# we1pingyu/CALD

Measured on AMD Instinct MI355X. Metric: unlabeled images scored/sec (CALD consistency sweep), higher is better.
Workload: dtype f32

## Files before the change

### cald_amd/_ffi.py

```python
import ctypes as C
import os

_HERE = os.path.dirname(os.path.abspath(__file__))
LIB_PATH = os.path.join(_HERE, "lib", "libcaldhip.so")
_lib = None

c_f = C.POINTER(C.c_float)
c_i = C.POINTER(C.c_int)
c_i64 = C.POINTER(C.c_int64)
c_d = C.POINTER(C.c_double)
c_u8 = C.POINTER(C.c_uint8)
c_i8 = C.POINTER(C.c_int8)


class ModelCfg(C.Structure):
    _fields_ = [("arch", C.c_int), ("depth", C.c_int), ("num_classes", C.c_int), ("min_size", C.c_int),
                ("max_size", C.c_int), ("box_score_thresh", C.c_float), ("box_nms_thresh", C.c_float),
                ("detections_per_img", C.c_int), ("rpn_pre_nms_top_n", C.c_int), ("rpn_post_nms_top_n", C.c_int),
                ("rpn_nms_thresh", C.c_float), ("precision", C.c_int)]


PRECISION = {"fp32": 0, "f16x3": 1}


# ... 144 lines not shown
    "cald_op_cls_corr": (C.c_int, [C.c_void_p, C.c_int, c_f, c_i64, C.c_int, c_f]),
    "cald_op_score_batch": (C.c_int, [C.c_void_p, C.POINTER(ScoreProbe)]),
    "cald_op_pair_params": (C.c_int, [C.c_int, C.c_int, C.c_int, C.c_double, c_f]),
    "cald_op_ls_tail": (C.c_int, [C.c_int, c_f, C.c_int, c_f, c_i, c_i, c_d]),
    "cald_op_coco_match": (C.c_int, [C.c_void_p, C.c_int, c_i64, c_i64, c_d, c_d, c_d, c_d, c_u8, c_u8, C.c_int, c_d, C.c_int, c_d,
                                     C.POINTER(C.c_int32), c_u8, c_u8]),
    "cald_op_voc_match": (C.c_int, [C.c_void_p, C.c_int, c_i64, c_i64, c_d, c_u8, c_d, c_i64, C.c_int, c_d, C.c_int64, c_d, c_i64, c_u8, c_u8]),
    "cald_op_pil_resize": (C.c_int, [C.c_void_p, C.c_void_p, C.c_int, C.c_int, C.c_void_p, C.c_int, C.c_int]),
    "cald_op_cutout_rects": (C.c_int, [C.c_uint64, C.c_int, C.c_int, C.c_int, c_f, C.c_int, c_i, c_i]),
    "cald_op_cutout_geometry": (C.c_int, [C.c_int, C.c_int, C.c_int, C.c_int, C.c_int, c_i, C.c_int, c_i, c_i]),
    "cald_op_augment": (C.c_int, [C.c_void_p, C.c_int, C.c_double, C.c_uint64, C.c_void_p, C.c_int, C.c_int, C.c_int, c_f,
                                  C.c_void_p, c_f, c_i]),
    "cald_op_noise_stream": (C.c_int, [C.c_void_p, C.c_uint64, C.c_void_p, C.c_int, C.c_int, C.c_int, c_i, c_d, C.POINTER(C.c_void_p)]),
    "cald_op_frcnn_postprocess": (C.c_int, [C.c_void_p, C.c_int, C.c_int, c_f, c_f, c_f, C.c_int, C.c_int, C.c_int, C.c_int, C.c_float, C.c_float,
                                            C.c_int, c_f, c_f, c_i64, c_f, c_f, c_f, c_i]),
    "cald_op_frcnn_postprocess_min": (C.c_int, [C.c_void_p, C.c_int, C.c_int, c_f, c_f, c_f, C.c_int, C.c_int, C.c_int, C.c_int, C.c_float, C.c_float,
                                                C.c_int, C.c_float, c_f, c_f, c_i64, c_f, c_f, c_f, c_i]),
    "cald_op_ssm_postprocess": (C.c_int, [C.c_void_p, C.c_int, C.c_int, c_f, c_f, c_f, C.c_int, C.c_int, C.c_int, C.c_int, C.c_float, C.c_int,
                                          c_i, c_i, c_f, c_f, c_i8]),
    "cald_op_retina_postprocess": (C.c_int, [C.c_void_p, C.POINTER(c_f), C.POINTER(c_f), c_i, C.c_int, C.c_int, c_f] + [C.c_int] * 6
                                   + [C.c_float, C.c_float, C.c_int, c_f, c_f, c_i64, c_f, c_f, c_i]),
    "cald_op_retina_ssm_postprocess": (C.c_int, [C.c_void_p, C.POINTER(c_f), C.POINTER(c_f), c_i, C.c_int, C.c_int, c_f] + [C.c_int] * 6
                                       + [C.c_float, C.c_float, C.c_int, C.c_void_p, C.c_void_p, c_i, c_i, c_i, c_f, c_f, c_i8]),
    "cald_op_rpn_prune": (C.c_int, [C.c_void_p, C.POINTER(RpnPruneProbe)]),
    "cald_op_roi_align": (C.c_int, [C.c_void_p, C.POINTER(c_f), c_i, C.c_int, C.c_int, c_f, c_f]),
    "cald_op_conv2d": (C.c_int, [C.c_void_p, c_f, C.c_int, C.c_int, C.c_int, c_f, C.c_int, C.c_int, C.c_int, C.c_int,
                                 C.c_int, c_f, c_f, c_f, c_f, C.c_int, c_f]),
    "cald_op_conv_probe": (C.c_int, [C.c_void_p, C.c_int, C.POINTER(ConvProbe), C.c_int, C.c_int, C.c_int, C.c_char_p, C.c_int]),
    "cald_op_mfma_f16": (C.c_int, [C.c_void_p, C.POINTER(C.c_uint16), C.POINTER(C.c_uint16), C.POINTER(C.c_uint32), C.POINTER(C.c_uint32), C.c_int64]),
    "cald_op_conv2d_f16x3": (C.c_int, [C.c_void_p, c_f, C.c_int, C.c_int, C.c_int, c_f, C.c_int, C.c_int, C.c_int, C.c_int,
                                       C.c_int, c_f, c_f, c_f, c_f, C.c_int, c_f]),
    "cald_op_conv_bench": (C.c_int, [C.c_void_p] + [C.c_int] * 12 + [c_d, c_d]),
    "cald_op_row_pack_lookup": (C.c_int, [C.c_int, c_i, c_i, C.c_int, C.c_int, C.c_int64, c_i64, c_i, c_i64, c_i64]),
    "cald_op_transform_size": (C.c_int, [C.c_int, C.c_int, C.c_int, C.c_int, c_i, c_i, c_i, c_i]),
    "cald_debug_tensor": (C.c_int, [C.c_void_p, C.c_char_p, C.c_int, c_f, C.c_int64, c_i64]),
    "cald_jpeg_info": (C.c_int, [C.c_void_p, C.c_size_t, c_i, c_i, c_i]),
    "cald_jpeg_decode_batch": (C.c_int, [C.c_void_p, C.c_int, C.POINTER(C.c_void_p), C.POINTER(C.c_size_t), C.POINTER(C.c_void_p)]),
    "cald_jpeg_probe": (C.c_int, [C.c_void_p, C.c_size_t, c_i, c_i, c_i, c_i]),
    "cald_jpeg_decode_batch_any": (C.c_int, [C.c_void_p, C.c_int, C.POINTER(C.c_void_p), C.POINTER(C.c_size_t), C.POINTER(C.c_void_p)]),
    "cald_jpeg_decode_host": (C.c_int, [C.c_void_p, C.c_size_t, C.c_void_p]),
    "cald_profile_enable": (C.c_int, [C.c_void_p, C.c_int]),
    "cald_profile_read": (C.c_int, [C.c_void_p, c_d, c_d, c_i64, c_d]),
    "cald_profile_prune": (C.c_int, [C.c_void_p, c_d, c_d, c_d, c_d, c_d]),
    "cald_profile_roi_rows": (C.c_int, [C.c_void_p, c_d, c_i64]),
    "cald_profile_cutout": (C.c_int, [C.c_void_p, c_d, c_d, c_i64, c_i64]),
    "cald_model_set_cutout_reuse": (C.c_int, [C.c_void_p, C.c_int, c_i]),
    "cald_profile_cutout_stages": (C.c_int, [C.c_void_p, c_d, c_d, c_d, c_d, c_i64]),
    "cald_model_set_cutout_retention_cap": (C.c_int, [C.c_void_p, C.c_int64, c_i64]),
    "cald_op_cutout_fpn_geometry": (C.c_int, [C.c_int, C.c_int, C.c_int, C.c_int, C.c_int, c_i, C.c_int, c_i, c_i]),
    "cald_model_set_look_fuse": (C.c_int, [C.c_void_p, C.c_int, c_i]),
    "cald_model_set_row_packing": (C.c_int, [C.c_void_p, C.c_int, c_i]),
    "cald_model_set_box_min_size": (C.c_int, [C.c_void_p, C.c_float, c_f]),
    "cald_profile_dump": (C.c_int, [C.c_void_p, C.c_char_p]),
    "cald_train_packed_floats": (C.c_int, [C.c_int] * 6 + [c_i64]),
    "cald_train_pack_conv": (C.c_int, [C.c_void_p] * 5 + [C.c_int] * 6 + [C.c_void_p]),
    "cald_train_pack_plan_scratch_floats": (C.c_int, [C.c_int, C.POINTER(PackJob), c_i64]),
    "cald_train_pack_plan_create": (C.c_int, [C.c_void_p, C.c_int, C.POINTER(PackJob), C.c_void_p, C.c_int64, C.POINTER(C.c_void_p)]),
    "cald_train_pack_plan_run": (C.c_int, [C.c_void_p, C.c_void_p]),
    "cald_train_pack_plan_destroy": (C.c_int, [C.c_void_p]),
    "cald_train_conv": (C.c_int, [C.c_void_p, C.c_int, C.c_int, C.c_int, C.c_void_p, C.c_int, C.c_void_p] + [C.c_int] * 8
                        + [C.c_void_p, C.c_void_p, C.c_int, C.c_int, C.c_void_p, C.c_void_p, C.c_int]),
    "cald_train_conv_group": (C.c_int, [C.c_void_p, C.c_int, C.c_int, c_i, C.POINTER(C.c_void_p), C.c_int, C.POINTER(C.c_void_p)] + [C.c_int] * 8
                              + [C.POINTER(C.c_void_p), C.POINTER(C.c_void_p), C.c_int]),
    "cald_train_conv_wgrad": (C.c_int, [C.c_void_p, C.c_int, C.c_int, C.c_int, C.c_void_p, C.c_int, C.c_int, C.c_void_p, C.c_int,
                                        C.c_int, C.c_int, C.c_int, C.c_int, C.c_int, C.c_void_p, C.c_void_p, C.c_void_p, C.c_int]),
    "cald_train_linear_wgrad": (C.c_int, [C.c_void_p, C.c_int, C.c_void_p, C.c_int, C.c_void_p, C.c_int, C.c_int, C.c_int,
                                          C.c_void_p, C.c_void_p, C.c_int]),
    "cald_train_wgrad_plan": (C.c_int, [C.c_longlong] + [C.c_int] * 12 + [C.POINTER(WgradPlan)]),
    "cald_train_relu_bwd": (C.c_int, [C.c_void_p, C.c_longlong, C.c_int, C.c_void_p, C.c_void_p, C.c_void_p]),
    "cald_train_add": (C.c_int, [C.c_void_p, C.c_longlong, C.c_void_p, C.c_void_p, C.c_void_p]),
    "cald_train_dilate": (C.c_int, [C.c_void_p] + [C.c_int] * 7 + [C.c_void_p, C.c_void_p]),
    "cald_train_upsample_bwd": (C.c_int, [C.c_void_p] + [C.c_int] * 6 + [C.c_void_p, C.c_void_p]),
    "cald_train_rpn_proposals": (C.c_int, [C.c_void_p, C.c_int, C.c_int, C.c_int, c_i, C.POINTER(C.c_void_p), c_i, C.c_int, C.c_int, C.c_int,
                                           C.c_float, C.c_float, C.c_void_p, C.c_void_p]),
    "cald_train_roi_sample_host": (C.c_int, [C.c_int, c_i, c_i, c_i, C.c_void_p, C.c_void_p, C.c_void_p, C.c_int, C.c_double, C.c_int, C.c_int,
                                             C.c_void_p, C.c_void_p, C.c_void_p, C.c_void_p, C.c_void_p, C.c_void_p, c_i, c_i, c_i]),
    "cald_train_roi_gather": (C.c_int, [C.c_void_p, C.c_void_p, C.c_void_p, C.c_void_p, C.c_int, C.c_int, C.c_int] + [C.c_float] * 4 + [C.c_void_p, C.c_void_p]),
    "cald_train_anchors": (C.c_int, [C.c_void_p, C.c_int, C.c_int, C.c_int, c_i, C.c_void_p]),
    "cald_train_match": (C.c_int, [C.c_void_p, C.c_int, C.c_void_p, C.c_int, C.c_void_p, C.c_float, C.c_float, C.c_int, C.c_void_p, C.c_void_p]),
    "cald_train_box_encode": (C.c_int, [C.c_void_p, C.c_int, C.c_void_p, C.c_void_p, C.c_float, C.c_float, C.c_float, C.c_float, C.c_void_p]),
    "cald_train_roi_align": (C.c_int, [C.c_void_p, C.POINTER(C.c_void_p), c_i, C.c_int, C.c_int, C.c_void_p, C.c_void_p]),
    "cald_train_roi_align_bwd": (C.c_int, [C.c_void_p, C.c_int, C.POINTER(C.c_void_p), c_i, C.c_int, C.c_int, C.c_void_p, C.c_void_p]),
    "cald_train_softmax_ce": (C.c_int, [C.c_void_p, C.c_int, C.c_int, C.c_int, C.c_void_p, C.c_void_p, C.c_float, C.c_void_p, C.c_void_p]),
    "cald_train_smooth_l1": (C.c_int, [C.c_void_p, C.c_int, C.c_void_p, C.c_void_p, C.c_void_p, C.c_float, C.c_float, C.c_void_p, C.c_float,
# ... 55 lines not shown
```

### cald_amd/csrc/common.h

```cpp
#pragma once
#include <hip/hip_runtime.h>
#include <stdint.h>
#include <math.h>

#define CALD_MAX_VIEWS 128
#define CALD_MAX_LEVELS 9
#define CALD_ROI_CAP 1000
#define CALD_MAX_CUT 4

struct LevelSeg {
    long long pix_off;
    int H, W;
    int tile_start;
    int pad_;
};

#if defined(__HIPCC__)
__device__ __forceinline__ int seg_find_view(const LevelSeg* __restrict__ seg, const int V, const int mt) {
    int lo = 0, hi = V - 1;
    while (lo < hi) {
        const int mid = (lo + hi + 1) >> 1;
        if (seg[mid].tile_start <= mt) lo = mid; else hi = mid - 1;
    }
    return lo;
}
__host__ __device__ __forceinline__ int seg_find_row(const LevelSeg* __restrict__ seg, const int V, const long long row) {
    int lo = 0, hi = V - 1;
    while (lo < hi) {
        const int mid = (lo + hi + 1) >> 1;
        if (seg[mid].pix_off <= row) lo = mid; else hi = mid - 1;
    }
    return lo;
}
#endif

static inline int conv_pack_rows(const LevelSeg* si, const LevelSeg* so, const LevelSeg* su, int V, int Cin, int out_ld) {
    const long long total = so[V].pix_off, LIM = 0x7FFE0000LL - (1 << 16);
    if (V < 1 || total < 1 || total > 0x7FFFFFFFLL - 128) return 0;
    int vf = 0;
    for (int v = 0; v < V; v++) {
        const long long b = so[v].pix_off, e = so[v + 1].pix_off;
        if (e == b) continue;
        if ((e - b + 128) * out_ld * 4 > LIM) return 0;
        if (b % 128 == 0) continue;
        const long long t0 = b / 128 * 128;
        while (so[vf + 1].pix_off <= t0) vf++;
        if ((si[v + 1].pix_off - si[vf].pix_off) * Cin * 4 > LIM) return 0;
        if (su && (su[v + 1].pix_off - su[vf].pix_off) * out_ld * 4 > LIM) return 0;
    }
    return (int)total;
}

struct BatchPlan {
    LevelSeg seg[CALD_MAX_LEVELS][CALD_MAX_VIEWS + 1];
};

#define CALD_GATHER_RECTS 8
struct GatherSet {
    int nr;
    int cum[CALD_GATHER_RECTS + 1];
    int x0[CALD_GATHER_RECTS], y0[CALD_GATHER_RECTS], w[CALD_GATHER_RECTS];
};
__device__ __forceinline__ int gather_pixel(const GatherSet& g, const int m, const int W) {
    int k = 0;
    while (k + 1 < g.nr && m >= g.cum[k + 1]) k++;
    const int j = m - g.cum[k], w = g.w[k], ry = j / w;
    return (g.y0[k] + ry) * W + g.x0[k] + (j - ry * w);
}

struct ConvArgs {
    const float* in;
    float* out;
    const float* w;
    const float* w4;
    const void* w16;
    float w16_unscale;
    const float* bias;
    const float* scale;
    const float* shift;
    const float* residual;
    const float* up;
    const LevelSeg* seg_in;
    const LevelSeg* seg_out;
    const LevelSeg* seg_up;
    const int* dyn_rows;
    const int* row_map;
    int V;
    int Cin, Cout, CoutPad, Kpad;
    int KH, KW, stride, pad;
    int relu;
    int total_mtiles;
    int out_ld;
    const float* zeros;
    int in_relu;
    const float* mask;
    const float* wstem;
// ... 174 lines not shown
```

### cald_amd/csrc/conv_p4.hip

```cpp
#include "h16.h"

typedef float f32x16 __attribute__((ext_vector_type(16)));
typedef int i32x4 __attribute__((ext_vector_type(4)));
typedef float f32x4 __attribute__((ext_vector_type(4)));

template <int EPI, bool MASK, int TM, int TN, bool GATHER = false, bool GEXTRA = false>
__device__ __forceinline__ void p4_epilogue(const ConvArgs& a, const f32x16 (&acc)[TM][TN], float* smem, const int v, const LevelSeg& so,
                                            const int m0, const int Mv, const int n0, const bool straddle = false) {
    constexpr int BM = 128, WN = 2;
    const int tid = threadIdx.x, lane = tid & 63, wave = tid >> 6;
    const int wm = wave / WN, wn = wave % WN;
    const int kh_lane = lane >> 5, l31 = lane & 31;
    const int Ho = so.H, Wo = so.W;
    const int out_ld = a.out_ld;
    float* __restrict__ out_v = a.out + so.pix_off * (long long)out_ld;
    const float* __restrict__ ex_v = nullptr;
    int upH = 1, upW = 1;
    float uph_s = 0.f, upw_s = 0.f;
    long long up_off = 0;
    if (EPI == 1) ex_v = a.residual + so.pix_off * (long long)out_ld;
    if (EPI == 2) {
        const LevelSeg su = a.seg_up[v];
        up_off = su.pix_off;
        ex_v = a.up + su.pix_off * (long long)out_ld;
        upH = su.H; upW = su.W;
        uph_s = (float)upH / (float)Ho; upw_s = (float)upW / (float)Wo;
    }
    const bool relu = a.relu != 0, has_bias = a.bias != nullptr, has_bn = a.scale != nullptr;
    constexpr bool has_mask = MASK;
    const float* __restrict__ mask_v = has_mask ? a.mask + so.pix_off * (long long)out_ld : out_v;
    const int row_b = out_ld * 4;
    const unsigned long long vb64 = (unsigned long long)(GATHER ? Ho * Wo : Mv) * (unsigned)row_b;
    const unsigned valid_b = vb64 < 0x7FFE0000ull ? (unsigned)vb64 : 0x7FFE0000u;
    const __amdgpu_buffer_rsrc_t rsO = __builtin_amdgcn_make_buffer_rsrc((void*)out_v, 0, valid_b, 0x00020000);
    const __amdgpu_buffer_rsrc_t rsX = __builtin_amdgcn_make_buffer_rsrc((void*)(EPI != 0 ? ex_v : out_v), 0, EPI == 1 ? valid_b : 0x7FFE0000, 0x00020000);
    const __amdgpu_buffer_rsrc_t rsM = __builtin_amdgcn_make_buffer_rsrc((void*)mask_v, 0, valid_b, 0x00020000);
    static_assert(!(GATHER && EPI == 2), "gathered rows take no top-down term");
    const int Mlast = Mv - 1;
    int* const s_src = reinterpret_cast<int*>(smem);
    if (EPI == 2 || GATHER) {
        if (tid < BM) {
            int m = m0 + tid;
            if (GATHER) {
                s_src[tid] = m < Mv ? gather_pixel(a.gather[v], m, Wo) * row_b : 0x7FFF0000;
            } else if (EPI == 2 && straddle) {
                int src = 0;
                if (m < Mv) {
                    const long long r = so.pix_off + m;
                    int vr = v;
                    while (vr + 1 < a.V && a.seg_out[vr + 1].pix_off <= r) vr++;
                    const LevelSeg sor = a.seg_out[vr], sur = a.seg_up[vr];
                    const int ml = (int)(r - sor.pix_off), oy = ml / sor.W, ox = ml - oy * sor.W;
                    const float hs = (float)sur.H / (float)sor.H, ws = (float)sur.W / (float)sor.W;
                    int sy = (int)floorf((float)oy * hs); sy = sy > sur.H - 1 ? sur.H - 1 : sy;
                    int sx = (int)floorf((float)ox * ws); sx = sx > sur.W - 1 ? sur.W - 1 : sx;
                    src = ((int)(sur.pix_off - up_off) + sy * sur.W + sx) * out_ld * 4;
                }
                s_src[tid] = src;
            } else {
                m = m < Mlast ? m : Mlast;
                const int oy = m / Wo, ox = m - oy * Wo;
                int sy = (int)floorf((float)oy * uph_s); sy = sy > upH - 1 ? upH - 1 : sy;
                int sx = (int)floorf((float)ox * upw_s); sx = sx > upW - 1 ? upW - 1 : sx;
                s_src[tid] = (sy * upW + sx) * out_ld * 4;
            }
        }
        __syncthreads();
    }
    auto gather_offs = [&](const int i, const int n, const bool nok, int (&go)[16]) {
        const int rl = wm * TM * 32 + i * 32 + 4 * kh_lane;
#pragma unroll
        for (int q = 0; q < 4; q++) {
            const i32x4 so4 = *reinterpret_cast<const i32x4*>(s_src + rl + 8 * q);
#pragma unroll
            for (int jj = 0; jj < 4; jj++) go[4 * q + jj] = nok ? so4[jj] + n * 4 : 0x7FFF0000;
        }
    };
// ... 152 lines not shown
    constexpr bool MASK = (EPIX & 4) != 0;
    constexpr bool FUSE = (EPIX & 8) != 0;
    constexpr bool GATHER = (EPIX & 16) != 0;
    constexpr bool GEXTRA = (EPIX & 32) != 0;
    static_assert(!GEXTRA || GATHER, "the extras bit rides on the gathered-rows bit");
    static_assert(!(GATHER && (FUSE || MASK || C4)), "gathered rows: plain EPI 0 / 1 kernels only");
    constexpr int BM = 128, BN = 64 * TN, BK = 16, TM = 2, WN = 2;
    constexpr int TILE_A = 2 * BM * 8, TILE_F = TILE_A + 2 * BN * 8;
    constexpr int FUSE_T = 4 * TILE_A;
    __shared__ __attribute__((aligned(16))) float smem[FUSE ? FUSE_T + 4096 : 3 * TILE_F];

    const int tid = threadIdx.x, lane = tid & 63, wave = tid >> 6;
    const int wm = wave / WN, wn = wave % WN;
    const int NT = a.CoutPad / BN;
    unsigned long long* const trace = (a.trace && blockIdx.x < (1u << 17)) ? a.trace + (size_t)blockIdx.x * 8 : nullptr;
    if (trace && tid == 0) {
        trace[0] = __builtin_amdgcn_s_memtime();
        trace[5] = (unsigned)__builtin_amdgcn_s_getreg((31 << 11) | 4);
        trace[6] = (unsigned)__builtin_amdgcn_s_getreg((31 << 11) | 20);
        trace[7] = blockIdx.x;
    }
    int mt, nt;
    if (a.KH * a.KW > 1) {
        const int MT = a.total_mtiles, CH = (MT + 7) >> 3;
        const int xcd = blk & 7, idx = blk >> 3;
        mt = xcd * CH + idx / NT; nt = idx % NT;
        if (idx / NT >= CH || mt >= MT) return;
    } else {
        const int b = blk, MT = a.total_mtiles, MT8 = MT & ~7;
        if (b < MT8 * NT) { const int xcd = b & 7, idx = b >> 3; mt = (idx / NT) * 8 + xcd; nt = idx % NT; }
        else { const int r = b - MT8 * NT; mt = MT8 + r / NT; nt = r % NT; }
    }
    const int n0 = nt * BN;
    constexpr bool CAN_PACK = !C4 && !MASK && !FUSE && !GATHER;
    const bool packed = CAN_PACK && a.packed_rows != 0;
    const int v = packed ? seg_find_row(a.seg_out, a.V, (long long)mt * BM) : seg_find_view(a.seg_out, a.V, mt);
    const LevelSeg so = a.seg_out[v];
    const LevelSeg si = a.seg_in[v];
    const int Ho = so.H, Wo = so.W, Hi = si.H, Wi = si.W;
    int Mv = Ho * Wo;
    if (a.dyn_rows) { const int d = a.dyn_rows[v]; Mv = d < Mv ? d : Mv; }
    if (GATHER) Mv = a.gather[v].cum[a.gather[v].nr];
    int m0 = (mt - so.tile_start) * BM;
    bool straddle = false;
    if (CAN_PACK && packed) {
        const int row0 = mt * BM, left = a.packed_rows - row0;
        m0 = row0 - (int)so.pix_off;
        const int end = m0 + (left < BM ? left : BM);
        straddle = end > Mv;
        Mv = end;
    }
    if (m0 >= Mv) return;
    const float* __restrict__ in_v = a.in + si.pix_off * (long long)a.Cin;
    const int Cin = a.Cin, KW = a.KW, KH = a.KH, CoutPad = a.CoutPad;
    const bool in_relu = a.in_relu != 0;

    const int g = tid & 3, arow = tid >> 2;
    unsigned rowmask[2];
    int rowvoff[2], riy0[2], rix0[2];
    int tapw[2] = {0, 0};
#pragma unroll
    for (int p = 0; p < 2; p++) {
        const int m = m0 + arow + 64 * p;
        int ml = m, Wo_r = Wo, Hi_r = Hi, Wi_r = Wi, dpix = 0;
        if (CAN_PACK && straddle && m < Mv) {
            const long long r = so.pix_off + m;
            int vr = v;
            while (vr + 1 < a.V && a.seg_out[vr + 1].pix_off <= r) vr++;
            const LevelSeg sor = a.seg_out[vr], sir = a.seg_in[vr];
            ml = (int)(r - sor.pix_off); Wo_r = sor.W; Hi_r = sir.H; Wi_r = sir.W; dpix = (int)(sir.pix_off - si.pix_off);
        }
        const int mp = GATHER ? (m < Mv ? gather_pixel(a.gather[v], m, Wo) : 0) : (a.row_map && m < Mv) ? a.row_map[so.pix_off + m] : ml;
        const int oy = mp / Wo_r, ox = mp - oy * Wo_r;
        const int iy0 = oy * a.stride - a.pad, ix0 = ox * a.stride - a.pad;
        unsigned msk = 0;
        if (!C4 && m < Mv)
            for (int t = 0; t < KH * KW; t++) {
                const int th = t / KW, tw = t - th * KW;
                const int iy = iy0 + th, ix = ix0 + tw;
                if (iy >= 0 && iy < Hi_r && ix >= 0 && ix < Wi_r) msk |= 1u << t;
            }
        rowmask[p] = msk;
        rowvoff[p] = (((oy * a.stride) * Wi + ox * a.stride) * Cin + (C4 ? 0 : 4 * g)) * 4;
        if (CAN_PACK && straddle) { rowvoff[p] = ((dpix + iy0 * Wi_r + ix0) * Cin + 4 * g) * 4; tapw[p] = Wi_r; }
        riy0[p] = m < Mv ? iy0 : -0x40000000; rix0[p] = ix0;
    }
    const int Wi_s = straddle ? 0 : Wi, Cin_s = straddle ? 0 : Cin, cin_v4 = straddle ? Cin * 4 : 0;
    const __amdgpu_buffer_rsrc_t rsA = __builtin_amdgcn_make_buffer_rsrc(
        (void*)(in_v - (straddle ? 0ll : (long long)a.pad * (Wi + 1) * Cin)), 0, 0x7FFE0000, 0x00020000);
    const __amdgpu_buffer_rsrc_t rsB = __builtin_amdgcn_make_buffer_rsrc((void*)(a.w4 + (long long)n0 * 8), 0, 0x7FFE0000, 0x00020000);
    int u_kh = 0, u_kw = 0, u_ci = 0, u_kt = 0;
    const int a_kq = g >> 1, a_j = 2 * (g & 1);
    int aw_off[2][2];
#pragma unroll
    for (int p = 0; p < 2; p++) {
        const int r = arow + 64 * p;
#pragma unroll
        for (int h = 0; h < 2; h++) aw_off[p][h] = ((a_kq * BM + r) * 2 + (h ^ ((r >> 3) & 1))) * 4 + a_j;
    }
    const int b_t = TN == 2 ? tid : (tid & 127), b_kq = TN == 2 ? 0 : (tid >> 7);
    const int b_nl = b_t >> 1, b_h = b_t & 1;
    const int bvoff0 = (b_kq * CoutPad * 8 + b_nl * 8 + b_h * 4) * 4, bvoff1 = bvoff0 + CoutPad * 8 * 4;
    const int bw_off0 = TILE_A + ((b_kq * BN + b_nl) * 2 + (b_h ^ ((b_nl >> 3) & 1))) * 4, bw_off1 = bw_off0 + BN * 8;

    f32x4 ra0, ra1, rb0, rb1 = {0.f, 0.f, 0.f, 0.f};
// ... 344 lines not shown
__global__ __launch_bounds__(256, 3) void conv_p4_kernel(const ConvArgs a) { conv_p4_body<EPI, C4, TN, TAPS>(a, blockIdx.x); }
template <int EPI, bool C4, int TN, int TAPS>
__global__ __launch_bounds__(256, 3) void conv_p4_group_kernel(const ConvGroup g) {
    int i = 0;
    while (i + 1 < g.n && g.blk0[i + 1] <= (int)blockIdx.x) i++;
    conv_p4_body<EPI, C4, TN, TAPS>(g.p[i], (int)blockIdx.x - g.blk0[i]);
}
__global__ __launch_bounds__(256, 3) void conv_p4_fused_kernel(const ConvGroup g) { conv_p4_body<8, false, 1, 9>(g.p[0], blockIdx.x, &g.p[1]); }

static inline int p4_taps(const ConvArgs& a) {
    if (a.Cin % 16 != 0) return 0;
    if (a.KH == 3 && a.KW == 3) return 9;
    if (a.KH == 1 && a.KW == 1) return 1;
    return 0;
}

static inline int p4_grid_mtiles(const ConvArgs& a) { return a.KH * a.KW > 1 ? 8 * ((a.total_mtiles + 7) / 8) : a.total_mtiles; }

static inline bool p4_refuses(const ConvArgs& a) {
    if (!a.w4 || !a.out || a.in16 || a.ex16 || a.CoutPad % 64 != 0 || (a.residual && a.up)) return true;
    const bool extra = a.out16 || a.energy4;
    if (extra && (a.residual || a.up || a.mask)) return true;
    if (a.energy4 && a.CoutPad != 256) return true;
    if (a.row_map && (a.residual || a.up || a.mask || a.gather)) return true;
    return false;
}
static inline bool p4_tile_ok(const ConvArgs& a, const bool wide, const ConvForce f) {
    if (f.tile == TILE_NARROW && wide) return false;
    if (f.tile == TILE_WIDE && !wide) return false;
    return !(a.energy4 && !wide);
}

static inline ConvArgs p4_tiled(ConvArgs a) {
    if (a.packed_rows > 0 && a.Cin != 4 && !a.dyn_rows && !a.row_map && !a.gather && !a.mask) a.total_mtiles = (a.packed_rows + 127) / 128;
    else a.packed_rows = 0;
    return a;
}

#define P4_NAME(K, EPIV, C4V, TNV, TAPSV) K "<" #EPIV "," #C4V "," #TNV "," #TAPSV ">"
template <int EPI, bool C4, int TN, int TAPS>
static const char* p4_go(const dim3 grid, hipStream_t stream, const ConvArgs& a, const char* name) {
    hipLaunchKernelGGL((conv_p4_kernel<EPI, C4, TN, TAPS>), grid, dim3(256), 0, stream, a);
    return name;
}
template <int EPI, int TN, int TAPS>
static const char* p4_group_go(const dim3 grid, hipStream_t stream, const ConvGroup& g, const char* name) {
    hipLaunchKernelGGL((conv_p4_group_kernel<EPI, false, TN, TAPS>), grid, dim3(256), 0, stream, g);
    return name;
}

const char* launch_conv_p4_group(const ConvArgs* p, int n, hipStream_t stream, ConvForce f) {
    if (n < 1 || n > CALD_MAX_GROUP) return nullptr;
    const bool wide = f.tile == TILE_NARROW ? false : p[0].CoutPad % 128 == 0;
    ConvGroup g; g.n = n; int blk = 0;
    for (int i = 0; i < n; i++) {
        const ConvArgs a = p4_tiled(p[i]);
        if (p4_refuses(a) || !p4_tile_ok(a, wide, f) || (a.CoutPad % 128 == 0) != (p[0].CoutPad % 128 == 0)) return nullptr;
        if (a.Cin % 16 != 0 || a.KH * a.KW > 32 || a.residual || a.up) return nullptr;
        if ((a.mask != nullptr) != (p[0].mask != nullptr) || (a.gather != nullptr) != (p[0].gather != nullptr)) return nullptr;
        if (a.gather && (!wide || p4_taps(a) != 9 || a.mask || a.in_relu || a.dyn_rows || a.row_map)) return nullptr;
        if (a.mask && (a.out16 || a.energy4)) return nullptr;
        g.blk0[i] = blk; blk += p4_grid_mtiles(a) * (a.CoutPad / (wide ? 128 : 64)); g.p[i] = a;
    }
    g.blk0[n] = blk;
    const int taps = p4_taps(p[0]);
    for (int i = 1; i < n; i++) if (p4_taps(p[i]) != taps) return nullptr;
    const dim3 grid((unsigned)blk);
// ... 70 lines not shown
```

### cald_amd/csrc/ctx.hip

```cpp
#include "host.h"

static thread_local char g_err[512] = "";
int cald_host::fail(int code, const char* fmt, ...) {
    va_list ap; va_start(ap, fmt); vsnprintf(g_err, sizeof(g_err), fmt, ap); va_end(ap);
    return code;
}

int cald_internal_fail(int code, const char* fmt, ...) {
    va_list ap; va_start(ap, fmt); vsnprintf(g_err, sizeof(g_err), fmt, ap); va_end(ap);
    return code;
}
void cald_internal_train_release(cald_ctx* c);

extern "C" const char* cald_last_error(void) { return g_err; }
extern "C" int cald_version(void) { return 100; }

hipStream_t cald_internal_stream(cald_ctx* c) { return c->stream; }
int cald_internal_device(cald_ctx* c) { return c->device; }
const float* cald_internal_zeros(cald_ctx* c) { return c->d_zeros; }
int cald_internal_scratch(cald_ctx* c, size_t bytes, void** out) {
    if (bytes > c->train_scratch_cap) {
        HIPCHK(hipStreamSynchronize(c->stream));
        if (c->train_scratch) HIPCHK(hipFree(c->train_scratch));
        c->train_scratch = nullptr; c->train_scratch_cap = 0;
// ... 129 lines not shown
    return 0;
}

extern "C" int cald_profile_roi_rows(cald_ctx* c, double* mean_rows_per_view, int64_t* views) {
    if (!c) return fail(CALD_ERR_INVALID, "ctx is null");
    HIPCHK(hipStreamSynchronize(c->stream));
    unsigned long long rows = 0;
    HIPCHK(hipMemcpy(&rows, c->d_roi_rows, 8, hipMemcpyDeviceToHost));
    if (views) *views = c->prof_roi_views;
    if (mean_rows_per_view) *mean_rows_per_view = c->prof_roi_views ? (double)rows / (double)c->prof_roi_views : 0.0;
    return 0;
}

extern "C" int cald_profile_cutout(cald_ctx* c, double* rows3, double* dense_rows3, int64_t* batches, int64_t* fallbacks) {
    if (!c) return fail(CALD_ERR_INVALID, "ctx is null");
    for (int i = 0; i < 3; i++) { if (rows3) rows3[i] = c->cut_rows[i]; if (dense_rows3) dense_rows3[i] = c->cut_dense[i]; }
    if (batches) *batches = c->cut_batches;
    if (fallbacks) *fallbacks = c->cut_fallbacks;
    return 0;
}

extern "C" int cald_profile_cutout_stages(cald_ctx* c, double* rows6, double* dense_rows6, double* tiles6, double* dense_tiles6, int64_t* kept3) {
    if (!c) return fail(CALD_ERR_INVALID, "ctx is null");
    for (int i = 0; i < 6; i++) {
        if (rows6) rows6[i] = c->cut_st_rows[i];
        if (dense_rows6) dense_rows6[i] = c->cut_st_dense[i];
        if (tiles6) tiles6[i] = c->cut_st_tiles[i];
        if (dense_tiles6) dense_tiles6[i] = c->cut_st_dense_tiles[i];
    }
    if (kept3) for (int i = 0; i < 3; i++) kept3[i] = c->cut_kept[i];
    return 0;
}

extern "C" int cald_profile_dump(cald_ctx* c, const char* path) {
    if (!c || !path) return fail(CALD_ERR_INVALID, "null argument");
    HIPCHK(hipStreamSynchronize(c->stream));
    FILE* f = fopen(path, "w");
    if (!f) return fail(CALD_ERR_INVALID, "cannot open %s", path);
    fprintf(f, "launch,desc,gflop,ms,tflops\n");
    std::vector<unsigned long long> lg((size_t)CALD_PRUNE_LOG * 4, 0ull);
    if (!c->prof_gather.empty()) HIPCHK(hipMemcpy(lg.data(), c->d_prune_log, lg.size() * 8, hipMemcpyDeviceToHost));
    for (size_t i = 0; i < c->prof_launches.size(); i++) {
        const ProfLaunch& L = c->prof_launches[i];
        float t = 0.f; hipEventElapsedTime(&t, L.e0, L.e1);
        double fl = L.flops;
        const char* extra = L.tag ? ",f16x3-lookahead" : "";
        auto g = c->prof_gather.find(i);
        if (g != c->prof_gather.end()) {
            for (int l = 0; l < 2; l++) {
                const unsigned long long sel = lg[(size_t)g->second.log * 4 + 2 * l], tot = lg[(size_t)g->second.log * 4 + 2 * l + 1];
                if (tot) fl -= g->second.cap[l] * (1.0 - (double)sel / (double)tot);
            }
            extra = ",gathered-rows";
        }
        fprintf(f, "%zu,\"%s%s\",%.3f,%.4f,%.2f\n", i, L.desc.c_str(), extra, fl / 1e9, t, fl / (t * 1e-3) / 1e12);
    }
    fclose(f);
    return 0;
}
extern "C" int cald_profile_prune_fallbacks(cald_ctx* c, int64_t* n) {
    if (!c || !n) return fail(CALD_ERR_INVALID, "null argument");
    *n = (int64_t)c->prune_fallbacks;
    return 0;
}

int cald_host::prof_begin(cald_ctx* c, ProfLaunch& t) {
    if (!c->prof) return 0;
    HIPCHK(hipEventCreate(&t.e0)); HIPCHK(hipEventCreate(&t.e1));
    HIPCHK(hipEventRecord(t.e0, c->stream));
    return 0;
}
int cald_host::prof_end(cald_ctx* c, ProfLaunch& t, double flops, int tag, const char* fmt, ...) {
    if (!c->prof) return 0;
    HIPCHK(hipEventRecord(t.e1, c->stream));
    char d[160];
    va_list ap; va_start(ap, fmt); vsnprintf(d, sizeof(d), fmt, ap); va_end(ap);
    t.flops = flops; t.tag = tag; t.desc = d;
    c->prof_launches.push_back(t); c->prof_flops += flops;
    return 0;
}

int cald_host::conv_refused(const ConvArgs& a) {
    return fail(CALD_ERR_UNSUPPORTED, "no conv kernel implements this launch (Cin=%d Cout=%d k=%dx%d residual=%d up=%d mask=%d gather=%d energy4=%d out16=%d)",
                a.Cin, a.Cout, a.KH, a.KW, a.residual != nullptr, a.up != nullptr, a.mask != nullptr, a.gather != nullptr, a.energy4 != nullptr,
                a.out16 != nullptr);
}
int cald_host::run_conv(cald_ctx* c, const ConvArgs& a, double flops) {
    ProfLaunch t; int rc;
    if ((rc = prof_begin(c, t))) return rc;
    const char* k = launch_conv(a, c->stream);
    if ((rc = prof_end(c, t, flops, c->prof_tag_now, "mt=%d,Cin=%d,Cout=%d,k=%dx%d,s=%d", a.total_mtiles, a.Cin, a.Cout, a.KH, a.KW, a.stride))) return rc;
    if (!k) return conv_refused(a);
    return 0;
}
```

### cald_amd/csrc/forward.hip

```cpp
#include "host.h"

#define ROI_DENSE_VIEWS 32
void cald_host::build_plan(BatchPlan& P, int V, const ViewDesc* views, const int (*hp)[2], bool retina) {
    memset(&P, 0, sizeof(P));
    for (int l = 0; l < CALD_MAX_LEVELS; l++) {
        long long off = 0; int tile = 0;
        for (int v = 0; v <= V; v++) {
            LevelSeg& s = P.seg[l][v];
            s.pix_off = off; s.tile_start = tile;
            if (v == V) break;
            int H, W;
            if (l == 7 && retina) { int h6 = (hp[v][0] / 32 - 1) / 2 + 1, w6 = (hp[v][1] / 32 - 1) / 2 + 1; H = (h6 - 1) / 2 + 1; W = (w6 - 1) / 2 + 1; }
            else if (l == 7) { H = 1; W = CALD_ROI_CAP; }
            else if (l == 8) {
                const int first = v * ROI_DENSE_VIEWS, cnt = first < V ? (V - first < ROI_DENSE_VIEWS ? V - first : ROI_DENSE_VIEWS) : 0;
                H = cnt ? 1 : 0; W = cnt * CALD_ROI_CAP;
            }
            else if (l == 6) { H = (hp[v][0] / 32 - 1) / 2 + 1; W = (hp[v][1] / 32 - 1) / 2 + 1; }
            else { H = hp[v][0] >> l; W = hp[v][1] >> l; }
            s.H = H; s.W = W;
            off += (long long)H * W;
            tile += (H * W + 127) / 128;
        }
    }
// ... 257 lines not shown
        if ((rc = prof_begin(c, t))) return rc;
        if (launch_conv_p4_fused(a2, a3, c->stream) != nullptr)
            return prof_end(c, t, f2 + f3, 0, "mt=%d,Cin=%d,Cout=%d,k=3x3+1x1,s=1,fused->%d", a2.total_mtiles, a2.Cin, a2.Cout, a3.Cout);
        if (c->prof) { hipEventDestroy(t.e0); hipEventDestroy(t.e1); }
    }
    int rc = conv_on(m, L2, in, mid, lin, lout, V, true);
    if (rc) return rc;
    return conv_on(m, L3, mid, out, lout, lout, V, true, residual);
}
static int conv_group_on(cald_model* m, const ConvSpec* sp, int n, int V) {
    ConvArgs a[CALD_MAX_GROUP];
    double flops = 0.0; int tiles = 0;
    for (int i = 0; i < n; i++) {
        const double f = fill_conv_args(m, a[i], *sp[i].L, sp[i].in, sp[i].out, sp[i].level, sp[i].level, V, sp[i].relu, nullptr, nullptr, 0, sp[i].dyn);
        if (f < 0.0) return (int)f;
        a[i].row_map = sp[i].row_map;
        if (sp[i].in16) a[i].in16 = sp[i].in16;
        if (sp[i].out16) a[i].out16 = sp[i].out16;
        a[i].energy4 = sp[i].energy4;
        offer_packing(m, a[i], sp[i].level, sp[i].level, 0, V);
        flops += f; tiles += a[i].total_mtiles;
    }
    cald_ctx* c = m->ctx;
    const char* names[CALD_MAX_GROUP];
    ProfLaunch t; int rc;
    if ((rc = prof_begin(c, t))) return rc;
    const int launches = launch_conv_group(a, n, c->stream, names);
    if (c->prof) c->prof_extra_launches += launches - 1;
    if ((rc = prof_end(c, t, flops, c->prof_tag_now, "mt=%d,Cin=%d,Cout=%d,k=%dx%d,s=%d,group=%d", tiles, a[0].Cin, a[0].Cout, a[0].KH, a[0].KW, a[0].stride, n))) return rc;
    for (int i = 0; i < n; i++) if (!names[i]) return conv_refused(a[i]);
    return 0;
}

static int gconv_on(cald_model* m, const ConvLayer& L, const float* in, float* out, int lin, int lout, int V, bool relu, const float* residual,
                    const FwdReuse& ru, int b, int kind) {
    if (!ru.tiles[b][kind]) return 0;
    ConvArgs a;
    const double f = fill_conv_args(m, a, L, in, out, lin, lout, V, relu, residual);
    if (f < 0.0) return (int)f;
    const char* base = ru.d_gp + (size_t)(2 * b + kind) * cut_plan_set_bytes(V);
    a.seg_out = reinterpret_cast<const LevelSeg*>(base);
    a.gather = reinterpret_cast<const GatherSet*>(base + (size_t)(V + 1) * sizeof(LevelSeg));
    a.total_mtiles = ru.tiles[b][kind];
    return run_conv(m->ctx, a, 2.0 * ru.rows[b][kind] * (double)L.Cout * (double)(L.KH * L.KW * L.CinTrue));
}

static int gconv_group_on(cald_model* m, const ConvSpec* sp, int n, int V, const FwdReuse& ru) {
    ConvArgs a[CALD_MAX_GROUP];
    double flops = 0.0; int tiles = 0;
    for (int i = 0; i < n; i++) {
        const double f = fill_conv_args(m, a[i], *sp[i].L, sp[i].in, sp[i].out, sp[i].level, sp[i].level, V, sp[i].relu);
        if (f < 0.0) return (int)f;
        const char* base = ru.d_gp + (size_t)(2 * ru.nblk + i) * cut_plan_set_bytes(V);
        a[i].seg_out = reinterpret_cast<const LevelSeg*>(base);
        a[i].gather = reinterpret_cast<const GatherSet*>(base + (size_t)(V + 1) * sizeof(LevelSeg));
        a[i].total_mtiles = ru.fpn_tiles[i];
        a[i].out16 = sp[i].out16; a[i].energy4 = sp[i].energy4;
        flops += 2.0 * ru.fpn_rows[i] * (double)sp[i].L->Cout * (double)(sp[i].L->KH * sp[i].L->KW * sp[i].L->CinTrue); tiles += ru.fpn_tiles[i];
    }
    if (!tiles) return 0;
    cald_ctx* c = m->ctx;
    ProfLaunch t; int rc;
    if ((rc = prof_begin(c, t))) return rc;
    const char* k = launch_conv_p4_group(a, n, c->stream);
    if ((rc = prof_end(c, t, flops, c->prof_tag_now, "mt=%d,Cin=%d,Cout=%d,k=%dx%d,s=%d,group=%d,gathered-rows", tiles, a[0].Cin, a[0].Cout, a[0].KH, a[0].KW, a[0].stride, n))) return rc;
    return k ? 0 : conv_refused(a[0]);
}

__global__ void accumulate_rows_kernel(const int* __restrict__ counts, int V, unsigned long long* acc) {
    unsigned long long s = 0;
    for (int v = threadIdx.x; v < V; v += 64) s += (unsigned long long)counts[v];
    for (int o = 32; o > 0; o >>= 1) s += __shfl_down(s, o);
    if (threadIdx.x == 0) atomicAdd(acc, s);
}

static const float RPN_MIN_SIZE = 1e-3f;
struct ForwardRun {
    cald_model* m; int V; ViewDesc* views; const DetBuffers& det; float* audit_out; bool prune_ok; const FwdReuse* ru; FwdFeatures* feat; FwdSsm* ssm; FwdRetinaSsm* rssm;
    cald_ctx* c = nullptr; hipStream_t st = nullptr; const BatchPlan* dp = nullptr;
    bool retina = false, prune = false;
    int hp[CALD_MAX_VIEWS][2], max_pix0 = 0, max_pix2 = 0, max_pix6 = 0;
    BodyBufs Fb; PyramidBufs Fp; RetinaBufs Fr; RpnBufs Fn; PruneBufs Fq; BoxBufs Fx; AuditBufs Fa;
    void layout(Bump& B) {
        const BatchPlan& P = m->plan; long long px[8];
        for (int l = 0; l < 8; l++) px[l] = level_pix(P, l, V);
        m->split.clear();
        static const bool split_on = !(getenv("CALD_H3_S16") && atoi(getenv("CALD_H3_S16")) == 0);
        SplitReg S{m, B, m->cfg.precision == CALD_PRECISION_F16X3 && split_on};
        Fb.layout(B, S, px);
        Fp.layout(B, S, px, retina);
        if (feat) return;
// ... 49 lines not shown
        { Bump real(c->arena, false); layout(real); }
        const int si = c->stage_i; c->stage_i = (si + 1) % cald_ctx::NSTAGE;
        HIPCHK(hipEventSynchronize(c->stage_ev[si]));
        memcpy(c->h_stage[si], &m->plan, sizeof(BatchPlan));
        memcpy(c->h_stage[si] + sizeof(BatchPlan), views, sizeof(ViewDesc) * V);
        HIPCHK(hipMemcpyAsync(c->d_plan, c->h_stage[si], sizeof(BatchPlan), hipMemcpyHostToDevice, c->stream));
        HIPCHK(hipMemcpyAsync(c->d_views, c->h_stage[si] + sizeof(BatchPlan), sizeof(ViewDesc) * V, hipMemcpyHostToDevice, c->stream));
        HIPCHK(hipEventRecord(c->stage_ev[si], c->stream));
        dp = c->d_plan; st = c->stream;
        m->dbg.clear();
        return 0;
    }
    int dense_block(const Bottleneck& B, const float* cur, float* dst, int lvl, int lout) {
        int rc; const float* idn = cur;
        if (B.has_down) { if ((rc = conv_on(m, B.down, cur, Fb.D, lvl, lout, V, false))) return rc; idn = Fb.D; }
        if ((rc = conv_on(m, B.c1, cur, Fb.T1, lvl, lvl, V, true))) return rc;
        return conv_pair_on(m, B.c2, B.c3, Fb.T1, Fb.T2, dst, lvl, lout, V, idn);
    }
    int gathered_block(const Bottleneck& B, int b, const float* cur, float* dst, int lvl, int lout) {
        int rc; const float* idn = cur;
        if (B.has_down) { if ((rc = gconv_on(m, B.down, cur, Fb.D, lvl, lout, V, false, nullptr, *ru, b, 0))) return rc; idn = Fb.D; }
        if ((rc = gconv_on(m, B.c1, cur, Fb.T1, lvl, lvl, V, true, nullptr, *ru, b, 1))) return rc;
        if ((rc = gconv_on(m, B.c2, Fb.T1, Fb.T2, lvl, lout, V, true, nullptr, *ru, b, 0))) return rc;
        return gconv_on(m, B.c3, Fb.T2, dst, lout, lout, V, true, idn, *ru, b, 0);
    }
    int body() {
        int rc;
        launch_preprocess(c->d_views, dp->seg[0], Fb.in0, V, max_pix0, st);
        m->dbg["input"] = {Fb.in0, 0, 4, 0};
        if ((rc = conv_on(m, m->conv1, Fb.in0, Fb.c1, 0, 1, V, true))) return rc;
        m->dbg["conv1"] = {Fb.c1, 1, 64, 0};
        launch_maxpool(Fb.c1, Fb.p1, dp->seg[1], dp->seg[2], 64, V, max_pix2, st, m->split.count(Fb.p1) != 0);
        m->dbg["pool1"] = {Fb.p1, 2, 64, 0};
        const float* cur = Fb.p1; int lvl = 2, layer = 0, xi = 0;
        for (size_t b = 0; b < m->blocks.size(); b++) {
            const Bottleneck& B = m->blocks[b];
            const int lout = lvl + (B.c2.stride == 2 ? 1 : 0);
            const bool kept = ru && (int)b < ru->nblk;
            float* dst = kept ? ru->out[b] : (B.layer_end ? Fb.Cf[layer] : Fb.X[xi]);
            if ((rc = kept && ru->mode == 2 && ru->gather[layer] ? gathered_block(B, (int)b, cur, dst, lvl, lout) : dense_block(B, cur, dst, lvl, lout))) return rc;
            if (B.layer_end) Fb.Cf[layer] = dst;
            cur = dst; lvl = lout;
            if (B.layer_end) layer++; else xi ^= 1;
        }
        const char* cn[4] = {"C2", "C3", "C4", "C5"};
        for (int i = 0; i < 4; i++) m->dbg[cn[i]] = {Fb.Cf[i], 2 + i, CCH[i], 0};
        return 0;
    }
    void name_pyramid(int first, int n) { for (int i = 0; i < n; i++) m->dbg["P" + std::to_string(first + i)] = {Fp.Pf[i], first + i, 256, 0}; }
    int fpn() {
        const int first = retina ? 3 : 2, nl = retina ? 3 : 4, c0 = 4 - nl;
        int rc; ConvSpec sp[4];
        const bool kept = ru && ru->fpn && !retina;
        if (kept) {
            for (int i = 0; i < 4; i++) Fp.Pf[i] = ru->pf[i];
            if (prune) for (int i = 0; i < 2; i++) { Fq.p16[i] = ru->p16[i]; Fq.energy[i] = ru->energy[i]; }
        }
        if ((rc = conv_on(m, m->fpn_inner[nl - 1], Fb.Cf[3], Fp.inner[nl - 1], 5, 5, V, false))) return rc;
        for (int i = nl - 2; i >= 0; i--)
            if ((rc = conv_on(m, m->fpn_inner[i], Fb.Cf[c0 + i], Fp.inner[i], first + i, first + i, V, false, nullptr, Fp.inner[i + 1], first + 1 + i))) return rc;
        for (int i = 0; i < nl; i++) m->dbg["inner" + std::to_string(first + i)] = {Fp.inner[i], first + i, 256, 0};
        for (int i = 0; i < nl; i++) sp[i] = {&m->fpn_layer[i], Fp.inner[i], Fp.Pf[i], first + i, false};
        if (prune)
            for (int i = 0; i < 2; i++) { sp[i].out16 = Fq.p16[i]; sp[i].energy4 = Fq.energy[i]; }
        if ((rc = kept && ru->mode == 2 && ru->gather_fpn ? gconv_group_on(m, sp, nl, V, *ru) : conv_group_on(m, sp, nl, V))) return rc;
        if (!retina) return 0;
        if ((rc = conv_on(m, m->p6, Fp.Pf[2], Fp.Pf[3], 5, 6, V, false))) return rc;
        if (feat && !feat->p7) return 0;
        return conv_on(m, m->p7, Fp.Pf[3], Fp.Pf[4], 6, 7, V, false, nullptr, nullptr, 0, nullptr, true);
    }
    void hand_out(int first, int n) {
        name_pyramid(first, n);
        for (int i = 0; i < n; i++) {
            auto sp = m->split.find(Fp.Pf[i]);
// ... 252 lines not shown
```

### cald_amd/csrc/host.h

```cpp
#pragma once
#include "../../include/cald_hip.h"
#include "common.h"
#include "kernels.h"
#include "host_logic.h"

#include <climits>
#include <cmath>
#include <cstdarg>
#include <cstdio>
#include <cstring>
#include <algorithm>
#include <map>
#include <string>
#include <vector>

namespace cald_host {
int fail(int code, const char* fmt, ...);
#define HIPCHK(x) do { hipError_t e_ = (x); if (e_ != hipSuccess) return fail(CALD_ERR_HIP, "%s failed: %s (%s:%d)", #x, hipGetErrorString(e_), __FILE__, __LINE__); } while (0)

struct PilCoef { int ksize; int* d_bounds; int* d_kk; };
struct PilKey { int in, out, fid; bool operator<(const PilKey& o) const { return in != o.in ? in < o.in : (out != o.out ? out < o.out : fid < o.fid); } };
struct ProfLaunch {
    hipEvent_t e0 = nullptr, e1 = nullptr;
    double flops = 0.0;
// ... 3 lines not shown
}
using namespace cald_host;

#define CALD_PRUNE_LOG 4096
struct cald_ctx {
    int device = 0;
    hipStream_t stream = nullptr;
    bool own_stream = false;
    char* arena = nullptr; size_t arena_cap = 0, arena_off = 0;
    BatchPlan* d_plan = nullptr;
    ViewDesc* d_views = nullptr;
    float* d_zeros = nullptr;
    static const int NSTAGE = 8;
    char* h_stage[NSTAGE] = {nullptr}; hipEvent_t stage_ev[NSTAGE] = {nullptr}; int stage_i = 0;
    bool prof = false;
    std::vector<ProfLaunch> prof_launches;
    double prof_flops = 0.0; int64_t prof_extra_launches = 0;
    int prof_tag_now = 0;
    double prof_prune_flops_cap[2] = {0.0, 0.0};
    hipEvent_t tot0 = nullptr, tot1 = nullptr; bool tot_open = false; double tot_ms = 0.0;
    float prune_worst = 0.0f;
    long long prune_fallbacks = 0;
    float* d_prune_check = nullptr;
    unsigned long long* d_prune_stat = nullptr;
    unsigned long long* d_prune_log = nullptr; int prune_log_n = 0;
    struct GatherNote { int log; double cap[2]; };
    std::map<size_t, GatherNote> prof_gather;
    unsigned long long* d_roi_rows = nullptr; double prof_roi_rows_cap = 0.0, prof_roi_flops_cap = 0.0; long long prof_roi_views = 0;
    std::map<PilKey, PilCoef> pil;
    char* train_scratch = nullptr; size_t train_scratch_cap = 0;
    double cut_rows[3] = {0.0, 0.0, 0.0}, cut_dense[3] = {0.0, 0.0, 0.0};
    long long cut_batches = 0, cut_fallbacks = 0;
    double cut_st_rows[6] = {}, cut_st_dense[6] = {}, cut_st_tiles[6] = {}, cut_st_dense_tiles[6] = {};
    long long cut_kept[3] = {0, 0, 0};
};

namespace cald_host {
struct ScopedDev {
    std::vector<void*> ptrs;
    hipStream_t st;
    explicit ScopedDev(hipStream_t s) : st(s) {}
    ~ScopedDev() { if (!ptrs.empty()) { hipStreamSynchronize(st); for (void* p : ptrs) hipFree(p); } }
    void release() { ptrs.clear(); }
    template <typename T> int alloc(T** out, size_t bytes) {
        HIPCHK(hipMalloc((void**)out, bytes ? bytes : 1));
        ptrs.push_back((void*)*out);
        return 0;
    }
    template <typename T> int upload(T** out, const void* h, size_t bytes) {
        *out = nullptr;
        if (!h) return 0;
        if (int rc = alloc(out, bytes)) return rc;
        HIPCHK(hipMemcpy((void*)*out, h, bytes, hipMemcpyHostToDevice));
        return 0;
    }
};
struct Bump {
    char* base; size_t off = 0; bool dry;
    explicit Bump(char* b, bool d) : base(b), dry(d) {}
    template <typename T> T* get(size_t count) {
        size_t bytes = (count * sizeof(T) + 255) & ~(size_t)255;
        T* p = dry ? nullptr : reinterpret_cast<T*>(base + off);
        off += bytes;
        return p;
    }
};

struct HostTensor { std::vector<float> data; std::vector<int64_t> shape; };
struct ConvLayer {
    float *w = nullptr, *w4 = nullptr, *bias = nullptr, *scale = nullptr, *shift = nullptr;
    float* wstem = nullptr;
    uint16_t* w16 = nullptr; float w16_unscale = 1.0f;
    int Cin = 0, Cout = 0, CoutPad = 0, K = 0, Kpad = 0, KH = 1, KW = 1, stride = 1, pad = 0;
    int CinTrue = 0;
};
struct Bottleneck { ConvLayer c1, c2, c3, down; bool has_down = false; bool layer_end = false; };
struct DebugEntry { const float* ptr; int level; int C; int kind; };
}

struct cald_model {
    cald_ctx* ctx = nullptr;
    cald_model_cfg cfg;
    std::map<std::string, HostTensor> sd;
    bool finalized = false;
    ConvLayer conv1; std::vector<Bottleneck> blocks;
    ConvLayer fpn_inner[4], fpn_layer[4], rpn_conv, rpn_head, fc6, fc7, pred;
    ConvLayer rpn_conv16; bool prune = false; float prune_c1[3] = {0, 0, 0}, prune_c0[3] = {0, 0, 0};
    bool prune_allowed = false;
    int look_fuse = 1; float* look_head_w = nullptr; float look_head_b[3] = {0, 0, 0};
    int row_packing = -1;
    bool prune_bound_voided = false;
    bool prune_capture = false;
    ConvLayer p6, p7, cls_tower[4], reg_tower[4], cls_out, reg_out;
    int det_cap() const { return cfg.arch == CALD_ARCH_RETINANET ? cfg.num_classes * cfg.detections_per_img : cfg.detections_per_img; }
    float* d_anchors = nullptr;
    std::vector<void*> owned;
    std::map<std::string, DebugEntry> dbg;
    BatchPlan plan; int last_V = 0;
    struct SplitFmt { unsigned* s16; bool fp32_dead; };
    std::map<const float*, SplitFmt> split;
    std::vector<ViewDesc> last_views;
    DetBuffers sweep_det; int sweep_det_views = 0;
    DetBuffers sweep_det2; int sweep_det2_views = 0;
    struct SweepScratch {
        size_t dev_bytes = 0, pin_bytes = 0, aug_cap = 0;
        char* dev = nullptr; char* pin = nullptr; uint8_t* d_aug = nullptr;
        hipEvent_t ev_ref[2] = {nullptr, nullptr}, ev_score[2] = {nullptr, nullptr};
    } ss;
    float box_min_size = 0.0f;
    int key_cap = 32768;
    struct CutReuse {
        int mode = -1;
        char* slot[2] = {nullptr, nullptr}; size_t cap[2] = {0, 0};
        bool ext_refused = false;
        size_t ext_cap = 0;
        char* h_gp[2] = {nullptr, nullptr}; char* d_gp = nullptr;
    } cr;
};

namespace cald_host {
struct ConvPack {
    std::vector<float> w, w4, wstem;
    std::vector<uint16_t> w16; float w16_unscale = 1.0f;
    int Cout = 0, CoutPad = 0, K = 0, Kpad = 0;
};
struct ConvSpec { const ConvLayer* L; const float* in; float* out; int level; bool relu; const int* dyn = nullptr; const int* row_map = nullptr; const unsigned* in16 = nullptr;
                  unsigned* out16 = nullptr; float* energy4 = nullptr; };

#define CUT_MAX_BLOCKS 36
#define CUT_STAGE_LATERAL 4
#define CUT_STAGE_OUTPUT 5
#define CUT_KEPT_FPN 0
#define CUT_KEPT_STAGES 1
#define CUT_KEPT_NONE 2
struct FwdReuse {
    int mode = 0;
    int nblk = 0;
    float* out[CUT_MAX_BLOCKS] = {};
    bool gather[3] = {false, false, false};
    const char* d_gp = nullptr;
    int tiles[CUT_MAX_BLOCKS][2] = {};
    double rows[CUT_MAX_BLOCKS][2] = {};
    bool fpn = false, gather_fpn = false;
    float* pf[4] = {}; unsigned* p16[2] = {}; float* energy[2] = {};
    int fpn_tiles[4] = {};
    double fpn_rows[4] = {};
};
struct FwdFeatures {
    const int (*pad_to)[2] = nullptr;
    bool p7 = false;
    const float* P[5] = {}; bool split_only[5] = {}; int plan_level[5] = {};
};
struct ProposalBufs { float* proposals = nullptr; int* prop_count = nullptr; void layout(Bump& B, int V); };
struct RoiBufs { float* roi = nullptr; int* order = nullptr; void layout(Bump& B, int V, int C); };
struct PostBufs {
    float *prob = nullptr, *pmax = nullptr, *cbox = nullptr; unsigned long long* keys = nullptr; int* key_count = nullptr; int key_cap = 0;
    unsigned char* skip = nullptr;
    void layout(Bump& B, int V, int C, int key_cap);
};
struct SsmBufs {
    float *prob = nullptr, *kept_box = nullptr, *boxes = nullptr, *scores = nullptr; unsigned* vmax = nullptr; signed char* labels = nullptr;
    int *kept_prop = nullptr, *cls_count = nullptr, *row_off = nullptr, *al = nullptr, *count = nullptr, *total = nullptr;
    void layout(Bump& B, int V, int C, int cap);
};
struct FwdSsm { SsmBufs out; };
#define SSM_NMS_THR 0.3f
#define SSM_CONF_THR 0.5f
struct RetinaTailBufs {
    int *cand_count = nullptr, *kept_anchor = nullptr, *kept_count = nullptr, cand_cap = 0, max_anchors = 0; unsigned long long* cand_key = nullptr;
    float *cand_box = nullptr, *kept_box = nullptr; unsigned char* cand_skip = nullptr;
    void layout(Bump& B, int V, int K, int per_class, int max_anchors);
};
struct RetinaSsmBufs {
    int *cand_count = nullptr, *blk_off = nullptr, *list = nullptr, *al = nullptr, *picks = nullptr, *n_picks = nullptr, *kept_anchor = nullptr, *kept_count = nullptr,
        *row_off = nullptr, *count = nullptr, *total = nullptr, cand_cap = 0, nblk = 0;
    unsigned* vmax = nullptr; float *kept_box = nullptr, *boxes = nullptr, *scores = nullptr; signed char* labels = nullptr;
    void layout(Bump& B, int V, int K, int per_class, int max_anchors);
};
struct FwdRetinaSsm { cald_ssm_pick_fn pick = nullptr; void* user = nullptr; int image0 = 0; RetinaSsmBufs out; };
RetinaSsmArgs retina_ssm_args(const RetinaSsmBufs& S, const float* const* cls, const float* const* reg, const BatchPlan* plan, const ViewDesc* views,
                              const float* base_anchors, int A, int K, int V, float score_thr, float nms_thr, int per_class);
int retina_ssm_pick_stop(cald_ctx* c, const RetinaSsmBufs& S, int V, int K, cald_ssm_pick_fn pick, void* user, int image0, int* h_counts);
RoiArgs roi_args(const RoiBufs& S, const float* const* feat, const BatchPlan* plan, int C, int V, const ProposalBufs& P, bool out16);
PostArgs post_args(const PostBufs& S, const float* pred, int pred_ld, int C, int V, const ProposalBufs& P, const ViewDesc* views,
                   float score_thr, float nms_thr, const DetBuffers& det);
SsmArgs ssm_args(const SsmBufs& S, const float* pred, int pred_ld, int C, int V, const ProposalBufs& P, const ViewDesc* views, float score_thr, int cap);
RetinaArgs retina_args(const RetinaTailBufs& S, const float* const* cls, const float* const* reg, const BatchPlan* plan, const ViewDesc* views,
                       const float* base_anchors, int A, int K, int V, float score_thr, float nms_thr, int per_class, const DetBuffers& det);
inline size_t cut_plan_set_bytes(int V) { return (size_t)(V + 1) * sizeof(LevelSeg) + (size_t)V * sizeof(GatherSet); }
inline long long level_pix(const BatchPlan& P, int l, int V) { return P.seg[l][V].pix_off; }

int arena_reserve(cald_ctx* c, size_t bytes);
int prof_begin(cald_ctx* c, ProfLaunch& t);
int prof_end(cald_ctx* c, ProfLaunch& t, double flops, int tag, const char* fmt, ...);
int conv_refused(const ConvArgs& a);
int run_conv(cald_ctx* c, const ConvArgs& a, double flops);
int pil_resize(cald_ctx* c, const uint8_t* src, int H, int W, uint8_t* dst, int oh, int ow, uint8_t* tmp, int fid = 0);
std::vector<float> pack_w4(const std::vector<float>& w, int Kpad, int CoutPad);
void pack_conv(const std::vector<const float*>& ts, const std::vector<int>& couts, int cin, int cinp, int kh, int kw, int stride, int pad,
               bool want16, ConvPack* P);
void build_plan(BatchPlan& P, int V, const ViewDesc* views, const int (*hp)[2], bool retina);
bool stem_grid_exact(const LevelSeg* seg, int V);
bool conv_pack_default();
int forward_model(cald_model* m, int V, ViewDesc* views, const DetBuffers& det, float* audit_out = nullptr, bool prune_ok = false,
                  const FwdReuse* ru = nullptr, FwdFeatures* feat = nullptr, FwdSsm* ssm = nullptr, FwdRetinaSsm* rssm = nullptr);
void free_det(DetBuffers& d);
int alloc_det(DetBuffers& d, int V, int cap, int C);
struct ScopedDet { DetBuffers d{}; ~ScopedDet() { free_det(d); } int alloc(int V, int cap, int C) { return alloc_det(d, V, cap, C); } };
struct PairLayout {
    int P_MAX, B, VT;
    struct Ptrs { int *ref_view, *aug_view, *aug_kind, *pair_img, *ref_sel, *ref_n, *view_img, *view_isref; };
    size_t n_ints() const { return (size_t)P_MAX * 4 + (size_t)B * 51 + (size_t)VT * 2; }
    Ptrs at(int* base) const {
        Ptrs p;
        p.ref_view = base; p.aug_view = p.ref_view + P_MAX; p.aug_kind = p.aug_view + P_MAX; p.pair_img = p.aug_kind + P_MAX;
        p.ref_sel = p.pair_img + P_MAX; p.ref_n = p.ref_sel + (size_t)B * 50; p.view_img = p.ref_n + B; p.view_isref = p.view_img + VT;
        return p;
    }
    ScoreArgs score_args(int* d_base, const DetBuffers& D, const float* d_par, int P, float bp, float* cons) const {
        const Ptrs p = at(d_base);
        ScoreArgs sa; sa.det = D;
        sa.ref_view = p.ref_view; sa.aug_view = p.aug_view; sa.aug_kind = p.aug_kind; sa.pair_img = p.pair_img;
        sa.ref_sel = p.ref_sel; sa.ref_n = p.ref_n; sa.aug_param = d_par; sa.P = P; sa.bp = bp; sa.cons = cons;
        return sa;
    }
};
}
```

### cald_amd/csrc/lossnet.hip

```cpp
#include "host.h"
#include "h16.h"

#define GAP_CHUNK 256
#define LL_C 256

struct GapArgs {
    const float* feat[4];
    const LevelSeg* seg[4];
    int split[4];
    int nslot, V, chunk_stride;
    float* partial;
};

__global__ __launch_bounds__(256) void gap_partial_kernel(const GapArgs a) {
    __shared__ float4 sm[4][64];
    const int s = blockIdx.y, v = blockIdx.z, chunk = blockIdx.x;
    const LevelSeg sg = a.seg[s][v];
    const int N = sg.H * sg.W, p0 = chunk * GAP_CHUNK;
    if (p0 >= N) return;
    const int n = N - p0 < GAP_CHUNK ? N - p0 : GAP_CHUNK;
    const int phase = threadIdx.x >> 6, cq = threadIdx.x & 63;
    const int cnt = n > phase ? (n - phase + 3) >> 2 : 0;
    float4 acc = make_float4(0.f, 0.f, 0.f, 0.f);
    if (!a.split[s]) {
// ... 164 lines not shown
    HIPCHK(hipMemcpyAsync(d_seg, sg, sizeof(sg), hipMemcpyHostToDevice, c->stream));
    GapArgs a; memset(&a, 0, sizeof(a));
    a.feat[0] = d_x; a.seg[0] = d_seg; a.nslot = 1; a.V = 1; a.chunk_stride = nch; a.partial = d_part;
    GapFinishArgs fa; memset(&fa, 0, sizeof(fa)); fa.pooled = d_mean;
    if ((rc = run_gap(c, a, fa, 1, nch, (long long)N * LL_C * 4))) return rc;
    HIPCHK(hipMemcpyAsync(mean_out, d_mean, LL_C * 4, hipMemcpyDeviceToHost, c->stream));
    HIPCHK(hipStreamSynchronize(c->stream));
    return 0;
}

extern "C" int cald_op_lossnet(cald_lossnet* ln, int n, const float* pooled, float* out) {
    if (!ln || !pooled || !out || n < 1) return fail(CALD_ERR_INVALID, "bad argument");
    if (!ln->finalized) return fail(CALD_ERR_STATE, "LossNet not finalized (call cald_lossnet_finalize)");
    cald_ctx* c = ln->ctx;
    HIPCHK(hipSetDevice(c->device));
    ScopedDev scratch(c->stream);
    float *d_p = nullptr, *d_o = nullptr; int rc;
    if ((rc = scratch.alloc(&d_p, (size_t)n * 4 * LL_C * 4)) || (rc = scratch.alloc(&d_o, (size_t)n * 4))) return rc;
    HIPCHK(hipMemcpyAsync(d_p, pooled, (size_t)n * 4 * LL_C * 4, hipMemcpyHostToDevice, c->stream));
    launch_head(ln, n, d_p, d_o, c->stream);
    HIPCHK(hipGetLastError());
    HIPCHK(hipMemcpyAsync(out, d_o, (size_t)n * 4, hipMemcpyDeviceToHost, c->stream));
    HIPCHK(hipStreamSynchronize(c->stream));
    return 0;
}

int cald_internal_scratch(cald_ctx* c, size_t bytes, void** out);

struct DenseHW { int H[4], W[4]; };
__global__ void dense_seg_fill_kernel(LevelSeg* seg, const int N, const DenseHW g) {
    const int i = blockIdx.x * blockDim.x + threadIdx.x;
    if (i >= 4 * N) return;
    const int l = i / N, n = i % N, H = g.H[l], W = g.W[l];
    LevelSeg s; s.pix_off = (long long)n * H * W; s.H = H; s.W = W; s.tile_start = n * ((H * W + 127) / 128); s.pad_ = 0;
    seg[i] = s;
}

extern "C" int cald_train_gap(cald_ctx* c, int N, const float* const* maps, const int* level_hw, float* pooled) {
    if (!c || !maps || !level_hw || !pooled) return fail(CALD_ERR_INVALID, "null argument");
    if (N < 1 || N > CALD_MAX_VIEWS) return fail(CALD_ERR_INVALID, "batch of %d images outside [1, %d]", N, CALD_MAX_VIEWS);
    DenseHW g; int max_chunks = 1; long long bytes = 0;
    for (int l = 0; l < 4; l++) {
        const int H = level_hw[2 * l], W = level_hw[2 * l + 1];
        if (!maps[l] || H < 1 || W < 1 || (long long)H * W > (1ll << 22)) return fail(CALD_ERR_INVALID, "level %d: bad map (%d x %d)", l, H, W);
        g.H[l] = H; g.W[l] = W;
        const int ch = (H * W + GAP_CHUNK - 1) / GAP_CHUNK;
        if (ch > max_chunks) max_chunks = ch;
        bytes += (long long)N * H * W * LL_C * 4;
    }
    HIPCHK(hipSetDevice(c->device));
    const size_t seg_bytes = ((size_t)4 * N * sizeof(LevelSeg) + 255) / 256 * 256;
    void* scratch = nullptr; int rc;
    if ((rc = cald_internal_scratch(c, seg_bytes + (size_t)N * 4 * max_chunks * LL_C * 4, &scratch))) return rc;
    LevelSeg* d_seg = reinterpret_cast<LevelSeg*>(scratch);
    hipLaunchKernelGGL(dense_seg_fill_kernel, dim3((4 * N + 255) / 256), dim3(256), 0, c->stream, d_seg, N, g);
    GapArgs a; memset(&a, 0, sizeof(a));
    for (int l = 0; l < 4; l++) { a.feat[l] = maps[l]; a.seg[l] = d_seg + (size_t)l * N; }
    a.nslot = 4; a.V = N; a.chunk_stride = max_chunks; a.partial = reinterpret_cast<float*>(reinterpret_cast<char*>(scratch) + seg_bytes);
    GapFinishArgs fa; for (int j = 0; j < 4; j++) fa.branch_slot[j] = j;
    fa.pooled = pooled;
    return run_gap(c, a, fa, 4, max_chunks, bytes);
}

extern "C" int cald_sweep_ll(cald_model* m, cald_lossnet* ln, int n_images, const uint8_t* const* images_dev, const int* H, const int* W,
                             const int* group, const cald_ll_cfg* cfg, double* uncertainty_out, float* pooled_out) {
    if (!m || !ln || !images_dev || !H || !W || !group || !uncertainty_out || n_images < 0) return fail(CALD_ERR_INVALID, "null argument");
    if (!m->finalized) return fail(CALD_ERR_STATE, "model not finalized");
// ... 78 lines not shown
```

### cald_amd/csrc/model.hip

```cpp
#include "host.h"

extern "C" int cald_model_create(cald_ctx* ctx, const cald_model_cfg* cfg, cald_model** out) {
    if (!ctx || !cfg || !out) return fail(CALD_ERR_INVALID, "null argument");
    if (cfg->arch != CALD_ARCH_FRCNN && cfg->arch != CALD_ARCH_RETINANET) return fail(CALD_ERR_INVALID, "unknown arch %d", cfg->arch);
    if (cfg->depth != 50 && cfg->depth != 101) return fail(CALD_ERR_INVALID, "depth must be 50 or 101");
    if (cfg->num_classes < 2 || cfg->num_classes > 256) return fail(CALD_ERR_INVALID, "num_classes out of range");
    if (cfg->rpn_pre_nms_top_n > 1024 || cfg->rpn_post_nms_top_n > CALD_ROI_CAP || cfg->rpn_pre_nms_top_n < 1 || cfg->rpn_post_nms_top_n < 1)
        return fail(CALD_ERR_INVALID, "rpn top-n out of range (pre <= 1024, post <= %d)", CALD_ROI_CAP);
    if (cfg->detections_per_img < 1 || cfg->detections_per_img > 1024) return fail(CALD_ERR_INVALID, "detections_per_img out of range");
    if (cfg->precision != CALD_PRECISION_FP32 && cfg->precision != CALD_PRECISION_F16X3) return fail(CALD_ERR_INVALID, "unknown precision %d", cfg->precision);
    cald_model* m = new cald_model();
    m->ctx = ctx; m->cfg = *cfg;
    {
        const float thr = cfg->box_score_thresh;
        long long per = cfg->num_classes - 1;
        if (thr > 0.0f && std::isfinite(thr)) { const long long lim = (long long)std::ceil(1.0 / (double)thr) - 1; if (lim < per) per = lim < 1 ? 1 : lim; }
        long long need = (long long)CALD_ROI_CAP * per;
        int kc = 1024; while (kc < need) kc <<= 1;
        m->key_cap = kc;
    }
    memset(&m->sweep_det, 0, sizeof(m->sweep_det)); memset(&m->sweep_det2, 0, sizeof(m->sweep_det2));
    *out = m;
    return 0;
}
// ... 259 lines not shown
        }
        if ((rc = make_conv(m, m->cls_out, {"head.classification_head.cls_logits.weight"}, {"head.classification_head.cls_logits.bias"}, "", 1, 1))) return rc;
        if ((rc = make_conv(m, m->reg_out, {"head.regression_head.bbox_reg.weight"}, {"head.regression_head.bbox_reg.bias"}, "", 1, 1))) return rc;
        if (m->cls_out.Cout != 9 * m->cfg.num_classes || m->reg_out.Cout != 36)
            return fail(CALD_ERR_INVALID, "RetinaNet heads must have 9*num_classes / 36 outputs (got %d / %d)", m->cls_out.Cout, m->reg_out.Cout);
        std::vector<float> base(5 * 9 * 4);
        const float ratios[3] = {0.5f, 1.0f, 2.0f};
        for (int l = 0; l < 5; l++) {
            const int x = 32 << l;
            const float sizes[3] = {(float)x, (float)(int)((double)x * pow(2.0, 1.0 / 3)), (float)(int)((double)x * pow(2.0, 2.0 / 3))};
            for (int r = 0; r < 3; r++) {
                float hr = sqrtf(ratios[r]), wr = 1.0f / hr;
                for (int sidx = 0; sidx < 3; sidx++) {
                    float ws = wr * sizes[sidx], hs = hr * sizes[sidx];
                    float* b = &base[((l * 9) + r * 3 + sidx) * 4];
                    b[0] = rintf(-ws / 2.0f); b[1] = rintf(-hs / 2.0f); b[2] = rintf(ws / 2.0f); b[3] = rintf(hs / 2.0f);
                }
            }
        }
        if ((rc = upload(m, base, &m->d_anchors))) return rc;
    }
    m->sd.clear();
    m->finalized = true;
    return 0;
}
extern "C" int cald_model_set_rpn_prune(cald_model* m, int on, int* was) {
    if (!m) return fail(CALD_ERR_INVALID, "model is null");
    if (!m->finalized) return fail(CALD_ERR_STATE, "model not finalized");
    if (was) *was = m->prune ? 1 : 0;
    m->prune = on != 0 && m->prune_allowed;
    return 0;
}
extern "C" int cald_model_set_cutout_reuse(cald_model* m, int mode, int* was) {
    if (!m || mode < -1 || mode > 2) return fail(CALD_ERR_INVALID, "bad argument");
    if (was) *was = m->cr.mode;
    m->cr.mode = mode;
    return 0;
}
extern "C" int cald_model_set_cutout_retention_cap(cald_model* m, int64_t bytes, int64_t* was) {
    if (!m || bytes < 0) return fail(CALD_ERR_INVALID, "bad argument");
    if (was) *was = (int64_t)m->cr.ext_cap;
    m->cr.ext_cap = (size_t)bytes;
    return 0;
}
extern "C" int cald_model_set_row_packing(cald_model* m, int mode, int* was) {
    if (!m || mode < -1 || mode > 1) return fail(CALD_ERR_INVALID, "bad argument");
    if (was) *was = m->row_packing;
    m->row_packing = mode;
    return 0;
}
extern "C" int cald_model_set_look_fuse(cald_model* m, int mode, int* was) {
    if (!m || mode < 0 || mode > 2) return fail(CALD_ERR_INVALID, "bad argument");
    if (was) *was = m->look_fuse;
    m->look_fuse = mode;
    return 0;
}
extern "C" int cald_model_set_box_min_size(cald_model* m, float min_size, float* was) {
    if (!m || !(min_size >= 0.0f)) return fail(CALD_ERR_INVALID, "bad argument");
    if (m->cfg.arch != CALD_ARCH_FRCNN) return fail(CALD_ERR_INVALID, "box_min_size belongs to the Faster R-CNN tail (RetinaNet's always removes small boxes)");
    if (was) *was = m->box_min_size;
    m->box_min_size = min_size;
    return 0;
}
extern "C" int cald_model_set_rpn_prune_capture(cald_model* m, int on) {
    if (!m) return fail(CALD_ERR_INVALID, "model is null");
    if (on && !(m->prune && m->prune_allowed)) return fail(CALD_ERR_STATE, "certified RPN pruning is not active on this model");
    m->prune_capture = on != 0;
    return 0;
}
extern "C" int cald_model_rpn_prune_bound(cald_model* m, float* c1, float* c0) {
    if (!m || !c1 || !c0) return fail(CALD_ERR_INVALID, "null argument");
    if (!m->rpn_conv16.w16) return fail(CALD_ERR_STATE, "the model has no look-ahead layer (not an exact Faster R-CNN model)");
    for (int a = 0; a < 3; a++) { c1[a] = m->prune_c1[a]; c0[a] = m->prune_c0[a]; }
    return 0;
}
extern "C" int cald_model_set_rpn_prune_bound(cald_model* m, const float* c1, const float* c0) {
    if (!m || !c1 || !c0) return fail(CALD_ERR_INVALID, "null argument");
    if (!m->rpn_conv16.w16) return fail(CALD_ERR_STATE, "the model has no look-ahead layer (not an exact Faster R-CNN model)");
    for (int a = 0; a < 3; a++) { m->prune_c1[a] = c1[a]; m->prune_c0[a] = c0[a]; }
    m->prune_bound_voided = true;
    return 0;
// ... 18 lines not shown
```

### cald_amd/csrc/ops.hip

```cpp
#include "host.h"

extern "C" int cald_op_transform_size(int H, int W, int min_size, int max_size, int* Hr, int* Wr, int* Hp, int* Wp) {
    if (H <= 0 || W <= 0 || min_size <= 0 || max_size <= 0) return fail(CALD_ERR_INVALID, "bad sizes");
    transform_size(H, W, min_size, max_size, Hr, Wr, Hp, Wp);
    return 0;
}

extern "C" int cald_op_cutout_rects(uint64_t seed, int H, int W, int N, const float* boxes, int cut_num, int* rects_out, int* n_out) {
    if (cut_num < 0 || cut_num > CALD_MAX_CUT) return fail(CALD_ERR_INVALID, "cut_num must be 0..%d", CALD_MAX_CUT);
    *n_out = cutout_rects(seed, H, W, N, boxes, cut_num, rects_out);
    return 0;
}

extern "C" int cald_op_cutout_geometry(int H, int W, int min_size, int max_size, int nrect, const int* rects, int nblk, const int* strides, int* out) {
    if (H < 1 || W < 1 || nrect < 0 || nrect > CALD_MAX_CUT || (nrect && !rects) || nblk < 0 || nblk > 64 || (nblk && !strides) || !out)
        return fail(CALD_ERR_INVALID, "bad argument");
    int Hr, Wr, Hp, Wp;
    transform_size(H, W, min_size, max_size, &Hr, &Wr, &Hp, &Wp);
    std::vector<CutSet> o(nblk + 1), t(nblk + 1);
    cut_geometry(H, W, Hr, Wr, Hp, Wp, nrect, rects, nblk, strides, &o[0], o.data() + 1, t.data() + 1);
    t[0].n = 0;
    for (int e = 0; e <= nblk; e++)
        for (int k = 0; k < 2; k++) {
            const CutSet& sset = k ? t[e] : o[e];
// ... 196 lines not shown
    for (int i = 0; i < n; i++) {
        const cald_conv_probe& p = pr[i];
        if (p.V < 1 || p.V > CALD_PROBE_MAX_VIEWS || p.Cin < 4 || p.Cin % 4 || p.Cout < 1 || p.KH < 1 || p.KW < 1 || p.stride < 1 || p.pad < 0 ||
            p.out_ld < p.Cout || !p.weight || !p.in)
            return fail(CALD_ERR_INVALID, "cald_op_conv_probe: problem %d: bad layer", i);
        std::vector<LevelSeg> seg(3 * (CALD_PROBE_MAX_VIEWS + 1));
        memset(seg.data(), 0, seg.size() * sizeof(LevelSeg));
        LevelSeg* si = &seg[0]; LevelSeg* so = &seg[CALD_PROBE_MAX_VIEWS + 1]; LevelSeg* su = &seg[2 * (CALD_PROBE_MAX_VIEWS + 1)];
        std::vector<GatherSet> gs(p.V);
        long long rows_out = 0;
        for (int v = 0; v < p.V; v++) {
            const int H = p.in_hw[v][0], W = p.in_hw[v][1];
            if (H < 0 || W < 0) return fail(CALD_ERR_INVALID, "cald_op_conv_probe: negative view size");
            const int Ho = H && W ? (H + 2 * p.pad - p.KH) / p.stride + 1 : 0, Wo = H && W ? (W + 2 * p.pad - p.KW) / p.stride + 1 : 0;
            if (Ho < 0 || Wo < 0 || (H && W && (Ho < 1 || Wo < 1))) return fail(CALD_ERR_INVALID, "cald_op_conv_probe: view %d smaller than the filter", v);
            si[v].H = H; si[v].W = W; so[v].H = Ho; so[v].W = Wo; su[v].H = p.up_hw[v][0]; su[v].W = p.up_hw[v][1];
            long long m = (long long)Ho * Wo;
            if (p.gather) {
                GatherSet& g = gs[v]; memset(&g, 0, sizeof(g));
                if (p.nrect[v] < 0 || p.nrect[v] > CALD_GATHER_RECTS) return fail(CALD_ERR_INVALID, "cald_op_conv_probe: 0..%d rectangles", CALD_GATHER_RECTS);
                g.nr = p.nrect[v];
                for (int k = 0; k < g.nr; k++) {
                    const int* r = p.rect[v][k];
                    if (r[0] < 0 || r[1] < 0 || r[2] < 1 || r[3] < 1 || r[0] + r[2] > Wo || r[1] + r[3] > Ho)
                        return fail(CALD_ERR_INVALID, "cald_op_conv_probe: rectangle outside view %d", v);
                    g.x0[k] = r[0]; g.y0[k] = r[1]; g.w[k] = r[2]; g.cum[k + 1] = g.cum[k] + r[2] * r[3];
                }
                m = g.cum[g.nr];
            }
            si[v + 1].pix_off = si[v].pix_off + (long long)H * W;
            so[v + 1].pix_off = so[v].pix_off + (long long)Ho * Wo;
            su[v + 1].pix_off = su[v].pix_off + (long long)su[v].H * su[v].W;
            so[v + 1].tile_start = so[v].tile_start + (int)((m + 127) / 128);
            si[v + 1].tile_start = si[v].tile_start + (H * W + 127) / 128;
            rows_out = so[v + 1].pix_off;
        }
        const long long pix_in = si[p.V].pix_off, pix_up = su[p.V].pix_off;
        if ((p.out && p.out_n < rows_out * p.out_ld) || (p.out16 && p.out16_n < rows_out * p.out_ld) || (p.energy4 && p.energy4_n < rows_out * 4))
            return fail(CALD_ERR_INVALID, "cald_op_conv_probe: problem %d: an output buffer is smaller than the output", i);
        ConvPack pk;
        const int cin_true = p.cin_true > 0 ? p.cin_true : p.Cin;
        if (cin_true > p.Cin) return fail(CALD_ERR_INVALID, "cald_op_conv_probe: cin_true > Cin");
        pack_conv({p.weight}, {p.Cout}, cin_true, p.Cin, p.KH, p.KW, p.stride, p.pad, precision == CALD_PRECISION_F16X3, &pk);
        if (!stem_grid_exact(so, p.V)) pk.wstem.clear();
        ConvArgs& A = a[i]; memset(&A, 0, sizeof(A));
        const LevelSeg* d_seg;
        const size_t out_b = (size_t)p.out_ld * 4;
        if ((rc = upload_layer(sd, pk, p.bias, p.bn_scale, p.bn_scale ? p.bn_shift : nullptr, p.Cout, A)) ||
            (rc = sd.upload(&A.in, p.in, (size_t)pix_in * p.Cin * 4)) || (rc = sd.upload(&A.in16, p.in16, (size_t)pix_in * p.Cin * 4)) ||
            (rc = sd.upload(&A.residual, p.residual, (size_t)rows_out * out_b)) || (rc = sd.upload(&A.up, p.up, (size_t)pix_up * out_b)) ||
            (rc = sd.upload(&A.mask, p.mask, (size_t)rows_out * out_b)) || (rc = sd.upload(&A.row_map, p.row_map, (size_t)rows_out * 4)) ||
            (rc = sd.upload(&A.dyn_rows, p.has_dyn ? p.dyn_rows : nullptr, (size_t)p.V * 4)) ||
            (rc = sd.upload(&A.gather, p.gather ? gs.data() : nullptr, gs.size() * sizeof(GatherSet))) ||
            (rc = sd.upload(&d_seg, seg.data(), seg.size() * sizeof(LevelSeg))) || (rc = sd.upload(&A.out, p.out, (size_t)p.out_n * 4)) ||
            (rc = sd.upload(&A.out16, p.out16, (size_t)p.out16_n * 4)) || (rc = sd.upload(&A.energy4, p.energy4, (size_t)p.energy4_n * 4))) return rc;
        if (p.head_out) {
            if (path != CONV_H4_GROUP || !p.head_w || !p.head_b || p.head_ld < 3 || p.head_out_n < rows_out * p.head_ld)
                return fail(CALD_ERR_INVALID, "cald_op_conv_probe: problem %d: head fields need path 9, head_w, head_b, head_ld >= 3 and a buffer of the output's rows", i);
            if ((rc = sd.upload(&A.head_w, p.head_w, (size_t)3 * p.Cout * 4)) || (rc = sd.upload(&A.head_out, p.head_out, (size_t)p.head_out_n * 4))) return rc;
            for (int q = 0; q < 3; q++) A.head_b[q] = p.head_b[q];
            A.head_ld = p.head_ld;
            back.push_back({A.head_out, p.head_out, (size_t)p.head_out_n * 4});
        }
        A.seg_in = d_seg; A.seg_out = d_seg + CALD_PROBE_MAX_VIEWS + 1; A.seg_up = d_seg + 2 * (CALD_PROBE_MAX_VIEWS + 1);
        if (p.out) back.push_back({A.out, p.out, (size_t)p.out_n * 4});
        if (p.out16) back.push_back({A.out16, p.out16, (size_t)p.out16_n * 4});
        if (p.energy4) back.push_back({A.energy4, p.energy4, (size_t)p.energy4_n * 4});
        A.ex16 = p.ex16 ? 1 : 0;
        A.V = p.V; A.Cin = p.Cin; A.Cout = p.Cout;
        A.KH = p.KH; A.KW = p.KW; A.stride = p.stride; A.pad = p.pad; A.relu = p.relu ? 1 : 0; A.in_relu = p.in_relu ? 1 : 0;
        A.total_mtiles = so[p.V].tile_start; A.out_ld = p.out_ld; A.zeros = c->d_zeros;
        if (p.row_packing < CALD_PROBE_PACK_AUTO || p.row_packing > CALD_PROBE_PACK_ON) return fail(CALD_ERR_INVALID, "cald_op_conv_probe: problem %d: bad row_packing", i);
        const bool packable = !p.has_dyn && !p.row_map && !p.gather && !p.mask && p.Cin != 4 && path != CONV_P4_FUSED;
        if (packable && (p.row_packing == CALD_PROBE_PACK_ON || (p.row_packing == CALD_PROBE_PACK_AUTO && conv_pack_default())))
            A.packed_rows = conv_pack_rows(si, so, p.up ? su : nullptr, p.V, p.Cin, p.out_ld);
        if (p.row_packing == CALD_PROBE_PACK_ON && !A.packed_rows) return fail(CALD_ERR_INVALID, "cald_op_conv_probe: problem %d cannot run on packed row tiles", i);
    }
    if (path == CONV_P4_FUSED) a[1].in = a[0].out;
    const ConvForce f{path, tile};
    const char* names[CALD_MAX_GROUP] = {nullptr};
    if (path == CONV_P4_FUSED) names[0] = names[1] = launch_conv_p4_fused(a[0], a[1], c->stream);
    else if (n > 1 || path == CONV_P4_GROUP || path == CONV_H3_GROUP || path == CONV_H4_GROUP) launch_conv_group(a, n, c->stream, names, f);
    else names[0] = launch_conv(a[0], c->stream, f);
    HIPCHK(hipGetLastError());
    HIPCHK(hipStreamSynchronize(c->stream));
    std::string all;
    for (int i = 0; i < n; i++) {
        if (!names[i]) return fail(CALD_ERR_UNSUPPORTED, "cald_op_conv_probe: problem %d refused under path %d tile %d", i, path, tile);
        if (all.find(names[i]) == std::string::npos) { if (!all.empty()) all += ";"; all += names[i]; }
    }
    for (const Back& b : back) HIPCHK(hipMemcpy(b.host, b.dev, b.bytes, hipMemcpyDeviceToHost));
    snprintf(kernel, (size_t)kernel_cap, "%s", all.c_str());
    return 0;
}
extern "C" int cald_op_row_pack_lookup(int V, const int* in_hw, const int* out_hw, int Cin, int out_ld, int64_t n, const int64_t* rows,
                                       int* view_out, int64_t* local_out, int64_t* packed_rows_out) {
    if (V < 1 || V > CALD_MAX_VIEWS || !in_hw || !out_hw || n < 0 || (n && (!rows || !view_out || !local_out)))
        return fail(CALD_ERR_INVALID, "cald_op_row_pack_lookup: bad arguments");
    std::vector<LevelSeg> si(V + 1), so(V + 1);
    memset(si.data(), 0, si.size() * sizeof(LevelSeg)); memset(so.data(), 0, so.size() * sizeof(LevelSeg));
    for (int v = 0; v < V; v++) {
        if (in_hw[2 * v] < 0 || in_hw[2 * v + 1] < 0 || out_hw[2 * v] < 0 || out_hw[2 * v + 1] < 0) return fail(CALD_ERR_INVALID, "cald_op_row_pack_lookup: negative size");
        si[v].H = in_hw[2 * v]; si[v].W = in_hw[2 * v + 1]; so[v].H = out_hw[2 * v]; so[v].W = out_hw[2 * v + 1];
        si[v + 1].pix_off = si[v].pix_off + (long long)si[v].H * si[v].W;
        so[v + 1].pix_off = so[v].pix_off + (long long)so[v].H * so[v].W;
    }
    for (int64_t i = 0; i < n; i++) {
        if (rows[i] < 0 || rows[i] >= so[V].pix_off) return fail(CALD_ERR_INVALID, "cald_op_row_pack_lookup: row %lld outside the level", (long long)rows[i]);
        const int v = seg_find_row(so.data(), V, rows[i]);
        view_out[i] = v; local_out[i] = rows[i] - so[v].pix_off;
    }
    if (packed_rows_out) *packed_rows_out = conv_pack_rows(si.data(), so.data(), nullptr, V, Cin, out_ld);
    return 0;
}
void launch_mfma_f16_probe(const unsigned short* A, const unsigned short* B, const unsigned* C, unsigned* D, long long n, hipStream_t stream);
extern "C" int cald_op_mfma_f16(cald_ctx* c, const uint16_t* A, const uint16_t* B, const uint32_t* C, uint32_t* D, int64_t n) {
    if (!c || !A || !B || !C || !D || n < 1) return fail(CALD_ERR_INVALID, "cald_op_mfma_f16: null argument or n < 1");
    HIPCHK(hipSetDevice(c->device));
    ScopedDev sd(c->stream);
    const unsigned short *dA, *dB; const unsigned* dC; unsigned* dD; int rc;
    if ((rc = sd.upload(&dA, A, (size_t)n * 32)) || (rc = sd.upload(&dB, B, (size_t)n * 32)) || (rc = sd.upload(&dC, C, (size_t)n * 4)) ||
        (rc = sd.alloc(&dD, (size_t)n * 4))) return rc;
    launch_mfma_f16_probe(dA, dB, dC, dD, (long long)n, c->stream);
    HIPCHK(hipGetLastError());
    HIPCHK(hipMemcpyAsync(D, dD, (size_t)n * 4, hipMemcpyDeviceToHost, c->stream));
    HIPCHK(hipStreamSynchronize(c->stream));
    return 0;
}
extern "C" int cald_op_conv2d_f16x3(cald_ctx* c, const float* in, int H, int W, int Cin, const float* weight, int Cout, int KH, int KW,
                                    int stride, int pad, const float* bias, const float* bn_scale, const float* bn_shift,
                                    const float* residual, int relu, float* out) {
    return op_conv2d(c, CALD_PRECISION_F16X3, in, H, W, Cin, weight, Cout, KH, KW, stride, pad, bias, bn_scale, bn_shift, residual, relu, out);
}

__global__ void fill_random_kernel(float* p, long long n, unsigned seed) {
    for (long long i = blockIdx.x * (long long)blockDim.x + threadIdx.x; i < n; i += (long long)gridDim.x * blockDim.x) {
        unsigned x = (unsigned)i * 2654435761u ^ seed; x ^= x >> 15; x *= 2246822519u; x ^= x >> 13; x *= 3266489917u; x ^= x >> 16;
        p[i] = ((float)(x >> 8) * (1.0f / 8388608.0f) - 1.0f) * ((x & 7u) ? 1.0f : 0.0f);
    }
}
extern "C" int cald_op_conv_bench(cald_ctx* c, int V, int H, int W, int Cin, int Cout, int KH, int stride, int pad, int residual,
                                  int relu, int iters, int group, double* ms_out, double* tflops_out) {
    if (!c || V < 1 || V > CALD_MAX_VIEWS || iters < 1 || !ms_out || group < 1 || group > CALD_MAX_GROUP) return fail(CALD_ERR_INVALID, "bad arguments");
    if (Cin % 4) return fail(CALD_ERR_INVALID, "Cin must be a multiple of 4");
    HIPCHK(hipSetDevice(c->device));
// ... 477 lines not shown
```

### cald_amd/csrc/sweep.hip

```cpp
#include "host.h"

void cald_host::free_det(DetBuffers& d) {
    hipFree(d.boxes); hipFree(d.scores); hipFree(d.labels); hipFree(d.props); hipFree(d.prob_max); hipFree(d.scores_cls); hipFree(d.count);
    memset(&d, 0, sizeof(d));
}
int cald_host::alloc_det(DetBuffers& d, int V, int cap, int C) {
    memset(&d, 0, sizeof(d));
    d.cap = cap; d.C = C;
    hipError_t e = hipMalloc((void**)&d.boxes, (size_t)V * cap * 16);
    if (e == hipSuccess) e = hipMalloc((void**)&d.scores, (size_t)V * cap * 4);
    if (e == hipSuccess) e = hipMalloc((void**)&d.labels, (size_t)V * cap * 8);
    if (e == hipSuccess) e = hipMalloc((void**)&d.props, (size_t)V * cap * 16);
    if (e == hipSuccess) e = hipMalloc((void**)&d.prob_max, (size_t)V * cap * 4);
    if (e == hipSuccess) e = hipMalloc((void**)&d.scores_cls, (size_t)V * cap * C * 4);
    if (e == hipSuccess) e = hipMalloc((void**)&d.count, (size_t)V * 4);
    if (e != hipSuccess) {
        free_det(d);
        return fail(CALD_ERR_HIP, "hipMalloc of detection buffers (%d views x %d rows x %d classes) failed: %s", V, cap, C, hipGetErrorString(e));
    }
    return 0;
}
static int ensure_det(cald_model* m, DetBuffers& set, int& views, int VT) {
    if (views >= VT) return 0;
    if (views) {
// ... 7 lines not shown
    return 0;
}
static DetBuffers det_at(const DetBuffers& D, size_t o) {
    DetBuffers d2 = D;
    const int cap = D.cap, C = D.C;
    d2.boxes += o * cap * 4; d2.scores += o * cap; d2.labels += o * cap; d2.props += o * cap * 4;
    d2.prob_max += o * cap; d2.scores_cls += o * cap * C; d2.count += o;
    return d2;
}
static ViewDesc plain_view(const uint8_t* src, int H, int W) {
    ViewDesc d; memset(&d, 0, sizeof(d));
    d.src = src; d.H = H; d.W = W;
    return d;
}
static std::vector<ViewDesc> ref_views(const uint8_t* const* images_dev, const int* H, const int* W, int i0, int nb) {
    std::vector<ViewDesc> views(nb);
    for (int i = 0; i < nb; i++) views[i] = plain_view(images_dev[i0 + i], H[i0 + i], W[i0 + i]);
    return views;
}

static int sweep_fwd_views() {
    static const int env = getenv("CALD_FWD_VIEWS") ? atoi(getenv("CALD_FWD_VIEWS")) : 96;
    return env < 1 ? 1 : (env > CALD_MAX_VIEWS ? CALD_MAX_VIEWS : env);
}
static int fwd_count(int n) { return (n + sweep_fwd_views() - 1) / sweep_fwd_views(); }
static void fwd_span(int n, int f, int* a0, int* nv) {
    const int n_fw = fwd_count(n);
    *a0 = (int)(((long long)n * f) / n_fw); *nv = (int)(((long long)n * (f + 1)) / n_fw) - *a0;
}
static bool cut_reuse_env() {
    static const bool on = !(getenv("CALD_CUTOUT_REUSE") && atoi(getenv("CALD_CUTOUT_REUSE")) == 0);
    return on;
}
#define CUT_GATHER_MAX_COST 0.7
#define CUT_FPN_MAX_COST CUT_GATHER_MAX_COST

namespace {
struct SweepBatch {
    int i0 = 0, nb = 0, P = 0, VV = 0; bool live = false;
    int* h_count; float* h_boxes; int* h_ints; float* h_par; NoiseJob* h_jobs; float* h_cons; float* h_clsc; float* h_vm; float* h_pm;
    std::vector<int> ref_n, pair_img, view_img, pair_aug, view_aug;
    std::vector<char> view_inert;
    std::vector<float> cut_margin;
    bool kept = false;
    bool kept_fpn = false;
    std::vector<int> ref_sel, pair_kind, view_isref;
    std::vector<float> pair_par;
    std::vector<ViewDesc> aviews;
};

struct SweepRun {
    cald_model* m; int n_images; const uint8_t* const* images_dev; const int* H; const int* W; const int64_t* pool_pos;
    const cald_sweep_cfg* cfg; double* consistency_out; double* cls_corr_out; float* margins_out; bool force_dense;
    cald_ctx* c = nullptr;
    bool audit = false, prune_ok = false, retina = false, reuse = false;
    int C = 0, cap = 0, A = 0, B = 0, VT = 0, NB = 0, P_MAX = 0, cut_a = -1;
    PairLayout lay{0, 0, 0}; size_t n_ints = 0;
    DetBuffers* DS[2] = {nullptr, nullptr};
    int* d_ints = nullptr; float *d_par = nullptr, *d_cons = nullptr, *d_clsc = nullptr; NoiseJob* d_jobs = nullptr; unsigned long long* d_lsum = nullptr;
    float *d_vm[2] = {nullptr, nullptr}, *d_pm = nullptr;
    SweepBatch bt[2];
    int nblk = 0, blk_lin[CUT_MAX_BLOCKS], blk_lout[CUT_MAX_BLOCKS], blk_stage[CUT_MAX_BLOCKS], blk_stride[CUT_MAX_BLOCKS];
    int ngeo = 0, geo_stride[CUT_MAX_BLOCKS], c_blk[4] = {0, 0, 0, 0};
    bool fpn_ok = false;
    std::vector<BatchPlan> rplan;

    static size_t al(size_t b) { return (b + 255) & ~(size_t)255; }

    int setup() {
        if (!m || !images_dev || !H || !W || !pool_pos || !cfg || !consistency_out || !cls_corr_out) return fail(CALD_ERR_INVALID, "null argument");
        audit = margins_out != nullptr;
        prune_ok = !audit && !force_dense;
        if (!m->finalized) return fail(CALD_ERR_STATE, "model not finalized");
        c = m->ctx;
        HIPCHK(hipSetDevice(c->device));
        C = m->cfg.num_classes; cap = m->det_cap();
        A = cfg->n_augs;
        if (A < 0 || A > CALD_MAX_AUGS) return fail(CALD_ERR_INVALID, "n_augs %d outside [0, %d]", A, CALD_MAX_AUGS);
        int n_noise = 0; bool any_gauss = false;
        for (int a = 0; a < A; a++) {
            const int k = cfg->augs[a].kind;
            if (k < CALD_AUG_FLIP || k > CALD_AUG_ROTATE) return fail(CALD_ERR_INVALID, "augmentation %d: unknown kind %d", a, k);
            if (k == CALD_AUG_CUTOUT && (cfg->augs[a].param < 1.0 || cfg->augs[a].param > (double)CALD_MAX_CUT))
                return fail(CALD_ERR_INVALID, "cutout: cut_num must be in [1, %d]", CALD_MAX_CUT);
            if (k == CALD_AUG_RESIZE && !(cfg->augs[a].param > 0.0)) return fail(CALD_ERR_INVALID, "resize: ratio must be positive");
            n_noise += (k == CALD_AUG_GAUSS || k == CALD_AUG_SALT_PEPPER);
            any_gauss |= k == CALD_AUG_GAUSS;
        }
        if (n_noise > CALD_MAX_NOISE_SEG) return fail(CALD_ERR_INVALID, "at most %d GaussianNoise / SaltPepperNoise views per image", CALD_MAX_NOISE_SEG);
        if (any_gauss)
            for (int i = 0; i < n_images; i++)
                if (randn_unsupported(H[i], W[i]))
                    return fail(CALD_ERR_UNSUPPORTED, "GaussianNoise on image %d (%dx%d): torch.randn of fewer than 16 elements takes torch's scalar path, which is not implemented", i, H[i], W[i]);
        B = cfg->batch_images > 0 ? cfg->batch_images : 64;
// ... 11 lines not shown
                                al(sizeof(unsigned long long) * P_MAX) + 2 * al((size_t)VT * CALD_VM * 4) + al((size_t)P_MAX * 2 * 4);
        const size_t pin_set = al((size_t)VT * 4) + al((size_t)B * cap * 16) + al(n_ints * 4) + al((size_t)P_MAX * 12 * 4) + al(sizeof(NoiseJob) * B) +
                               al((size_t)P_MAX * 4) + al((size_t)VT * (C - 1) * 4) + al((size_t)VT * CALD_VM * 4) + al((size_t)P_MAX * 2 * 4);
        if (dev_need > S.dev_bytes || 2 * pin_set > S.pin_bytes) {
            HIPCHK(hipStreamSynchronize(c->stream));
            if (S.dev) { hipFree(S.dev); S.dev = nullptr; S.dev_bytes = 0; }
            if (S.pin) { hipHostFree(S.pin); S.pin = nullptr; S.pin_bytes = 0; }
            HIPCHK(hipMalloc((void**)&S.dev, dev_need)); S.dev_bytes = dev_need;
            HIPCHK(hipHostMalloc((void**)&S.pin, 2 * pin_set)); S.pin_bytes = 2 * pin_set;
        }
        for (int i = 0; i < 2; i++) {
            if (!S.ev_ref[i]) HIPCHK(hipEventCreateWithFlags(&S.ev_ref[i], hipEventDisableTiming));
            if (!S.ev_score[i]) HIPCHK(hipEventCreateWithFlags(&S.ev_score[i], hipEventDisableTiming));
        }
        { Bump b(S.dev, false); d_ints = b.get<int>(n_ints); d_par = b.get<float>((size_t)P_MAX * 12); d_cons = b.get<float>(P_MAX);
          d_clsc = b.get<float>((size_t)VT * (C - 1)); d_jobs = b.get<NoiseJob>(B); d_lsum = b.get<unsigned long long>(P_MAX);
          d_vm[0] = b.get<float>((size_t)VT * CALD_VM); d_vm[1] = b.get<float>((size_t)VT * CALD_VM); d_pm = b.get<float>((size_t)P_MAX * 2); }
        for (int q = 0; q < 2; q++) {
            Bump b(S.pin + (size_t)q * pin_set, false);
            bt[q].h_count = b.get<int>(VT); bt[q].h_boxes = b.get<float>((size_t)B * cap * 4); bt[q].h_ints = b.get<int>(n_ints);
            bt[q].h_par = b.get<float>((size_t)P_MAX * 12); bt[q].h_jobs = b.get<NoiseJob>(B); bt[q].h_cons = b.get<float>(P_MAX);
            bt[q].h_clsc = b.get<float>((size_t)VT * (C - 1));
            bt[q].h_vm = b.get<float>((size_t)VT * CALD_VM); bt[q].h_pm = b.get<float>((size_t)P_MAX * 2);
        }
        if (m->prune && prune_ok) HIPCHK(hipMemsetAsync(c->d_prune_check, 0, 8, c->stream));
        for (int a = 0; a < A && cut_a < 0; a++) if (cfg->augs[a].kind == CALD_AUG_CUTOUT) cut_a = a;
        init_blocks();
        reuse = (m->cr.mode < 0 ? cut_reuse_env() : m->cr.mode != 0) && cut_a >= 0 && !audit && m->cfg.precision == CALD_PRECISION_FP32 && nblk < CUT_MAX_BLOCKS;
        rplan.resize(reuse ? 1 : 0);
        return 0;
    }
    void init_blocks() {
        retina = m->cfg.arch == CALD_ARCH_RETINANET;
        for (int b = 0, layer = 0, l = 2; b < (int)m->blocks.size() && layer < 3 && nblk < CUT_MAX_BLOCKS; b++) {
            const Bottleneck& Bk = m->blocks[b];
            blk_stride[nblk] = Bk.c2.stride; blk_lin[nblk] = l; l += Bk.c2.stride == 2 ? 1 : 0; blk_lout[nblk] = l; blk_stage[nblk] = layer;
            nblk++;
            if (Bk.layer_end) layer++;
        }
        {
            int layer = 0; bool fits = true;
            for (size_t b = 0; b < m->blocks.size(); b++) {
                if (ngeo == CUT_MAX_BLOCKS || layer > 3) { fits = false; break; }
                geo_stride[ngeo] = m->blocks[b].c2.stride;
                if (m->blocks[b].layer_end) c_blk[layer++] = ngeo;
                ngeo++;
            }
            fpn_ok = fits && layer == 4 && !retina && ngeo >= nblk;
            if (!fpn_ok) { ngeo = nblk; for (int b = 0; b < nblk; b++) geo_stride[b] = blk_stride[b]; }
        }
    }

    void plan_of(int nv, const ViewDesc* vs, BatchPlan& P) const {
        int hp[CALD_MAX_VIEWS][2];
        for (int v = 0; v < nv; v++) { int Hr, Wr; transform_size(vs[v].H, vs[v].W, m->cfg.min_size, m->cfg.max_size, &Hr, &Wr, &hp[v][0], &hp[v][1]); }
        build_plan(P, nv, vs, hp, retina);
    }
    size_t retain_layout(const BatchPlan& P, int nv, char* base, float** out) const {
        size_t off = 0;
        for (int b = 0; b < nblk; b++) {
            if (out) out[b] = reinterpret_cast<float*>(base + off);
            off += al((size_t)level_pix(P, blk_lout[b], nv) * (size_t)m->blocks[b].c3.Cout * 4);
        }
        return off;
    }
    size_t retain_layout_fpn(const BatchPlan& P, int nv, char* base, FwdReuse* ru) const {
        size_t off = retain_layout(P, nv, base, ru ? ru->out : nullptr);
        auto take = [&](size_t bytes) { char* p = base + off; off += al(bytes); return p; };
        for (int i = 0; i < 4; i++) { char* p = take((size_t)level_pix(P, 2 + i, nv) * 256 * 4); if (ru) ru->pf[i] = reinterpret_cast<float*>(p); }
        if (m->prune && prune_ok)
            for (int i = 0; i < 2; i++) {
                char* p = take((size_t)level_pix(P, 2 + i, nv) * 256 * 4); char* e = take((size_t)level_pix(P, 2 + i, nv) * 4 * 4);
                if (ru) { ru->p16[i] = reinterpret_cast<unsigned*>(p); ru->energy[i] = reinterpret_cast<float*>(e); }
            }
        if (ru) ru->fpn = true;
        return off;
    }

    int enqueue_ref(int k) {
        SweepBatch& b = bt[k & 1];
        b.i0 = k * B; b.nb = (n_images - b.i0 < B) ? n_images - b.i0 : B; b.live = true; b.P = 0; b.VV = b.nb;
        std::vector<ViewDesc> views = ref_views(images_dev, H, W, b.i0, b.nb);
        const DetBuffers& D = *DS[k & 1];
        FwdReuse ru;
        if (int r = retain(k, views.data(), ru)) return r;
        int r = forward_model(m, b.nb, views.data(), D, audit ? d_vm[k & 1] : nullptr, prune_ok, b.kept ? &ru : nullptr);
        if (r) return r;
        if (hipMemcpyAsync(b.h_count, D.count, (size_t)b.nb * 4, hipMemcpyDeviceToHost, c->stream) != hipSuccess ||
            hipMemcpyAsync(b.h_boxes, D.boxes, (size_t)b.nb * cap * 16, hipMemcpyDeviceToHost, c->stream) != hipSuccess ||
            hipEventRecord(m->ss.ev_ref[k & 1], c->stream) != hipSuccess) return fail(CALD_ERR_HIP, "D2H of reference detections failed");
        return 0;
    }
    int retain(int k, const ViewDesc* views, FwdReuse& ru) {
        SweepBatch& b = bt[k & 1];
        b.kept = b.kept_fpn = false;
        if (reuse) {
            plan_of(b.nb, views, rplan[0]);
            cald_model::CutReuse& R = m->cr;
            const int q = k & 1;
            const size_t need3 = retain_layout(rplan[0], b.nb, nullptr, nullptr), needx = fpn_ok ? retain_layout_fpn(rplan[0], b.nb, nullptr, nullptr) : 0;
            bool ext = fpn_ok && !R.ext_refused && !(R.ext_cap && needx > R.ext_cap);
            for (int attempt = 0; attempt < 2; attempt++) {
                const size_t need = ext ? needx : need3;
                if (need <= R.cap[q]) break;
                HIPCHK(hipStreamSynchronize(c->stream));
                if (R.slot[q]) hipFree(R.slot[q]);
                R.slot[q] = nullptr; R.cap[q] = 0;
                if (hipMalloc((void**)&R.slot[q], need + (need >> 3)) == hipSuccess) { R.cap[q] = need + (need >> 3); break; }
                (void)hipGetLastError(); R.slot[q] = nullptr;
                if (!ext) break;
                ext = false; R.ext_refused = true;
            }
            if (R.slot[q]) {
                ru.mode = 1; ru.nblk = nblk; b.kept = true; b.kept_fpn = ext;
                if (ext) retain_layout_fpn(rplan[0], b.nb, R.slot[q], &ru); else retain_layout(rplan[0], b.nb, R.slot[q], ru.out);
            } else c->cut_fallbacks++;
            c->cut_kept[!b.kept ? CUT_KEPT_NONE : b.kept_fpn ? CUT_KEPT_FPN : CUT_KEPT_STAGES]++;
        }
        return 0;
    }

    int build_aug_views(int k) {
        SweepBatch& b = bt[k & 1];
        cald_model::SweepScratch& S = m->ss;
        const int nb = b.nb, i0 = b.i0;
        if (hipEventSynchronize(S.ev_ref[k & 1]) != hipSuccess) return fail(CALD_ERR_HIP, "reference forward failed: %s", hipGetErrorString(hipGetLastError()));
        const int* h_count = b.h_count; const float* h_boxes = b.h_boxes;
        b.ref_sel.assign((size_t)B * 50, 0); b.pair_aug.clear(); b.pair_kind.clear(); b.view_isref.assign(VT, 0);
        b.ref_n.assign(B, 0); b.pair_img.clear(); b.view_img.assign(VT, 0); b.cut_margin.assign(B, INFINITY);
        b.view_aug.assign(VT, 0); b.view_inert.assign(VT, 0);
        b.pair_par.clear(); b.aviews.clear();
        int njobs = 0;
        size_t need = 0;
        for (int i = 0; i < nb; i++) {
            if (h_count[i] == 0) continue;
            const int Hi = H[i0 + i], Wi = W[i0 + i];
            for (int a = 0; a < A; a++) {
                const int kd = cfg->augs[a].kind; const double prm = cfg->augs[a].param;
                if (kd == CALD_AUG_SALT_PEPPER) need += al((size_t)Hi * Wi * 3);
                else if (kd == CALD_AUG_GAUSS) need += al((size_t)Hi * Wi * 3 * sizeof(float));
                else if (kd == CALD_AUG_COLOR_ADJUST) need += 2 * al((size_t)Hi * Wi * 3);
                else if (kd == CALD_AUG_RESIZE) {
                    const int ow = (int)((double)Wi * prm), oh = (int)((double)Hi * prm);
                    if (ow < 1 || oh < 1) return fail(CALD_ERR_INVALID, "resize ratio %g empties a %dx%d image", prm, Hi, Wi);
                    need += al((size_t)oh * ow * 3) + al((size_t)Hi * ow * 3);
                } else if (kd == CALD_AUG_ROTATE) {
                    int fx[6], nh, nw; pil_rotate_setup(Hi, Wi, prm, fx, &nh, &nw);
                    need += al((size_t)nh * nw * 3) + al((size_t)nh * Wi * 3) + al((size_t)Hi * Wi * 3);
// ... 52 lines not shown
                    ViewDesc v = base;
                    float cm = INFINITY;
                    v.nrect = cutout_rects(pyrng, Hi, Wi, b.ref_n[i], sub, (int)prm, v.rects, &cm);
                    if (cm < b.cut_margin[i]) b.cut_margin[i] = cm;
                    add_view(v, 0, nullptr);
                } else if (kd == CALD_AUG_RESIZE) {
                    const int ow = (int)((double)Wi * prm), oh = (int)((double)Hi * prm);
                    uint8_t* dst = take((size_t)oh * ow * 3); uint8_t* tmp = take((size_t)Hi * ow * 3);
                    if ((r = pil_resize(c, images_dev[i0 + i], Hi, Wi, dst, oh, ow, tmp, 0))) break;
                    pair_params(2, Hi, Wi, prm, par); add_view(plain_view(dst, oh, ow), 2, par);
                } else if (kd == CALD_AUG_ROTATE) {
                    int fx[6], nh, nw; pil_rotate_setup(Hi, Wi, prm, fx, &nh, &nw);
                    uint8_t* rot = take((size_t)nh * nw * 3); uint8_t* tmp = take((size_t)nh * Wi * 3); uint8_t* dst = take((size_t)Hi * Wi * 3);
                    launch_affine_nearest(images_dev[i0 + i], Hi, Wi, rot, nh, nw, fx, c->stream);
                    if ((r = pil_resize(c, rot, nh, nw, dst, Hi, Wi, tmp, 1))) break;
                    ViewDesc v = base; v.src = dst;
                    pair_params(3, Hi, Wi, prm, par);
                    add_view(v, 3, par);
                }
            }
            if (r) return r;
            if (nj.nseg) b.h_jobs[njobs++] = nj;
        }
        if (njobs) {
            if (hipMemcpyAsync(d_jobs, b.h_jobs, sizeof(NoiseJob) * njobs, hipMemcpyHostToDevice, c->stream) != hipSuccess) return fail(CALD_ERR_HIP, "H2D of noise jobs failed");
            launch_noise_stream(d_jobs, njobs, c->stream);
        }
        return 0;
    }

    int cut_plan(int k, int V, const ViewDesc* vs, FwdReuse& ru) {
        cald_model::CutReuse& R = m->cr;
        const bool fpn = bt[k & 1].kept_fpn;
        const size_t per = cut_plan_set_bytes(V), total = per * (2 * (size_t)nblk + (fpn ? 4 : 0));
        if (!R.d_gp) {
            const size_t cap = cut_plan_set_bytes(CALD_MAX_VIEWS) * (2 * CUT_MAX_BLOCKS + 4);
            HIPCHK(hipMalloc((void**)&R.d_gp, cap));
            HIPCHK(hipHostMalloc((void**)&R.h_gp[0], cap)); HIPCHK(hipHostMalloc((void**)&R.h_gp[1], cap));
        }
        plan_of(V, vs, rplan[0]);
        const BatchPlan& P = rplan[0];
        char* const h = R.h_gp[k & 1];
        std::vector<CutSet> g_out((size_t)V * ngeo), g_t1((size_t)V * ngeo), g_fpn((size_t)V * 4);
        for (int v = 0; v < V; v++) {
            int Hr, Wr, Hp, Wp; CutSet pool1;
            transform_size(vs[v].H, vs[v].W, m->cfg.min_size, m->cfg.max_size, &Hr, &Wr, &Hp, &Wp);
            cut_geometry(vs[v].H, vs[v].W, Hr, Wr, Hp, Wp, vs[v].nrect, vs[v].rects, ngeo, geo_stride, &pool1, &g_out[(size_t)v * ngeo], &g_t1[(size_t)v * ngeo]);
            if (fpn) {
                CutSet cs[4], inner[4];
                for (int i = 0; i < 4; i++) cs[i] = g_out[(size_t)v * ngeo + c_blk[i]];
                cut_fpn_geometry(Hp, Wp, cs, inner, &g_fpn[(size_t)v * 4]);
            }
        }
        auto put_set = [&](size_t index, int lvl, const CutSet* sets, size_t stride_v, int* tiles_out, double* rows_out) {
            LevelSeg* sg = reinterpret_cast<LevelSeg*>(h + index * per);
            GatherSet* gs = reinterpret_cast<GatherSet*>(reinterpret_cast<char*>(sg) + (size_t)(V + 1) * sizeof(LevelSeg));
            int tiles = 0; double rows = 0.0;
            for (int v = 0; v < V; v++) {
                LevelSeg L = P.seg[lvl][v]; L.tile_start = tiles; sg[v] = L;
                CutRect rr[CALD_GATHER_RECTS];
                int n = cut_disjoint(sets[(size_t)v * stride_v], rr, CALD_GATHER_RECTS);
                if (n < 0) { n = 1; rr[0] = {0, 0, L.W - 1, L.H - 1}; }
                GatherSet& G = gs[v]; memset(&G, 0, sizeof(G));
                G.nr = n;
                for (int q = 0; q < n; q++) {
                    G.x0[q] = rr[q].x0; G.y0[q] = rr[q].y0; G.w[q] = rr[q].x1 - rr[q].x0 + 1;
                    G.cum[q + 1] = G.cum[q] + G.w[q] * (rr[q].y1 - rr[q].y0 + 1);
                }
                tiles += (G.cum[n] + 127) / 128; rows += (double)G.cum[n];
            }
            sg[V] = P.seg[lvl][V]; sg[V].tile_start = tiles;
            *tiles_out = tiles; *rows_out = rows;
        };
        auto kf = [](const ConvLayer& L) { return (double)L.Cout * (double)(L.KH * L.KW * L.CinTrue); };
        double cost_g[3] = {0, 0, 0}, cost_d[3] = {0, 0, 0}, rows_g[3] = {0, 0, 0}, rows_d[3] = {0, 0, 0}, tiles_g[3] = {0, 0, 0}, tiles_d[3] = {0, 0, 0};
        for (int b = 0; b < nblk; b++)
            for (int kind = 0; kind < 2; kind++) {
                const int lvl = kind ? blk_lin[b] : blk_lout[b];
                int tiles; double rows;
                put_set((size_t)(2 * b + kind), lvl, (kind ? g_t1.data() : g_out.data()) + b, (size_t)ngeo, &tiles, &rows);
                ru.tiles[b][kind] = tiles; ru.rows[b][kind] = rows;
                const Bottleneck& Bk = m->blocks[b];
                const double w = kind ? kf(Bk.c1) : kf(Bk.c2) + kf(Bk.c3) + (Bk.has_down ? kf(Bk.down) : 0.0);
                const double nconv = kind ? 1.0 : (Bk.has_down ? 3.0 : 2.0), dense = (double)level_pix(P, lvl, V);
                const int st = blk_stage[b];
                cost_g[st] += 128.0 * tiles * w; cost_d[st] += dense * w;
                rows_g[st] += rows * nconv; rows_d[st] += dense * nconv;
                tiles_g[st] += tiles * nconv; tiles_d[st] += (double)P.seg[lvl][V].tile_start * nconv;
            }
        for (int st = 0; st < 3; st++) {
            ru.gather[st] = m->cr.mode != 2 && cost_g[st] <= CUT_GATHER_MAX_COST * cost_d[st];
            c->cut_rows[st] += ru.gather[st] ? rows_g[st] : rows_d[st]; c->cut_dense[st] += rows_d[st];
            c->cut_st_rows[st] += ru.gather[st] ? rows_g[st] : rows_d[st]; c->cut_st_dense[st] += rows_d[st];
            c->cut_st_tiles[st] += ru.gather[st] ? tiles_g[st] : tiles_d[st]; c->cut_st_dense_tiles[st] += tiles_d[st];
        }
        {
            double r4 = 0.0, t4 = 0.0, rl = 0.0, tl = 0.0;
            int lvl = 2;
            for (size_t b = 0; b < m->blocks.size(); b++) {
                const Bottleneck& Bk = m->blocks[b];
                const int lo = lvl + (Bk.c2.stride == 2 ? 1 : 0);
                if ((int)b >= nblk) {
                    const double n_in = 1.0, n_out = Bk.has_down ? 3.0 : 2.0;
                    r4 += n_in * (double)level_pix(P, lvl, V) + n_out * (double)level_pix(P, lo, V);
                    t4 += n_in * (double)P.seg[lvl][V].tile_start + n_out * (double)P.seg[lo][V].tile_start;
                }
                lvl = lo;
            }
            if (!retina) for (int i = 0; i < 4; i++) { rl += (double)level_pix(P, 2 + i, V); tl += (double)P.seg[2 + i][V].tile_start; }
            c->cut_st_rows[3] += r4; c->cut_st_dense[3] += r4; c->cut_st_tiles[3] += t4; c->cut_st_dense_tiles[3] += t4;
            c->cut_st_rows[CUT_STAGE_LATERAL] += rl; c->cut_st_dense[CUT_STAGE_LATERAL] += rl;
            c->cut_st_tiles[CUT_STAGE_LATERAL] += tl; c->cut_st_dense_tiles[CUT_STAGE_LATERAL] += tl;
            double fg = 0.0, fd = 0.0, frg = 0.0, frd = 0.0;
            if (fpn)
                for (int i = 0; i < 4; i++) {
                    put_set(2 * (size_t)nblk + i, 2 + i, g_fpn.data() + i, 4, &ru.fpn_tiles[i], &ru.fpn_rows[i]);
                    fg += ru.fpn_tiles[i]; frg += ru.fpn_rows[i];
                }
            if (!retina) for (int i = 0; i < 4; i++) { fd += (double)P.seg[2 + i][V].tile_start; frd += (double)level_pix(P, 2 + i, V); }
            ru.gather_fpn = fpn && m->cr.mode != 2 && 128.0 * fg <= CUT_FPN_MAX_COST * frd;
            c->cut_st_rows[CUT_STAGE_OUTPUT] += ru.gather_fpn ? frg : frd; c->cut_st_dense[CUT_STAGE_OUTPUT] += frd;
            c->cut_st_tiles[CUT_STAGE_OUTPUT] += ru.gather_fpn ? fg : fd; c->cut_st_dense_tiles[CUT_STAGE_OUTPUT] += fd;
        }
        if (hipMemcpyAsync(R.d_gp, h, total, hipMemcpyHostToDevice, c->stream) != hipSuccess) return fail(CALD_ERR_HIP, "H2D of the cut_out gather plan failed");
        ru.mode = 2; ru.nblk = nblk; ru.d_gp = R.d_gp;
        if (fpn) retain_layout_fpn(P, V, m->cr.slot[k & 1], &ru); else retain_layout(P, V, m->cr.slot[k & 1], ru.out);
        c->cut_batches++;
        return 0;
    }

    int enqueue_aug_forwards(int k) {
        SweepBatch& b = bt[k & 1];
        const DetBuffers& D = *DS[k & 1];
        const int nb = b.nb, na = (int)b.aviews.size();
        int r, n_rest = na, rest_slot = nb;
        ViewDesc* rest_views = b.aviews.data();
        std::vector<ViewDesc> rest;
        int n_cut = 0;
        for (int j = 0; j < na; j++) n_cut += b.view_aug[nb + j] == cut_a;
        b.VV = nb + na;
        if (b.kept && n_cut > 0 && 2 * nb + (na - n_cut) <= VT) {
            std::vector<ViewDesc> cutv(nb);
            std::vector<int> slot(na), nimg(VT, 0), naug(VT, 0);
            std::vector<char> has(nb, 0), ninert(VT, 0);
            for (int i = 0; i < nb; i++) nimg[i] = i;
            int nr2 = 0;
            for (int j = 0; j < na; j++) {
                const int img = b.view_img[nb + j];
                if (b.view_aug[nb + j] == cut_a) { slot[j] = nb + img; cutv[img] = b.aviews[j]; has[img] = 1; }
                else { slot[j] = 2 * nb + nr2++; rest.push_back(b.aviews[j]); }
                nimg[slot[j]] = img; naug[slot[j]] = b.view_aug[nb + j];
            }
            for (int i = 0; i < nb; i++)
                if (!has[i]) {
                    cutv[i] = plain_view(images_dev[b.i0 + i], H[b.i0 + i], W[b.i0 + i]);
                    nimg[nb + i] = i; naug[nb + i] = cut_a; ninert[nb + i] = 1;
                }
            for (size_t p = 0; p < b.pair_aug.size(); p++) b.pair_aug[p] = slot[b.pair_aug[p] - nb];
            b.view_img = nimg; b.view_aug = naug; b.view_inert = ninert;
// ... 376 lines not shown
```

### cald_amd/csrc/train_geom.hip

```cpp
#include "train_host.h"
#include <map>
#include <mutex>
#include <tuple>

static std::mutex g_seg_stage_mu;
static std::map<std::tuple<cald_ctx*, int, int, int>, LevelSeg*> g_seg;
static bool g_seg_evict = false;
static size_t seg_cache_cap() {
    static const size_t cap = [] { const char* e = getenv("CALD_SEG_CACHE_CAP"); const long v = e ? atol(e) : 0; return (size_t)(v > 0 ? v : 1024); }();
    return cap;
}
int cald_train_host::seg_entry() {
    std::lock_guard<std::mutex> lk(g_seg_stage_mu);
    if (!g_seg_evict) return 0;
    THIP(hipDeviceSynchronize());
    for (auto& kv : g_seg) hipFree(kv.second);
    g_seg.clear();
    g_seg_evict = false;
    return 0;
}
int cald_train_host::dense_seg(cald_ctx* c, int N, int H, int W, const LevelSeg** out) {
    std::lock_guard<std::mutex> lk(g_seg_stage_mu);
    auto key = std::make_tuple(c, N, H, W);
    auto it = g_seg.find(key);
    if (it == g_seg.end()) {
        if (g_seg.size() >= seg_cache_cap()) g_seg_evict = true;
        std::vector<LevelSeg> h(N + 1);
        const int tiles = (H * W + 127) / 128;
        for (int v = 0; v <= N; v++) { h[v].pix_off = (long long)v * H * W; h[v].H = H; h[v].W = W; h[v].tile_start = v * tiles; h[v].pad_ = 0; }
        LevelSeg* d = nullptr;
        THIP(hipMalloc((void**)&d, sizeof(LevelSeg) * (N + 1)));
        THIP(hipMemcpy(d, h.data(), sizeof(LevelSeg) * (N + 1), hipMemcpyHostToDevice));
        it = g_seg.emplace(key, d).first;
    }
    *out = it->second;
    return 0;
}

struct StageRing { char* host; char* dev; hipEvent_t ev[8]; bool used[8]; int next; };
static std::map<cald_ctx*, StageRing> g_stage;
int cald_train_host::stage_upload(cald_ctx* c, const void* src, size_t bytes, hipStream_t st, const void** dev_out, int* slot_out) {
    if (bytes > kStageSlot) TFAIL(CALD_ERR_INVALID, "staging slot too small");
    std::lock_guard<std::mutex> lk(g_seg_stage_mu);
    auto it = g_stage.find(c);
    if (it == g_stage.end()) {
        StageRing r; memset(&r, 0, sizeof(r));
        THIP(hipHostMalloc((void**)&r.host, kStageSlot * 8, hipHostMallocDefault));
        THIP(hipMalloc((void**)&r.dev, kStageSlot * 8));
        for (int i = 0; i < 8; i++) THIP(hipEventCreateWithFlags(&r.ev[i], hipEventDisableTiming));
        it = g_stage.emplace(c, r).first;
    }
    StageRing& r = it->second;
    const int s = r.next; r.next = (s + 1) & 7;
    if (r.used[s]) THIP(hipEventSynchronize(r.ev[s]));
    memcpy(r.host + kStageSlot * s, src, bytes);
    THIP(hipMemcpyAsync(r.dev + kStageSlot * s, r.host + kStageSlot * s, bytes, hipMemcpyHostToDevice, st));
    *dev_out = r.dev + kStageSlot * s; *slot_out = s;
    return 0;
}
int cald_train_host::stage_consumed(cald_ctx* c, int slot, hipStream_t st) {
    std::lock_guard<std::mutex> lk(g_seg_stage_mu);
    StageRing& r = g_stage[c];
// ... 19 lines not shown
```

### cald_amd/csrc/vaal.hip

```cpp
#include "host.h"

#define VAAL_SIDE 256
#define VAAL_PIX (VAAL_SIDE * VAAL_SIDE)
#define VAAL_LAYERS 5
#define VAAL_Z 256
#define VAAL_FC_K 65536
#define VAAL_FC_SEG 256
#define VAAL_FC_NSEG (VAAL_FC_K / VAAL_FC_SEG)
#define VAAL_FC_TILE 16
#define VAAL_HID 512
#define BN_CHUNK 256
#define BN_EPS 1e-5f

__global__ __launch_bounds__(256) void vaal_resize_kernel(const VaalImage* __restrict__ imgs, float4* __restrict__ out) {
    const int i = blockIdx.x * 256 + threadIdx.x, dy = i >> 8, dx = i & (VAAL_SIDE - 1);
    const VaalImage im = imgs[blockIdx.y];
    int sy = (int)(((long long)dy * im.H) >> 8), sx = (int)(((long long)dx * im.W) >> 8);
    if (sy > im.H - 1) sy = im.H - 1;
    if (sx > im.W - 1) sx = im.W - 1;
    const uint8_t* p = im.src + ((size_t)sy * im.W + sx) * 3;
    out[(size_t)blockIdx.y * VAAL_PIX + i] = make_float4((float)p[0], (float)p[1], (float)p[2], 0.0f);
}

template <bool VAR>
// ... 230 lines not shown
    for (int j = 0; j < VAAL_HID; j++) {
        for (int k = 0; k < VAAL_Z; k++) w1t[(size_t)k * VAAL_HID + j] = w1->data[(size_t)j * VAAL_Z + k];
        for (int k = 0; k < VAAL_HID; k++) w2t[(size_t)k * VAAL_HID + j] = w2->data[(size_t)j * VAAL_HID + k];
    }
    if ((rc = vaal_upload(v, w1t, &v->w1t)) || (rc = vaal_upload(v, b1->data, &v->b1)) || (rc = vaal_upload(v, w2t, &v->w2t)) ||
        (rc = vaal_upload(v, b2->data, &v->b2)) || (rc = vaal_upload(v, w3->data, &v->w3))) return rc;
    v->b3 = b3->data[0];
    return 0;
}
extern "C" int cald_vaal_finalize(cald_vaal* v) {
    if (!v) return fail(CALD_ERR_INVALID, "null argument");
    if (v->finalized) return 0;
    HIPCHK(hipSetDevice(v->ctx->device));
    const int rc = vaal_finalize(v);
    if (rc) { v->release(); return rc; }
    v->sd.clear();
    v->finalized = true;
    return 0;
}
extern "C" int cald_vaal_destroy(cald_vaal* v) {
    if (!v) return 0;
    hipStreamSynchronize(v->ctx->stream);
    v->release();
    delete v;
    return 0;
}

static void vaal_fill_seg(std::vector<LevelSeg>& seg, int cap) {
    seg.assign((size_t)(VAAL_LAYERS + 1) * (cap + 1), LevelSeg());
    for (int l = 0; l <= VAAL_LAYERS; l++) {
        const int side = VAAL_SIDE >> l, pix = kLevelPix[l], tiles = (pix + 127) / 128;
        for (int i = 0; i <= cap; i++) {
            LevelSeg& s = seg[(size_t)l * (cap + 1) + i];
            s.pix_off = (long long)i * pix; s.H = side; s.W = side; s.tile_start = i * tiles; s.pad_ = 0;
        }
    }
}

extern "C" int cald_sweep_vaal(cald_ctx* c, cald_vaal* v, int n_images, const uint8_t* const* images_dev, const int* H, const int* W,
                               const cald_vaal_cfg* cfg, float* preds_out, float* mu_out) {
    if (!c || !v || !images_dev || !H || !W || !preds_out || n_images < 0) return fail(CALD_ERR_INVALID, "null argument");
    if (!v->finalized) return fail(CALD_ERR_STATE, "VAAL model not finalized (call cald_vaal_finalize)");
    if (v->ctx != c) return fail(CALD_ERR_INVALID, "the VAAL model belongs to another context");
    const int mode = cfg ? cfg->bn_mode : CALD_VAAL_BN_BATCH;
    if (mode != CALD_VAAL_BN_BATCH && mode != CALD_VAAL_BN_RUNNING) return fail(CALD_ERR_INVALID, "bn_mode %d is not a CALD_VAAL_BN_* value", mode);
    int B = cfg && cfg->batch_images > 0 ? cfg->batch_images : 64; if (B > CALD_MAX_VIEWS) B = CALD_MAX_VIEWS;
    if (B > n_images) B = n_images;
    for (int i = 0; i < n_images; i++)
        if (!images_dev[i] || H[i] < 1 || W[i] < 1 || (long long)H[i] * W[i] > (1ll << 28)) return fail(CALD_ERR_INVALID, "image %d is malformed", i);
    if (!n_images) return 0;
    HIPCHK(hipSetDevice(c->device));
    ScopedDev sd(c->stream);
    VaalImage* d_imgs = nullptr; LevelSeg* d_seg = nullptr;
    float* act[VAAL_LAYERS + 1] = {};
    float *d_part = nullptr, *d_mean = nullptr, *d_istd = nullptr, *d_fcp = nullptr, *d_mu = nullptr, *d_pred = nullptr;
    int rc;
    std::vector<LevelSeg> seg; vaal_fill_seg(seg, B);
    if ((rc = sd.alloc(&d_imgs, (size_t)B * sizeof(VaalImage))) || (rc = sd.upload(&d_seg, seg.data(), seg.size() * sizeof(LevelSeg)))) return rc;
    for (int l = 0; l <= VAAL_LAYERS; l++)
        if ((rc = sd.alloc(&act[l], (size_t)B * kLevelPix[l] * (l ? kCout[l - 1] : 4) * 4))) return rc;
    if ((rc = sd.alloc(&d_part, (size_t)B * 4096 * 4)) || (rc = sd.alloc(&d_mean, (size_t)B * 1024 * 4)) || (rc = sd.alloc(&d_istd, (size_t)B * 1024 * 4)) ||
        (rc = sd.alloc(&d_fcp, (size_t)B * VAAL_FC_NSEG * VAAL_Z * 4)) || (rc = sd.alloc(&d_mu, (size_t)B * VAAL_Z * 4)) || (rc = sd.alloc(&d_pred, (size_t)B * 4))) return rc;
    std::vector<VaalImage> h_imgs(B);
    for (int i0 = 0; i0 < n_images; i0 += B) {
        const int nb = n_images - i0 < B ? n_images - i0 : B;
        for (int i = 0; i < nb; i++) { h_imgs[i].src = images_dev[i0 + i]; h_imgs[i].H = H[i0 + i]; h_imgs[i].W = W[i0 + i]; }
        HIPCHK(hipMemcpyAsync(d_imgs, h_imgs.data(), (size_t)nb * sizeof(VaalImage), hipMemcpyHostToDevice, c->stream));
// ... 89 lines not shown
```

### include/cald_hip.h

```cpp
#ifndef CALD_HIP_H
#define CALD_HIP_H
#include <stddef.h>
#include <stdint.h>
#ifdef __cplusplus
extern "C" {
#endif

typedef struct cald_ctx cald_ctx;
typedef struct cald_model cald_model;

#define CALD_OK 0
#define CALD_ERR_INVALID (-1)
#define CALD_ERR_HIP (-2)
#define CALD_ERR_STATE (-3)
#define CALD_ERR_MISSING_WEIGHT (-4)
#define CALD_ERR_UNSUPPORTED (-5)

#define CALD_PRECISION_FP32 0
#define CALD_PRECISION_F16X3 1

#define CALD_ARCH_FRCNN 0
#define CALD_ARCH_RETINANET 1

const char* cald_last_error(void);
// ... 253 lines not shown
    int in_hw[CALD_PROBE_MAX_VIEWS][2];
    int up_hw[CALD_PROBE_MAX_VIEWS][2];
    int dyn_rows[CALD_PROBE_MAX_VIEWS];
    int has_dyn;
    int gather;
    int nrect[CALD_PROBE_MAX_VIEWS];
    int rect[CALD_PROBE_MAX_VIEWS][CALD_PROBE_MAX_RECTS][4];
    int Cin, Cout, KH, KW, stride, pad, relu, in_relu, out_ld;
    int cin_true;
    const float* weight;
    const float* bias;
    const float* bn_scale;
    const float* bn_shift;
    const float* in;
    const uint32_t* in16;
    const float* residual;
    const float* up;
    int ex16;
    const float* mask;
    const int* row_map;
    float* out; int64_t out_n;
    uint32_t* out16; int64_t out16_n;
    float* energy4; int64_t energy4_n;
    const float* head_w; const float* head_b;
    float* head_out; int64_t head_out_n; int head_ld;
    int row_packing;
} cald_conv_probe;
#define CALD_PROBE_PACK_AUTO 0
#define CALD_PROBE_PACK_OFF 1
#define CALD_PROBE_PACK_ON 2
int cald_op_conv_probe(cald_ctx* ctx, int precision, cald_conv_probe* probs, int n, int path, int tile, char* kernel, int kernel_cap);
int cald_op_row_pack_lookup(int V, const int* in_hw, const int* out_hw, int Cin, int out_ld, int64_t n, const int64_t* rows,
                            int* view_out, int64_t* local_out, int64_t* packed_rows_out);
int cald_op_mfma_f16(cald_ctx* ctx, const uint16_t* A, const uint16_t* B, const uint32_t* C, uint32_t* D, int64_t n);
int cald_op_conv_bench(cald_ctx* ctx, int n_views, int H, int W, int Cin, int Cout, int KH, int stride, int pad, int residual,
                       int relu, int iters, int group, double* ms_out, double* tflops_out);
int cald_op_transform_size(int H, int W, int min_size, int max_size, int* Hr, int* Wr, int* Hp, int* Wp);
int cald_debug_tensor(cald_model* m, const char* name, int view, float* host_out, int64_t capacity, int64_t* shape3);

#define CALD_JPEG_BASELINE 0
#define CALD_JPEG_GPU_EXTENDED 1
#define CALD_JPEG_HOST_ONLY 2
int cald_jpeg_info(const uint8_t* data, size_t size, int* H, int* W, int* ncomp);
int cald_jpeg_decode_batch(cald_ctx* ctx, int n, const uint8_t* const* data, const size_t* sizes, uint8_t* const* out_dev);
int cald_jpeg_probe(const uint8_t* data, size_t size, int* H, int* W, int* ncomp, int* kind);
int cald_jpeg_decode_batch_any(cald_ctx* ctx, int n, const uint8_t* const* data, const size_t* sizes, uint8_t* const* out_dev);
int cald_jpeg_decode_host(const uint8_t* data, size_t size, uint8_t* out_host);

int cald_profile_enable(cald_ctx* ctx, int on);
int cald_profile_read(cald_ctx* ctx, double* gemm_ms, double* gemm_flops, int64_t* gemm_launches, double* total_ms);
int cald_profile_prune(cald_ctx* ctx, double* lookahead_ms, double* lookahead_flops, double* selected_fraction_p2_p3, double* worst_bound_ratio,
                       double* pruned_flops);
int cald_profile_prune_fallbacks(cald_ctx* ctx, int64_t* n);
int cald_model_set_cutout_reuse(cald_model* m, int mode, int* was);
int cald_model_set_look_fuse(cald_model* m, int mode, int* was);
int cald_model_set_row_packing(cald_model* m, int mode, int* was);
int cald_model_set_box_min_size(cald_model* m, float min_size, float* was);
int cald_profile_cutout(cald_ctx* ctx, double* rows3, double* dense_rows3, int64_t* batches, int64_t* fallbacks);
int cald_profile_cutout_stages(cald_ctx* ctx, double* rows6, double* dense_rows6, double* tiles6, double* dense_tiles6, int64_t* kept3);
int cald_model_set_cutout_retention_cap(cald_model* m, int64_t bytes, int64_t* was);
int cald_debug_cutout_forward(cald_model* m, int n_views, const cald_view* views, const cald_dets* out, int prune);
int cald_profile_roi_rows(cald_ctx* ctx, double* mean_rows_per_view, int64_t* views);
int cald_profile_dump(cald_ctx* ctx, const char* path);

int cald_train_packed_floats(int Cout, int Cin, int KH, int KW, int CinK, int mode, int64_t* floats_out);
int cald_train_pack_conv(cald_ctx* ctx, const float* weight, const float* bias, const float* bn_scale, const float* bn_shift,
                         int Cout, int Cin, int KH, int KW, int CinK, int mode, float* packed);
typedef struct cald_pack_job {
    const float *weight, *bias, *bn_scale, *bn_shift;
    int Cout, Cin, KH, KW, CinK, mode;
    float* packed;
} cald_pack_job;
typedef struct cald_pack_plan cald_pack_plan;
int cald_train_pack_plan_scratch_floats(int n, const cald_pack_job* jobs, int64_t* floats_out);
int cald_train_pack_plan_create(cald_ctx* ctx, int n, const cald_pack_job* jobs, float* scratch, int64_t scratch_floats, cald_pack_plan** plan_out);
int cald_train_pack_plan_run(cald_ctx* ctx, const cald_pack_plan* plan);
int cald_train_pack_plan_destroy(cald_pack_plan* plan);
int cald_train_conv(cald_ctx* ctx, int N, int H, int W, const float* in, int CinK, const float* packed, int Cout, int Cin,
                    int KH, int KW, int stride, int pad, int mode, int flags, const float* residual, const float* up,
                    int Hup, int Wup, const float* mask, float* out, int out_ld);
int cald_train_conv_group(cald_ctx* ctx, int n, int N, const int* hw, const float* const* ins, int CinK, const float* const* packed,
                          int Cout, int Cin, int KH, int KW, int stride, int pad, int mode, int flags, const float* const* masks,
                          float* const* outs, int out_ld);
int cald_train_conv_wgrad(cald_ctx* ctx, int N, int H, int W, const float* x, int Cin, int ldx, const float* g, int Cout, int ldg,
                          int KH, int KW, int stride, int pad, const float* row_scale, float* dw, float* db, int accumulate);
int cald_train_linear_wgrad(cald_ctx* ctx, int R, const float* x, int K, const float* g, int Cout, int ldg, int taps,
                            float* dw, float* db, int accumulate);
enum { CALD_WGRAD_POINTWISE = 0, CALD_WGRAD_TABLE = 1, CALD_WGRAD_GENERAL = 2, CALD_WGRAD_GENERAL32 = 3, CALD_WGRAD_WIDE = 4 };
enum { CALD_WGRAD_REDUCE_FLAT = 0, CALD_WGRAD_REDUCE_TAPS = 1 };
typedef struct cald_wgrad_plan {
    int variant, reduce;
    int MT, JT;
// ... 70 lines not shown
```

Measured before the change: 181.4.

## Pack gathered cutout rows across views and extend gather reuse to layer4

```diff
diff --git a/cald_amd/_ffi.py b/cald_amd/_ffi.py
--- a/cald_amd/_ffi.py
+++ b/cald_amd/_ffi.py
@@ -200,6 +200,7 @@
                                        C.c_int, c_f, c_f, c_f, c_f, C.c_int, c_f]),
     "cald_op_conv_bench": (C.c_int, [C.c_void_p] + [C.c_int] * 12 + [c_d, c_d]),
     "cald_op_row_pack_lookup": (C.c_int, [C.c_int, c_i, c_i, C.c_int, C.c_int, C.c_int64, c_i64, c_i, c_i64, c_i64]),
+    "cald_op_gather_pack_lookup": (C.c_int, [C.c_int, c_i, c_i, c_i, c_i, C.c_int, C.c_int, C.c_int64, c_i64, c_i, c_i64, c_i64, c_i64]),
     "cald_op_transform_size": (C.c_int, [C.c_int, C.c_int, C.c_int, C.c_int, c_i, c_i, c_i, c_i]),
     "cald_debug_tensor": (C.c_int, [C.c_void_p, C.c_char_p, C.c_int, c_f, C.c_int64, c_i64]),
     "cald_jpeg_info": (C.c_int, [C.c_void_p, C.c_size_t, c_i, c_i, c_i]),
@@ -214,10 +215,13 @@
     "cald_profile_cutout": (C.c_int, [C.c_void_p, c_d, c_d, c_i64, c_i64]),
     "cald_model_set_cutout_reuse": (C.c_int, [C.c_void_p, C.c_int, c_i]),
     "cald_profile_cutout_stages": (C.c_int, [C.c_void_p, c_d, c_d, c_d, c_d, c_i64]),
+    "cald_profile_cutout_gather": (C.c_int, [C.c_void_p, c_d, c_d, c_d]),
     "cald_model_set_cutout_retention_cap": (C.c_int, [C.c_void_p, C.c_int64, c_i64]),
     "cald_op_cutout_fpn_geometry": (C.c_int, [C.c_int, C.c_int, C.c_int, C.c_int, C.c_int, c_i, C.c_int, c_i, c_i]),
     "cald_model_set_look_fuse": (C.c_int, [C.c_void_p, C.c_int, c_i]),
     "cald_model_set_row_packing": (C.c_int, [C.c_void_p, C.c_int, c_i]),
+    "cald_model_set_gather_packing": (C.c_int, [C.c_void_p, C.c_int, c_i]),
+    "cald_model_set_cutout_layer4": (C.c_int, [C.c_void_p, C.c_int, c_i]),
     "cald_model_set_box_min_size": (C.c_int, [C.c_void_p, C.c_float, c_f]),
     "cald_profile_dump": (C.c_int, [C.c_void_p, C.c_char_p]),
     "cald_train_packed_floats": (C.c_int, [C.c_int] * 6 + [c_i64]),
diff --git a/cald_amd/csrc/common.h b/cald_amd/csrc/common.h
--- a/cald_amd/csrc/common.h
+++ b/cald_amd/csrc/common.h
@@ -12,7 +12,7 @@
     long long pix_off;
     int H, W;
     int tile_start;
-    int pad_;
+    int row_start;
 };
 
 #if defined(__HIPCC__)
@@ -29,6 +29,14 @@
     while (lo < hi) {
         const int mid = (lo + hi + 1) >> 1;
         if (seg[mid].pix_off <= row) lo = mid; else hi = mid - 1;
+    }
+    return lo;
+}
+__host__ __device__ __forceinline__ int seg_find_grow(const LevelSeg* __restrict__ seg, const int V, const int row) {
+    int lo = 0, hi = V - 1;
+    while (lo < hi) {
+        const int mid = (lo + hi + 1) >> 1;
+        if (seg[mid].row_start <= row) lo = mid; else hi = mid - 1;
     }
     return lo;
 }
@@ -51,6 +59,22 @@
     return (int)total;
 }
 
+static inline int gather_pack_rows(const LevelSeg* si, const LevelSeg* so, const LevelSeg* su, int V, int Cin, int out_ld) {
+    const long long total = V < 1 ? 0 : so[V].row_start, LIM = 0x7FFE0000LL - (1 << 16);
+    if (total < 1 || total > 0x7FFFFFFFLL - 128) return 0;
+    int vf = 0, vl = 0;
+    for (long long t0 = 0; t0 < total; t0 += 128) {
+        const long long last = (t0 + 127 < total ? t0 + 127 : total - 1);
+        while (so[vf + 1].row_start <= t0) vf++;
+        if (vl < vf) vl = vf;
+        while (so[vl + 1].row_start <= last) vl++;
+        if (vl == vf) continue;
+        if ((si[vl + 1].pix_off - si[vf].pix_off) * Cin * 4 > LIM || (so[vl + 1].pix_off - so[vf].pix_off) * out_ld * 4 > LIM) return 0;
+        if (su && (su[vl + 1].pix_off - su[vf].pix_off) * out_ld * 4 > LIM) return 0;
+    }
+    return (int)total;
+}
+
 struct BatchPlan {
     LevelSeg seg[CALD_MAX_LEVELS][CALD_MAX_VIEWS + 1];
 };
@@ -61,7 +85,7 @@
     int cum[CALD_GATHER_RECTS + 1];
     int x0[CALD_GATHER_RECTS], y0[CALD_GATHER_RECTS], w[CALD_GATHER_RECTS];
 };
-__device__ __forceinline__ int gather_pixel(const GatherSet& g, const int m, const int W) {
+__host__ __device__ __forceinline__ int gather_pixel(const GatherSet& g, const int m, const int W) {
     int k = 0;
     while (k + 1 < g.nr && m >= g.cum[k + 1]) k++;
     const int j = m - g.cum[k], w = g.w[k], ry = j / w;
diff --git a/cald_amd/csrc/conv_p4.hip b/cald_amd/csrc/conv_p4.hip
--- a/cald_amd/csrc/conv_p4.hip
+++ b/cald_amd/csrc/conv_p4.hip
@@ -30,7 +30,8 @@
     constexpr bool has_mask = MASK;
     const float* __restrict__ mask_v = has_mask ? a.mask + so.pix_off * (long long)out_ld : out_v;
     const int row_b = out_ld * 4;
-    const unsigned long long vb64 = (unsigned long long)(GATHER ? Ho * Wo : Mv) * (unsigned)row_b;
+    const long long span = GATHER ? (straddle ? a.seg_out[a.V].pix_off - so.pix_off : (long long)Ho * Wo) : (long long)Mv;
+    const unsigned long long vb64 = (unsigned long long)span * (unsigned)row_b;
     const unsigned valid_b = vb64 < 0x7FFE0000ull ? (unsigned)vb64 : 0x7FFE0000u;
     const __amdgpu_buffer_rsrc_t rsO = __builtin_amdgcn_make_buffer_rsrc((void*)out_v, 0, valid_b, 0x00020000);
     const __amdgpu_buffer_rsrc_t rsX = __builtin_amdgcn_make_buffer_rsrc((void*)(EPI != 0 ? ex_v : out_v), 0, EPI == 1 ? valid_b : 0x7FFE0000, 0x00020000);
@@ -42,7 +43,17 @@
         if (tid < BM) {
             int m = m0 + tid;
             if (GATHER) {
-                s_src[tid] = m < Mv ? gather_pixel(a.gather[v], m, Wo) * row_b : 0x7FFF0000;
+                int off = 0x7FFF0000;
+                if (m < Mv) {
+                    if (straddle) {
+                        const int r = so.row_start + m;
+                        int vr = v;
+                        while (vr + 1 < a.V && a.seg_out[vr + 1].row_start <= r) vr++;
+                        const LevelSeg sor = a.seg_out[vr];
+                        off = ((int)(sor.pix_off - so.pix_off) + gather_pixel(a.gather[vr], r - sor.row_start, sor.W)) * row_b;
+                    } else off = gather_pixel(a.gather[v], m, Wo) * row_b;
+                }
+                s_src[tid] = off;
             } else if (EPI == 2 && straddle) {
                 int src = 0;
                 if (m < Mv) {
@@ -261,9 +272,9 @@
         else { const int r = b - MT8 * NT; mt = MT8 + r / NT; nt = r % NT; }
     }
     const int n0 = nt * BN;
-    constexpr bool CAN_PACK = !C4 && !MASK && !FUSE && !GATHER;
+    constexpr bool CAN_PACK = !C4 && !MASK && !FUSE;
     const bool packed = CAN_PACK && a.packed_rows != 0;
-    const int v = packed ? seg_find_row(a.seg_out, a.V, (long long)mt * BM) : seg_find_view(a.seg_out, a.V, mt);
+    const int v = !packed ? seg_find_view(a.seg_out, a.V, mt) : GATHER ? seg_find_grow(a.seg_out, a.V, mt * BM) : seg_find_row(a.seg_out, a.V, (long long)mt * BM);
     const LevelSeg so = a.seg_out[v];
     const LevelSeg si = a.seg_in[v];
     const int Ho = so.H, Wo = so.W, Hi = si.H, Wi = si.W;
@@ -274,7 +285,7 @@
     bool straddle = false;
     if (CAN_PACK && packed) {
         const int row0 = mt * BM, left = a.packed_rows - row0;
-        m0 = row0 - (int)so.pix_off;
+        m0 = row0 - (GATHER ? so.row_start : (int)so.pix_off);
         const int end = m0 + (left < BM ? left : BM);
         straddle = end > Mv;
         Mv = end;
@@ -291,15 +302,14 @@
 #pragma unroll
     for (int p = 0; p < 2; p++) {
         const int m = m0 + arow + 64 * p;
-        int ml = m, Wo_r = Wo, Hi_r = Hi, Wi_r = Wi, dpix = 0;
+        int ml = m, Wo_r = Wo, Hi_r = Hi, Wi_r = Wi, dpix = 0, vr = v;
         if (CAN_PACK && straddle && m < Mv) {
-            const long long r = so.pix_off + m;
-            int vr = v;
-            while (vr + 1 < a.V && a.seg_out[vr + 1].pix_off <= r) vr++;
+            const long long r = (GATHER ? (long long)so.row_start : so.pix_off) + m;
+            while (vr + 1 < a.V && (GATHER ? (long long)a.seg_out[vr + 1].row_start : a.seg_out[vr + 1].pix_off) <= r) vr++;
             const LevelSeg sor = a.seg_out[vr], sir = a.seg_in[vr];
-            ml = (int)(r - sor.pix_off); Wo_r = sor.W; Hi_r = sir.H; Wi_r = sir.W; dpix = (int)(sir.pix_off - si.pix_off);
-        }
-        const int mp = GATHER ? (m < Mv ? gather_pixel(a.gather[v], m, Wo) : 0) : (a.row_map && m < Mv) ? a.row_map[so.pix_off + m] : ml;
+            ml = (int)(r - (GATHER ? (long long)sor.row_start : sor.pix_off)); Wo_r = sor.W; Hi_r = sir.H; Wi_r = sir.W; dpix = (int)(sir.pix_off - si.pix_off);
+        }
+        const int mp = GATHER ? (m < Mv ? gather_pixel(a.gather[vr], ml, Wo_r) : 0) : (a.row_map && m < Mv) ? a.row_map[so.pix_off + m] : ml;
         const int oy = mp / Wo_r, ox = mp - oy * Wo_r;
         const int iy0 = oy * a.stride - a.pad, ix0 = ox * a.stride - a.pad;
         unsigned msk = 0;
@@ -710,7 +720,7 @@
 }
 
 static inline ConvArgs p4_tiled(ConvArgs a) {
-    if (a.packed_rows > 0 && a.Cin != 4 && !a.dyn_rows && !a.row_map && !a.gather && !a.mask) a.total_mtiles = (a.packed_rows + 127) / 128;
+    if (a.packed_rows > 0 && a.Cin != 4 && !a.dyn_rows && !a.row_map && !a.mask) a.total_mtiles = (a.packed_rows + 127) / 128;
     else a.packed_rows = 0;
     return a;
 }
diff --git a/cald_amd/csrc/ctx.hip b/cald_amd/csrc/ctx.hip
--- a/cald_amd/csrc/ctx.hip
+++ b/cald_amd/csrc/ctx.hip
@@ -185,6 +185,16 @@
     return 0;
 }
 
+extern "C" int cald_profile_cutout_gather(cald_ctx* c, double* rows6, double* view_tiles6, double* packed_tiles6) {
+    if (!c) return fail(CALD_ERR_INVALID, "ctx is null");
+    for (int i = 0; i < 6; i++) {
+        if (rows6) rows6[i] = c->cut_gp_rows[i];
+        if (view_tiles6) view_tiles6[i] = c->cut_gp_view_tiles[i];
+        if (packed_tiles6) packed_tiles6[i] = c->cut_gp_packed_tiles[i];
+    }
+    return 0;
+}
+
 extern "C" int cald_profile_dump(cald_ctx* c, const char* path) {
     if (!c || !path) return fail(CALD_ERR_INVALID, "null argument");
     HIPCHK(hipStreamSynchronize(c->stream));
@@ -242,7 +252,8 @@
     ProfLaunch t; int rc;
     if ((rc = prof_begin(c, t))) return rc;
     const char* k = launch_conv(a, c->stream);
-    if ((rc = prof_end(c, t, flops, c->prof_tag_now, "mt=%d,Cin=%d,Cout=%d,k=%dx%d,s=%d", a.total_mtiles, a.Cin, a.Cout, a.KH, a.KW, a.stride))) return rc;
+    if ((rc = prof_end(c, t, flops, c->prof_tag_now, "mt=%d,Cin=%d,Cout=%d,k=%dx%d,s=%d%s", a.total_mtiles, a.Cin, a.Cout, a.KH, a.KW, a.stride,
+                       a.gather ? ",gathered-rows" : ""))) return rc;
     if (!k) return conv_refused(a);
     return 0;
 }
diff --git a/cald_amd/csrc/forward.hip b/cald_amd/csrc/forward.hip
--- a/cald_amd/csrc/forward.hip
+++ b/cald_amd/csrc/forward.hip
@@ -313,6 +313,16 @@
     return 0;
 }
 
+bool cald_host::gather_pack_default() {
+    static const bool on = !(getenv("CALD_GATHER_PACK") && atoi(getenv("CALD_GATHER_PACK")) == 0);
+    return on;
+}
+static void offer_gather_packing(cald_model* m, ConvArgs& a, const FwdReuse& ru, size_t set, int lin, int V) {
+    if (!ru.pack || !ru.h_gp) return;
+    const LevelSeg* so = reinterpret_cast<const LevelSeg*>(ru.h_gp + set * cut_plan_set_bytes(V));
+    a.packed_rows = gather_pack_rows(m->plan.seg[lin], so, nullptr, V, a.Cin, a.out_ld);
+    if (a.packed_rows) a.total_mtiles = (a.packed_rows + 127) / 128;
+}
 static int gconv_on(cald_model* m, const ConvLayer& L, const float* in, float* out, int lin, int lout, int V, bool relu, const float* residual,
                     const FwdReuse& ru, int b, int kind) {
     if (!ru.tiles[b][kind]) return 0;
@@ -323,6 +333,7 @@
     a.seg_out = reinterpret_cast<const LevelSeg*>(base);
     a.gather = reinterpret_cast<const GatherSet*>(base + (size_t)(V + 1) * sizeof(LevelSeg));
     a.total_mtiles = ru.tiles[b][kind];
+    offer_gather_packing(m, a, ru, (size_t)(2 * b + kind), lin, V);
     return run_conv(m->ctx, a, 2.0 * ru.rows[b][kind] * (double)L.Cout * (double)(L.KH * L.KW * L.CinTrue));
 }
 
@@ -337,7 +348,8 @@
         a[i].gather = reinterpret_cast<const GatherSet*>(base + (size_t)(V + 1) * sizeof(LevelSeg));
         a[i].total_mtiles = ru.fpn_tiles[i];
         a[i].out16 = sp[i].out16; a[i].energy4 = sp[i].energy4;
-        flops += 2.0 * ru.fpn_rows[i] * (double)sp[i].L->Cout * (double)(sp[i].L->KH * sp[i].L->KW * sp[i].L->CinTrue); tiles += ru.fpn_tiles[i];
+        if (ru.fpn_tiles[i]) offer_gather_packing(m, a[i], ru, 2 * (size_t)ru.nblk + i, sp[i].level, V);
+        flops += 2.0 * ru.fpn_rows[i] * (double)sp[i].L->Cout * (double)(sp[i].L->KH * sp[i].L->KW * sp[i].L->CinTrue); tiles += a[i].total_mtiles;
     }
     if (!tiles) return 0;
     cald_ctx* c = m->ctx;
@@ -453,7 +465,7 @@
         m->dbg["conv1"] = {Fb.c1, 1, 64, 0};
         launch_maxpool(Fb.c1, Fb.p1, dp->seg[1], dp->seg[2], 64, V, max_pix2, st, m->split.count(Fb.p1) != 0);
         m->dbg["pool1"] = {Fb.p1, 2, 64, 0};
-        const float* cur = Fb.p1; int lvl = 2, layer = 0, xi = 0;
+        const float* cur = Fb.p1; int lvl = 2, layer = 0, xi = 0, n4 = 0;
         for (size_t b = 0; b < m->blocks.size(); b++) {
             const Bottleneck& B = m->blocks[b];
             const int lout = lvl + (B.c2.stride == 2 ? 1 : 0);
@@ -461,6 +473,7 @@
             float* dst = kept ? ru->out[b] : (B.layer_end ? Fb.Cf[layer] : Fb.X[xi]);
             if ((rc = kept && ru->mode == 2 && ru->gather[layer] ? gathered_block(B, (int)b, cur, dst, lvl, lout) : dense_block(B, cur, dst, lvl, lout))) return rc;
             if (B.layer_end) Fb.Cf[layer] = dst;
+            if (layer == 3) m->dbg["layer4." + std::to_string(n4++)] = {dst, lout, B.c3.Cout, 0};
             cur = dst; lvl = lout;
             if (B.layer_end) layer++; else xi ^= 1;
         }
diff --git a/cald_amd/csrc/host.h b/cald_amd/csrc/host.h
--- a/cald_amd/csrc/host.h
+++ b/cald_amd/csrc/host.h
@@ -59,6 +59,7 @@
     double cut_rows[3] = {0.0, 0.0, 0.0}, cut_dense[3] = {0.0, 0.0, 0.0};
     long long cut_batches = 0, cut_fallbacks = 0;
     double cut_st_rows[6] = {}, cut_st_dense[6] = {}, cut_st_tiles[6] = {}, cut_st_dense_tiles[6] = {};
+    double cut_gp_rows[6] = {}, cut_gp_view_tiles[6] = {}, cut_gp_packed_tiles[6] = {};
     long long cut_kept[3] = {0, 0, 0};
 };
 
@@ -116,6 +117,7 @@
     bool prune_allowed = false;
     int look_fuse = 1; float* look_head_w = nullptr; float look_head_b[3] = {0, 0, 0};
     int row_packing = -1;
+    int gather_packing = -1;
     bool prune_bound_voided = false;
     bool prune_capture = false;
     ConvLayer p6, p7, cls_tower[4], reg_tower[4], cls_out, reg_out;
@@ -138,6 +140,7 @@
     int key_cap = 32768;
     struct CutReuse {
         int mode = -1;
+        int layer4 = -1;
         char* slot[2] = {nullptr, nullptr}; size_t cap[2] = {0, 0};
         bool ext_refused = false;
         size_t ext_cap = 0;
@@ -164,8 +167,10 @@
     int mode = 0;
     int nblk = 0;
     float* out[CUT_MAX_BLOCKS] = {};
-    bool gather[3] = {false, false, false};
+    bool gather[4] = {false, false, false, false};
     const char* d_gp = nullptr;
+    const char* h_gp = nullptr;
+    bool pack = false;
     int tiles[CUT_MAX_BLOCKS][2] = {};
     double rows[CUT_MAX_BLOCKS][2] = {};
     bool fpn = false, gather_fpn = false;
@@ -229,6 +234,7 @@
 void build_plan(BatchPlan& P, int V, const ViewDesc* views, const int (*hp)[2], bool retina);
 bool stem_grid_exact(const LevelSeg* seg, int V);
 bool conv_pack_default();
+bool gather_pack_default();
 int forward_model(cald_model* m, int V, ViewDesc* views, const DetBuffers& det, float* audit_out = nullptr, bool prune_ok = false,
                   const FwdReuse* ru = nullptr, FwdFeatures* feat = nullptr, FwdSsm* ssm = nullptr, FwdRetinaSsm* rssm = nullptr);
 void free_det(DetBuffers& d);
diff --git a/cald_amd/csrc/lossnet.hip b/cald_amd/csrc/lossnet.hip
--- a/cald_amd/csrc/lossnet.hip
+++ b/cald_amd/csrc/lossnet.hip
@@ -220,7 +220,7 @@
     const int i = blockIdx.x * blockDim.x + threadIdx.x;
     if (i >= 4 * N) return;
     const int l = i / N, n = i % N, H = g.H[l], W = g.W[l];
-    LevelSeg s; s.pix_off = (long long)n * H * W; s.H = H; s.W = W; s.tile_start = n * ((H * W + 127) / 128); s.pad_ = 0;
+    LevelSeg s; s.pix_off = (long long)n * H * W; s.H = H; s.W = W; s.tile_start = n * ((H * W + 127) / 128); s.row_start = 0;
     seg[i] = s;
 }
 
diff --git a/cald_amd/csrc/model.hip b/cald_amd/csrc/model.hip
--- a/cald_amd/csrc/model.hip
+++ b/cald_amd/csrc/model.hip
@@ -315,7 +315,7 @@
     return 0;
 }
 extern "C" int cald_model_set_cutout_reuse(cald_model* m, int mode, int* was) {
-    if (!m || mode < -1 || mode > 2) return fail(CALD_ERR_INVALID, "bad argument");
+    if (!m || mode < -1 || mode > 3) return fail(CALD_ERR_INVALID, "bad argument");
     if (was) *was = m->cr.mode;
     m->cr.mode = mode;
     return 0;
@@ -330,6 +330,18 @@
     if (!m || mode < -1 || mode > 1) return fail(CALD_ERR_INVALID, "bad argument");
     if (was) *was = m->row_packing;
     m->row_packing = mode;
+    return 0;
+}
+extern "C" int cald_model_set_gather_packing(cald_model* m, int mode, int* was) {
+    if (!m || mode < -1 || mode > 1) return fail(CALD_ERR_INVALID, "bad argument");
+    if (was) *was = m->gather_packing;
+    m->gather_packing = mode;
+    return 0;
+}
+extern "C" int cald_model_set_cutout_layer4(cald_model* m, int mode, int* was) {
+    if (!m || mode < -1 || mode > 1) return fail(CALD_ERR_INVALID, "bad argument");
+    if (was) *was = m->cr.layer4;
+    m->cr.layer4 = mode;
     return 0;
 }
 extern "C" int cald_model_set_look_fuse(cald_model* m, int mode, int* was) {
diff --git a/cald_amd/csrc/ops.hip b/cald_amd/csrc/ops.hip
--- a/cald_amd/csrc/ops.hip
+++ b/cald_amd/csrc/ops.hip
@@ -252,6 +252,7 @@
             so[v + 1].pix_off = so[v].pix_off + (long long)Ho * Wo;
             su[v + 1].pix_off = su[v].pix_off + (long long)su[v].H * su[v].W;
             so[v + 1].tile_start = so[v].tile_start + (int)((m + 127) / 128);
+            if (p.gather) so[v + 1].row_start = so[v].row_start + (int)m;
             si[v + 1].tile_start = si[v].tile_start + (H * W + 127) / 128;
             rows_out = so[v + 1].pix_off;
         }
@@ -294,6 +295,9 @@
         const bool packable = !p.has_dyn && !p.row_map && !p.gather && !p.mask && p.Cin != 4 && path != CONV_P4_FUSED;
         if (packable && (p.row_packing == CALD_PROBE_PACK_ON || (p.row_packing == CALD_PROBE_PACK_AUTO && conv_pack_default())))
             A.packed_rows = conv_pack_rows(si, so, p.up ? su : nullptr, p.V, p.Cin, p.out_ld);
+        const bool gpackable = p.gather && !p.has_dyn && !p.row_map && !p.mask && p.Cin != 4 && path != CONV_P4_FUSED;
+        if (gpackable && (p.row_packing == CALD_PROBE_PACK_ON || (p.row_packing == CALD_PROBE_PACK_AUTO && gather_pack_default())))
+            A.packed_rows = gather_pack_rows(si, so, p.up ? su : nullptr, p.V, p.Cin, p.out_ld);
         if (p.row_packing == CALD_PROBE_PACK_ON && !A.packed_rows) return fail(CALD_ERR_INVALID, "cald_op_conv_probe: problem %d cannot run on packed row tiles", i);
     }
     if (path == CONV_P4_FUSED) a[1].in = a[0].out;
@@ -331,6 +335,40 @@
         view_out[i] = v; local_out[i] = rows[i] - so[v].pix_off;
     }
     if (packed_rows_out) *packed_rows_out = conv_pack_rows(si.data(), so.data(), nullptr, V, Cin, out_ld);
+    return 0;
+}
+extern "C" int cald_op_gather_pack_lookup(int V, const int* in_hw, const int* out_hw, const int* nrect, const int* rect, int Cin, int out_ld, int64_t n,
+                                          const int64_t* rows, int* view_out, int64_t* local_out, int64_t* pixel_out, int64_t* packed_rows_out) {
+    if (V < 1 || V > CALD_MAX_VIEWS || !in_hw || !out_hw || !nrect || !rect || n < 0 || (n && (!rows || !view_out || !local_out || !pixel_out)))
+        return fail(CALD_ERR_INVALID, "cald_op_gather_pack_lookup: bad arguments");
+    std::vector<LevelSeg> si(V + 1), so(V + 1);
+    std::vector<GatherSet> gs(V);
+    memset(si.data(), 0, si.size() * sizeof(LevelSeg)); memset(so.data(), 0, so.size() * sizeof(LevelSeg));
+    memset(gs.data(), 0, gs.size() * sizeof(GatherSet));
+    for (int v = 0; v < V; v++) {
+        if (in_hw[2 * v] < 0 || in_hw[2 * v + 1] < 0 || out_hw[2 * v] < 0 || out_hw[2 * v + 1] < 0) return fail(CALD_ERR_INVALID, "cald_op_gather_pack_lookup: negative size");
+        si[v].H = in_hw[2 * v]; si[v].W = in_hw[2 * v + 1]; so[v].H = out_hw[2 * v]; so[v].W = out_hw[2 * v + 1];
+        GatherSet& g = gs[v];
+        if (nrect[v] < 0 || nrect[v] > CALD_GATHER_RECTS) return fail(CALD_ERR_INVALID, "cald_op_gather_pack_lookup: 0..%d rectangles", CALD_GATHER_RECTS);
+        g.nr = nrect[v];
+        for (int k = 0; k < g.nr; k++) {
+            const int* r = rect + ((size_t)v * CALD_GATHER_RECTS + k) * 4;
+            if (r[0] < 0 || r[1] < 0 || r[2] < 1 || r[3] < 1 || r[0] + r[2] > so[v].W || r[1] + r[3] > so[v].H)
+                return fail(CALD_ERR_INVALID, "cald_op_gather_pack_lookup: rectangle outside view %d", v);
+            g.x0[k] = r[0]; g.y0[k] = r[1]; g.w[k] = r[2]; g.cum[k + 1] = g.cum[k] + r[2] * r[3];
+        }
+        si[v + 1].pix_off = si[v].pix_off + (long long)si[v].H * si[v].W;
+        so[v + 1].pix_off = so[v].pix_off + (long long)so[v].H * so[v].W;
+        if ((long long)so[v].row_start + g.cum[g.nr] > 0x7FFFFFFFLL) return fail(CALD_ERR_INVALID, "cald_op_gather_pack_lookup: too many rows");
+        so[v + 1].row_start = so[v].row_start + g.cum[g.nr];
+    }
+    for (int64_t i = 0; i < n; i++) {
+        if (rows[i] < 0 || rows[i] >= so[V].row_start) return fail(CALD_ERR_INVALID, "cald_op_gather_pack_lookup: row %lld outside the launch", (long long)rows[i]);
+        const int v = seg_find_grow(so.data(), V, (int)rows[i]);
+        view_out[i] = v; local_out[i] = rows[i] - so[v].row_start;
+        pixel_out[i] = gather_pixel(gs[v], (int)local_out[i], so[v].W);
+    }
+    if (packed_rows_out) *packed_rows_out = gather_pack_rows(si.data(), so.data(), nullptr, V, Cin, out_ld);
     return 0;
 }
 void launch_mfma_f16_probe(const unsigned short* A, const unsigned short* B, const unsigned* C, unsigned* D, long long n, hipStream_t stream);
diff --git a/cald_amd/csrc/sweep.hip b/cald_amd/csrc/sweep.hip
--- a/cald_amd/csrc/sweep.hip
+++ b/cald_amd/csrc/sweep.hip
@@ -63,6 +63,10 @@
     static const bool on = !(getenv("CALD_CUTOUT_REUSE") && atoi(getenv("CALD_CUTOUT_REUSE")) == 0);
     return on;
 }
+static bool cut_layer4_env() {
+    static const bool on = !(getenv("CALD_CUTOUT_LAYER4") && atoi(getenv("CALD_CUTOUT_LAYER4")) == 0);
+    return on;
+}
 #define CUT_GATHER_MAX_COST 0.7
 #define CUT_FPN_MAX_COST CUT_GATHER_MAX_COST
 
@@ -91,6 +95,7 @@
     int* d_ints = nullptr; float *d_par = nullptr, *d_cons = nullptr, *d_clsc = nullptr; NoiseJob* d_jobs = nullptr; unsigned long long* d_lsum = nullptr;
     float *d_vm[2] = {nullptr, nullptr}, *d_pm = nullptr;
     SweepBatch bt[2];
+    int nblk4 = 0, nblkx = 0;
     int nblk = 0, blk_lin[CUT_MAX_BLOCKS], blk_lout[CUT_MAX_BLOCKS], blk_stage[CUT_MAX_BLOCKS], blk_stride[CUT_MAX_BLOCKS];
     int ngeo = 0, geo_stride[CUT_MAX_BLOCKS], c_blk[4] = {0, 0, 0, 0};
     bool fpn_ok = false;
@@ -168,11 +173,13 @@
     }
     void init_blocks() {
         retina = m->cfg.arch == CALD_ARCH_RETINANET;
-        for (int b = 0, layer = 0, l = 2; b < (int)m->blocks.size() && layer < 3 && nblk < CUT_MAX_BLOCKS; b++) {
+        int nall = 0; bool three = false;
+        for (int b = 0, layer = 0, l = 2; b < (int)m->blocks.size() && layer < 4 && nall < CUT_MAX_BLOCKS; b++) {
             const Bottleneck& Bk = m->blocks[b];
-            blk_stride[nblk] = Bk.c2.stride; blk_lin[nblk] = l; l += Bk.c2.stride == 2 ? 1 : 0; blk_lout[nblk] = l; blk_stage[nblk] = layer;
-            nblk++;
-            if (Bk.layer_end) layer++;
+            blk_stride[nall] = Bk.c2.stride; blk_lin[nall] = l; l += Bk.c2.stride == 2 ? 1 : 0; blk_lout[nall] = l; blk_stage[nall] = layer;
+            nall++;
+            if (!three) nblk = nall;
+            if (Bk.layer_end) { layer++; three |= layer == 3; if (layer == 4) nblk4 = nall; }
         }
         {
             int layer = 0; bool fits = true;
@@ -185,6 +192,8 @@
             fpn_ok = fits && layer == 4 && !retina && ngeo >= nblk;
             if (!fpn_ok) { ngeo = nblk; for (int b = 0; b < nblk; b++) geo_stride[b] = blk_stride[b]; }
         }
+        const bool l4 = fpn_ok && nblk4 > nblk && nblk4 <= ngeo && (m->cr.layer4 < 0 ? cut_layer4_env() : m->cr.layer4 != 0);
+        nblkx = l4 ? nblk4 : nblk;
     }
 
     void plan_of(int nv, const ViewDesc* vs, BatchPlan& P) const {
@@ -192,16 +201,16 @@
         for (int v = 0; v < nv; v++) { int Hr, Wr; transform_size(vs[v].H, vs[v].W, m->cfg.min_size, m->cfg.max_size, &Hr, &Wr, &hp[v][0], &hp[v][1]); }
         build_plan(P, nv, vs, hp, retina);
     }
-    size_t retain_layout(const BatchPlan& P, int nv, char* base, float** out) const {
+    size_t retain_layout(const BatchPlan& P, int nv, char* base, float** out, int nb) const {
         size_t off = 0;
-        for (int b = 0; b < nblk; b++) {
+        for (int b = 0; b < nb; b++) {
             if (out) out[b] = reinterpret_cast<float*>(base + off);
             off += al((size_t)level_pix(P, blk_lout[b], nv) * (size_t)m->blocks[b].c3.Cout * 4);
         }
         return off;
     }
     size_t retain_layout_fpn(const BatchPlan& P, int nv, char* base, FwdReuse* ru) const {
-        size_t off = retain_layout(P, nv, base, ru ? ru->out : nullptr);
+        size_t off = retain_layout(P, nv, base, ru ? ru->out : nullptr, nblkx);
         auto take = [&](size_t bytes) { char* p = base + off; off += al(bytes); return p; };
         for (int i = 0; i < 4; i++) { char* p = take((size_t)level_pix(P, 2 + i, nv) * 256 * 4); if (ru) ru->pf[i] = reinterpret_cast<float*>(p); }
         if (m->prune && prune_ok)
@@ -234,7 +243,7 @@
             plan_of(b.nb, views, rplan[0]);
             cald_model::CutReuse& R = m->cr;
             const int q = k & 1;
-            const size_t need3 = retain_layout(rplan[0], b.nb, nullptr, nullptr), needx = fpn_ok ? retain_layout_fpn(rplan[0], b.nb, nullptr, nullptr) : 0;
+            const size_t need3 = retain_layout(rplan[0], b.nb, nullptr, nullptr, nblk), needx = fpn_ok ? retain_layout_fpn(rplan[0], b.nb, nullptr, nullptr) : 0;
             bool ext = fpn_ok && !R.ext_refused && !(R.ext_cap && needx > R.ext_cap);
             for (int attempt = 0; attempt < 2; attempt++) {
                 const size_t need = ext ? needx : need3;
@@ -248,8 +257,8 @@
                 ext = false; R.ext_refused = true;
             }
             if (R.slot[q]) {
-                ru.mode = 1; ru.nblk = nblk; b.kept = true; b.kept_fpn = ext;
-                if (ext) retain_layout_fpn(rplan[0], b.nb, R.slot[q], &ru); else retain_layout(rplan[0], b.nb, R.slot[q], ru.out);
+                ru.mode = 1; ru.nblk = ext ? nblkx : nblk; b.kept = true; b.kept_fpn = ext;
+                if (ext) retain_layout_fpn(rplan[0], b.nb, R.slot[q], &ru); else retain_layout(rplan[0], b.nb, R.slot[q], ru.out, nblk);
             } else c->cut_fallbacks++;
             c->cut_kept[!b.kept ? CUT_KEPT_NONE : b.kept_fpn ? CUT_KEPT_FPN : CUT_KEPT_STAGES]++;
         }
@@ -368,7 +377,8 @@
     int cut_plan(int k, int V, const ViewDesc* vs, FwdReuse& ru) {
         cald_model::CutReuse& R = m->cr;
         const bool fpn = bt[k & 1].kept_fpn;
-        const size_t per = cut_plan_set_bytes(V), total = per * (2 * (size_t)nblk + (fpn ? 4 : 0));
+        const int nbk = fpn ? nblkx : nblk;
+        const size_t per = cut_plan_set_bytes(V), total = per * (2 * (size_t)nbk + (fpn ? 4 : 0));
         if (!R.d_gp) {
             const size_t cap = cut_plan_set_bytes(CALD_MAX_VIEWS) * (2 * CUT_MAX_BLOCKS + 4);
             HIPCHK(hipMalloc((void**)&R.d_gp, cap));
@@ -377,90 +387,107 @@
         plan_of(V, vs, rplan[0]);
         const BatchPlan& P = rplan[0];
         char* const h = R.h_gp[k & 1];
-        std::vector<CutSet> g_out((size_t)V * ngeo), g_t1((size_t)V * ngeo), g_fpn((size_t)V * 4);
+        std::vector<CutSet> g_out((size_t)V * ngeo), g_t1((size_t)V * ngeo), g_fpn((size_t)V * 4), g_inner((size_t)V * 4);
         for (int v = 0; v < V; v++) {
             int Hr, Wr, Hp, Wp; CutSet pool1;
             transform_size(vs[v].H, vs[v].W, m->cfg.min_size, m->cfg.max_size, &Hr, &Wr, &Hp, &Wp);
             cut_geometry(vs[v].H, vs[v].W, Hr, Wr, Hp, Wp, vs[v].nrect, vs[v].rects, ngeo, geo_stride, &pool1, &g_out[(size_t)v * ngeo], &g_t1[(size_t)v * ngeo]);
-            if (fpn) {
-                CutSet cs[4], inner[4];
+            if (fpn_ok) {
+                CutSet cs[4];
                 for (int i = 0; i < 4; i++) cs[i] = g_out[(size_t)v * ngeo + c_blk[i]];
-                cut_fpn_geometry(Hp, Wp, cs, inner, &g_fpn[(size_t)v * 4]);
-            }
-        }
-        auto put_set = [&](size_t index, int lvl, const CutSet* sets, size_t stride_v, int* tiles_out, double* rows_out) {
-            LevelSeg* sg = reinterpret_cast<LevelSeg*>(h + index * per);
-            GatherSet* gs = reinterpret_cast<GatherSet*>(reinterpret_cast<char*>(sg) + (size_t)(V + 1) * sizeof(LevelSeg));
-            int tiles = 0; double rows = 0.0;
+                cut_fpn_geometry(Hp, Wp, cs, &g_inner[(size_t)v * 4], &g_fpn[(size_t)v * 4]);
+            }
+        }
+        auto put_set = [&](long long index, int lvl, const CutSet* sets, size_t stride_v, int* tiles_out, double* rows_out) {
+            LevelSeg* sg = index < 0 ? nullptr : reinterpret_cast<LevelSeg*>(h + (size_t)index * per);
+            GatherSet* gs = index < 0 ? nullptr : reinterpret_cast<GatherSet*>(reinterpret_cast<char*>(sg) + (size_t)(V + 1) * sizeof(LevelSeg));
+            int tiles = 0, grows = 0;
             for (int v = 0; v < V; v++) {
-                LevelSeg L = P.seg[lvl][v]; L.tile_start = tiles; sg[v] = L;
+                LevelSeg L = P.seg[lvl][v]; L.tile_start = tiles; L.row_start = grows;
                 CutRect rr[CALD_GATHER_RECTS];
                 int n = cut_disjoint(sets[(size_t)v * stride_v], rr, CALD_GATHER_RECTS);
                 if (n < 0) { n = 1; rr[0] = {0, 0, L.W - 1, L.H - 1}; }
-                GatherSet& G = gs[v]; memset(&G, 0, sizeof(G));
+                GatherSet G; memset(&G, 0, sizeof(G));
                 G.nr = n;
                 for (int q = 0; q < n; q++) {
                     G.x0[q] = rr[q].x0; G.y0[q] = rr[q].y0; G.w[q] = rr[q].x1 - rr[q].x0 + 1;
                     G.cum[q + 1] = G.cum[q] + G.w[q] * (rr[q].y1 - rr[q].y0 + 1);
                 }
-                tiles += (G.cum[n] + 127) / 128; rows += (double)G.cum[n];
-            }
-            sg[V] = P.seg[lvl][V]; sg[V].tile_start = tiles;
-            *tiles_out = tiles; *rows_out = rows;
+                if (sg) { sg[v] = L; gs[v] = G; }
+                tiles += (G.cum[n] + 127) / 128; grows += G.cum[n];
+            }
+            if (sg) { sg[V] = P.seg[lvl][V]; sg[V].tile_start = tiles; sg[V].row_start = grows; }
+            *tiles_out = tiles; *rows_out = (double)grows;
         };
+        const bool pack = m->gather_packing < 0 ? gather_pack_default() : m->gather_packing != 0;
+        auto issued = [&](int tiles, double rows) { return pack ? (double)(((long long)rows + 127) / 128) : (double)tiles; };
         auto kf = [](const ConvLayer& L) { return (double)L.Cout * (double)(L.KH * L.KW * L.CinTrue); };
-        double cost_g[3] = {0, 0, 0}, cost_d[3] = {0, 0, 0}, rows_g[3] = {0, 0, 0}, rows_d[3] = {0, 0, 0}, tiles_g[3] = {0, 0, 0}, tiles_d[3] = {0, 0, 0};
-        for (int b = 0; b < nblk; b++)
+        double cost_g[4] = {0, 0, 0, 0}, cost_d[4] = {0, 0, 0, 0}, rows_g[4] = {0, 0, 0, 0}, rows_d[4] = {0, 0, 0, 0}, tiles_g[4] = {0, 0, 0, 0}, tiles_d[4] = {0, 0, 0, 0};
+        const int nset = fpn_ok ? nblk4 : nblk;
+        for (int b = 0; b < nset; b++)
             for (int kind = 0; kind < 2; kind++) {
                 const int lvl = kind ? blk_lin[b] : blk_lout[b];
                 int tiles; double rows;
-                put_set((size_t)(2 * b + kind), lvl, (kind ? g_t1.data() : g_out.data()) + b, (size_t)ngeo, &tiles, &rows);
-                ru.tiles[b][kind] = tiles; ru.rows[b][kind] = rows;
+                put_set(b < nbk ? (long long)(2 * b + kind) : -1, lvl, (kind ? g_t1.data() : g_out.data()) + b, (size_t)ngeo, &tiles, &rows);
                 const Bottleneck& Bk = m->blocks[b];
                 const double w = kind ? kf(Bk.c1) : kf(Bk.c2) + kf(Bk.c3) + (Bk.has_down ? kf(Bk.down) : 0.0);
                 const double nconv = kind ? 1.0 : (Bk.has_down ? 3.0 : 2.0), dense = (double)level_pix(P, lvl, V);
                 const int st = blk_stage[b];
-                cost_g[st] += 128.0 * tiles * w; cost_d[st] += dense * w;
-                rows_g[st] += rows * nconv; rows_d[st] += dense * nconv;
-                tiles_g[st] += tiles * nconv; tiles_d[st] += (double)P.seg[lvl][V].tile_start * nconv;
-            }
-        for (int st = 0; st < 3; st++) {
-            ru.gather[st] = m->cr.mode != 2 && cost_g[st] <= CUT_GATHER_MAX_COST * cost_d[st];
-            c->cut_rows[st] += ru.gather[st] ? rows_g[st] : rows_d[st]; c->cut_dense[st] += rows_d[st];
-            c->cut_st_rows[st] += ru.gather[st] ? rows_g[st] : rows_d[st]; c->cut_st_dense[st] += rows_d[st];
-            c->cut_st_tiles[st] += ru.gather[st] ? tiles_g[st] : tiles_d[st]; c->cut_st_dense_tiles[st] += tiles_d[st];
-        }
-        {
-            double r4 = 0.0, t4 = 0.0, rl = 0.0, tl = 0.0;
+                c->cut_gp_rows[st] += rows * nconv; c->cut_gp_view_tiles[st] += tiles * nconv; c->cut_gp_packed_tiles[st] += (double)(((long long)rows + 127) / 128) * nconv;
+                rows_d[st] += dense * nconv; tiles_d[st] += (double)P.seg[lvl][V].tile_start * nconv;
+                if (b >= nbk) continue;
+                ru.tiles[b][kind] = tiles; ru.rows[b][kind] = rows;
+                cost_g[st] += 128.0 * issued(tiles, rows) * w; cost_d[st] += dense * w;
+                rows_g[st] += rows * nconv; tiles_g[st] += issued(tiles, rows) * nconv;
+            }
+        const int nst = nbk > nblk ? 4 : 3;
+        if (nst == 3 && !fpn_ok) {
             int lvl = 2;
             for (size_t b = 0; b < m->blocks.size(); b++) {
                 const Bottleneck& Bk = m->blocks[b];
                 const int lo = lvl + (Bk.c2.stride == 2 ? 1 : 0);
                 if ((int)b >= nblk) {
-                    const double n_in = 1.0, n_out = Bk.has_down ? 3.0 : 2.0;
-                    r4 += n_in * (double)level_pix(P, lvl, V) + n_out * (double)level_pix(P, lo, V);
-                    t4 += n_in * (double)P.seg[lvl][V].tile_start + n_out * (double)P.seg[lo][V].tile_start;
+                    const double n_out = Bk.has_down ? 3.0 : 2.0;
+                    rows_d[3] += (double)level_pix(P, lvl, V) + n_out * (double)level_pix(P, lo, V);
+                    tiles_d[3] += (double)P.seg[lvl][V].tile_start + n_out * (double)P.seg[lo][V].tile_start;
                 }
                 lvl = lo;
             }
+        }
+        for (int st = 0; st < 4; st++) {
+            ru.gather[st] = st < nst && (m->cr.mode == 3 || (m->cr.mode != 2 && cost_g[st] <= CUT_GATHER_MAX_COST * cost_d[st]));
+            if (st < 3) { c->cut_rows[st] += ru.gather[st] ? rows_g[st] : rows_d[st]; c->cut_dense[st] += rows_d[st]; }
+            c->cut_st_rows[st] += ru.gather[st] ? rows_g[st] : rows_d[st]; c->cut_st_dense[st] += rows_d[st];
+            c->cut_st_tiles[st] += ru.gather[st] ? tiles_g[st] : tiles_d[st]; c->cut_st_dense_tiles[st] += tiles_d[st];
+        }
+        {
+            double rl = 0.0, tl = 0.0;
             if (!retina) for (int i = 0; i < 4; i++) { rl += (double)level_pix(P, 2 + i, V); tl += (double)P.seg[2 + i][V].tile_start; }
-            c->cut_st_rows[3] += r4; c->cut_st_dense[3] += r4; c->cut_st_tiles[3] += t4; c->cut_st_dense_tiles[3] += t4;
             c->cut_st_rows[CUT_STAGE_LATERAL] += rl; c->cut_st_dense[CUT_STAGE_LATERAL] += rl;
             c->cut_st_tiles[CUT_STAGE_LATERAL] += tl; c->cut_st_dense_tiles[CUT_STAGE_LATERAL] += tl;
             double fg = 0.0, fd = 0.0, frg = 0.0, frd = 0.0;
-            if (fpn)
+            if (fpn_ok)
                 for (int i = 0; i < 4; i++) {
-                    put_set(2 * (size_t)nblk + i, 2 + i, g_fpn.data() + i, 4, &ru.fpn_tiles[i], &ru.fpn_rows[i]);
-                    fg += ru.fpn_tiles[i]; frg += ru.fpn_rows[i];
+                    int tiles; double rows;
+                    put_set(-1, 2 + i, g_inner.data() + i, 4, &tiles, &rows);
+                    c->cut_gp_rows[CUT_STAGE_LATERAL] += rows; c->cut_gp_view_tiles[CUT_STAGE_LATERAL] += tiles;
+                    c->cut_gp_packed_tiles[CUT_STAGE_LATERAL] += (double)(((long long)rows + 127) / 128);
+                    put_set(fpn ? (long long)(2 * (size_t)nbk + i) : -1, 2 + i, g_fpn.data() + i, 4, &tiles, &rows);
+                    c->cut_gp_rows[CUT_STAGE_OUTPUT] += rows; c->cut_gp_view_tiles[CUT_STAGE_OUTPUT] += tiles;
+                    c->cut_gp_packed_tiles[CUT_STAGE_OUTPUT] += (double)(((long long)rows + 127) / 128);
+                    if (!fpn) continue;
+                    ru.fpn_tiles[i] = tiles; ru.fpn_rows[i] = rows;
+                    fg += issued(tiles, rows); frg += rows;
                 }
             if (!retina) for (int i = 0; i < 4; i++) { fd += (double)P.seg[2 + i][V].tile_start; frd += (double)level_pix(P, 2 + i, V); }
-            ru.gather_fpn = fpn && m->cr.mode != 2 && 128.0 * fg <= CUT_FPN_MAX_COST * frd;
+            ru.gather_fpn = fpn && (m->cr.mode == 3 || (m->cr.mode != 2 && 128.0 * fg <= CUT_FPN_MAX_COST * frd));
             c->cut_st_rows[CUT_STAGE_OUTPUT] += ru.gather_fpn ? frg : frd; c->cut_st_dense[CUT_STAGE_OUTPUT] += frd;
             c->cut_st_tiles[CUT_STAGE_OUTPUT] += ru.gather_fpn ? fg : fd; c->cut_st_dense_tiles[CUT_STAGE_OUTPUT] += fd;
         }
+        ru.pack = pack; ru.h_gp = h;
         if (hipMemcpyAsync(R.d_gp, h, total, hipMemcpyHostToDevice, c->stream) != hipSuccess) return fail(CALD_ERR_HIP, "H2D of the cut_out gather plan failed");
-        ru.mode = 2; ru.nblk = nblk; ru.d_gp = R.d_gp;
-        if (fpn) retain_layout_fpn(P, V, m->cr.slot[k & 1], &ru); else retain_layout(P, V, m->cr.slot[k & 1], ru.out);
+        ru.mode = 2; ru.nblk = nbk; ru.d_gp = R.d_gp;
+        if (fpn) retain_layout_fpn(P, V, m->cr.slot[k & 1], &ru); else retain_layout(P, V, m->cr.slot[k & 1], ru.out, nblk);
         c->cut_batches++;
         return 0;
     }
diff --git a/cald_amd/csrc/train_geom.hip b/cald_amd/csrc/train_geom.hip
--- a/cald_amd/csrc/train_geom.hip
+++ b/cald_amd/csrc/train_geom.hip
@@ -27,7 +27,7 @@
         if (g_seg.size() >= seg_cache_cap()) g_seg_evict = true;
         std::vector<LevelSeg> h(N + 1);
         const int tiles = (H * W + 127) / 128;
-        for (int v = 0; v <= N; v++) { h[v].pix_off = (long long)v * H * W; h[v].H = H; h[v].W = W; h[v].tile_start = v * tiles; h[v].pad_ = 0; }
+        for (int v = 0; v <= N; v++) { h[v].pix_off = (long long)v * H * W; h[v].H = H; h[v].W = W; h[v].tile_start = v * tiles; h[v].row_start = 0; }
         LevelSeg* d = nullptr;
         THIP(hipMalloc((void**)&d, sizeof(LevelSeg) * (N + 1)));
         THIP(hipMemcpy(d, h.data(), sizeof(LevelSeg) * (N + 1), hipMemcpyHostToDevice));
diff --git a/cald_amd/csrc/vaal.hip b/cald_amd/csrc/vaal.hip
--- a/cald_amd/csrc/vaal.hip
+++ b/cald_amd/csrc/vaal.hip
@@ -286,7 +286,7 @@
         const int side = VAAL_SIDE >> l, pix = kLevelPix[l], tiles = (pix + 127) / 128;
         for (int i = 0; i <= cap; i++) {
             LevelSeg& s = seg[(size_t)l * (cap + 1) + i];
-            s.pix_off = (long long)i * pix; s.H = side; s.W = side; s.tile_start = i * tiles; s.pad_ = 0;
+            s.pix_off = (long long)i * pix; s.H = side; s.W = side; s.tile_start = i * tiles; s.row_start = 0;
         }
     }
 }
diff --git a/include/cald_hip.h b/include/cald_hip.h
--- a/include/cald_hip.h
+++ b/include/cald_hip.h
@@ -309,6 +309,8 @@
 int cald_op_conv_probe(cald_ctx* ctx, int precision, cald_conv_probe* probs, int n, int path, int tile, char* kernel, int kernel_cap);
 int cald_op_row_pack_lookup(int V, const int* in_hw, const int* out_hw, int Cin, int out_ld, int64_t n, const int64_t* rows,
                             int* view_out, int64_t* local_out, int64_t* packed_rows_out);
+int cald_op_gather_pack_lookup(int V, const int* in_hw, const int* out_hw, const int* nrect, const int* rect, int Cin, int out_ld, int64_t n,
+                               const int64_t* rows, int* view_out, int64_t* local_out, int64_t* pixel_out, int64_t* packed_rows_out);
 int cald_op_mfma_f16(cald_ctx* ctx, const uint16_t* A, const uint16_t* B, const uint32_t* C, uint32_t* D, int64_t n);
 int cald_op_conv_bench(cald_ctx* ctx, int n_views, int H, int W, int Cin, int Cout, int KH, int stride, int pad, int residual,
                        int relu, int iters, int group, double* ms_out, double* tflops_out);
@@ -332,9 +334,12 @@
 int cald_model_set_cutout_reuse(cald_model* m, int mode, int* was);
 int cald_model_set_look_fuse(cald_model* m, int mode, int* was);
 int cald_model_set_row_packing(cald_model* m, int mode, int* was);
+int cald_model_set_gather_packing(cald_model* m, int mode, int* was);
+int cald_model_set_cutout_layer4(cald_model* m, int mode, int* was);
 int cald_model_set_box_min_size(cald_model* m, float min_size, float* was);
 int cald_profile_cutout(cald_ctx* ctx, double* rows3, double* dense_rows3, int64_t* batches, int64_t* fallbacks);
 int cald_profile_cutout_stages(cald_ctx* ctx, double* rows6, double* dense_rows6, double* tiles6, double* dense_tiles6, int64_t* kept3);
+int cald_profile_cutout_gather(cald_ctx* ctx, double* rows6, double* view_tiles6, double* packed_tiles6);
 int cald_model_set_cutout_retention_cap(cald_model* m, int64_t bytes, int64_t* was);
 int cald_debug_cutout_forward(cald_model* m, int n_views, const cald_view* views, const cald_dets* out, int prune);
 int cald_profile_roi_rows(cald_ctx* ctx, double* mean_rows_per_view, int64_t* views);
```

New measurement: 183.1, median of 6. Within noise of the previous version (+0.9%).
